# mratsim/trace-of-radiance

Measured on AMD Instinct MI355X. Metric: Msamples/s (pixels×spp/s) on book-1 random_scene, higher is better.
Workload: dtype f64

## Files before the change

include/tor_render.h:

```cpp
#ifndef TOR_RENDER_H
#define TOR_RENDER_H

#include <stddef.h>
#include <stdint.h>

#ifdef __cplusplus
extern "C" {
#endif

#define TOR_API __attribute__((visibility("default")))


typedef struct TorVec3 { double x, y, z; } TorVec3;

enum { TOR_LAMBERTIAN = 0, TOR_METAL = 1, TOR_DIELECTRIC = 2 };

typedef struct TorMaterial {
  uint8_t kind;
  uint8_t _pad[7];
  union {
    struct { TorVec3 albedo; } lambertian;
    struct { TorVec3 albedo; double fuzz; } metal;
    struct { double refraction_index; } dielectric;
  } u;
// ... 199 lines not shown
                                double time_hi, int32_t mode, TorHit* hits, const uint32_t* masks, uint32_t mask);
TOR_API int tor_occluded_masked_device(TorContext* ctx, int64_t n_rays, const TorRay* d_rays, const double* d_t_range,
                                       const int32_t* d_list, int64_t n_list, double time_lo, double time_hi, int32_t mode,
                                       int32_t* d_occluded, void* hip_stream, const uint32_t* d_mask, uint32_t mask);
TOR_API int tor_occluded_masked_host(TorContext* ctx, int64_t n_rays, const TorRay* rays, const double* t_range, const int32_t* list,
                                     int64_t n_list, double time_lo, double time_hi, int32_t mode, int32_t* occluded,
                                     const uint32_t* masks, uint32_t mask);
TOR_API int tor_bounce_masked_device(TorContext* ctx, int64_t n_rays, TorRay* d_rays, TorRng* d_rng, const int32_t* d_list,
                                     int64_t n_list, double time_lo, double time_hi, int32_t mode, TorHit* d_hits,
                                     double* d_attenuation, int32_t* d_status, void* hip_stream, const uint32_t* d_mask, uint32_t mask);

enum { TOR_CROSSINGS_MAX = 16 };
typedef struct TorCrossing { double t; int32_t object; int32_t which; } TorCrossing;
TOR_API int tor_crossings_device(TorContext* ctx, int64_t n_rays, const TorRay* d_rays, const double* d_t_range, const int32_t* d_list,
                                 int64_t n_list, int32_t k, const uint32_t* d_mask, uint32_t mask, double time_lo, double time_hi,
                                 int32_t mode, TorCrossing* d_cross, int32_t* d_count, TorHit* d_records, void* hip_stream);
TOR_API int tor_crossings_host(TorContext* ctx, int64_t n_rays, const TorRay* rays, const double* t_range, const int32_t* list,
                               int64_t n_list, int32_t k, const uint32_t* masks, uint32_t mask, double time_lo, double time_hi,
                               int32_t mode, TorCrossing* cross, int32_t* count, TorHit* records);

typedef struct TorPoint { TorVec3 p; double time; } TorPoint;
enum { TOR_NEAREST_MAX = 16 };
typedef struct TorNear { double distance; int32_t object; int32_t inside; } TorNear;
TOR_API int tor_nearest_device(TorContext* ctx, int64_t n_points, const TorPoint* d_points, const double* d_max_dist, const int32_t* d_list,
                               int64_t n_list, int32_t k, const uint32_t* d_mask, uint32_t mask, double time_lo, double time_hi,
                               int32_t mode, TorNear* d_near, int32_t* d_count, void* hip_stream);
TOR_API int tor_nearest_host(TorContext* ctx, int64_t n_points, const TorPoint* points, const double* max_dist, const int32_t* list,
                             int64_t n_list, int32_t k, const uint32_t* masks, uint32_t mask, double time_lo, double time_hi,
                             int32_t mode, TorNear* near, int32_t* count);

TOR_API int tor_deposit_device(TorContext* ctx, int64_t n, const double* d_color, const int32_t* d_pixel, const int32_t* d_index,
                               int64_t n_index, double max_value, int64_t npix, double* d_sums, double* d_moments, int32_t* d_counts,
                               int64_t* d_rejected, void* hip_stream);

TOR_API int tor_comm_unique_id(uint8_t id_out[128]);
TOR_API int tor_comm_init_rank(TorContext* ctx, const uint8_t id[128], int32_t rank, int32_t world);
TOR_API int tor_comm_destroy(TorContext* ctx);
TOR_API int tor_comm_abort(TorContext* ctx);
TOR_API int tor_comm_count(TorContext* ctx, int32_t* ranks_out);
TOR_API int tor_render_gather_device(TorContext* ctx, const TorCamera* cam, int32_t nrows, int32_t ncols,
                                     int32_t samples_per_pixel, float gamma_correction, int64_t max_depth,
                                     const TorOptions* opt, int32_t root, double* d_frame, void* hip_stream);

TOR_API int tor_context_handoff_stalled(TorContext* ctx, int32_t* stalled_out, int64_t* total_out);

TOR_API int tor_context_scene_counters(TorContext* ctx, int64_t out[3]);

TOR_API int tor_quantize_rgb8_device(TorContext* ctx, const double* d_pixels, int64_t n_values,
                                     uint8_t* d_rgb8, void* hip_stream);

TOR_API int tor_h264_stream_header(int32_t width, int32_t height, uint8_t* out, int32_t cap);
TOR_API int64_t tor_h264_frame_bytes(int32_t width, int32_t height);
TOR_API int tor_mp4_mux_file(const char* src_annexb_path, const char* dst_mp4_path, int32_t width,
                             int32_t height, int32_t fps);
TOR_API int tor_encode_frame_device(TorContext* ctx, const double* d_pixels, int32_t nrows, int32_t ncols,
                                    uint8_t* d_slice, uint8_t* d_y, uint8_t* d_cb, uint8_t* d_cr,
                                    void* hip_stream);

TOR_API int tor_render_frame_h264(TorContext* ctx, const TorCamera* cam, int32_t nrows, int32_t ncols,
                                  int32_t samples_per_pixel, float gamma_correction, int64_t max_depth,
                                  const TorOptions* opt, uint8_t* slice_out, int64_t cap);

TOR_API int tor_last_kernel_ms(TorContext* ctx, float* ms_out, int64_t* samples_out);
TOR_API int tor_kernel_ms_mean(TorContext* ctx, int32_t last_n, float* mean_ms_out, int32_t* n_used_out);

typedef struct TorStats {
  uint64_t hit_queries;
  uint64_t object_tests;
  uint64_t candidates;
  uint64_t wave_iterations;
  uint64_t lane_slots;
  uint64_t samples;
  uint64_t block_tests;
  uint64_t exact_tests;
} TorStats;
TOR_API int tor_context_set_stats(TorContext* ctx, int32_t enable);
TOR_API int tor_last_stats(TorContext* ctx, TorStats* out);
TOR_API int tor_last_wave_log(TorContext* ctx, uint64_t* out, int64_t cap_waves);
TOR_API int tor_last_handoff_counters(TorContext* ctx, uint64_t out[16]);
TOR_API int64_t tor_last_pixel_cost(TorContext* ctx, uint32_t* out, int64_t cap_pixels);


TOR_API int tor_camera_init(TorCamera* out, const TorVec3* look_from, const TorVec3* look_at,
                            const TorVec3* view_up, double vertical_fov_degrees,
                            double aspect_ratio, double aperture, double focus_distance,
                            double shutter_open, double shutter_close);

TOR_API int64_t tor_random_scene(uint64_t seed, TorHittableVariant* out, int64_t cap);

typedef struct TorAnimation TorAnimation;
TOR_API int tor_animation_create(uint64_t seed, int32_t height, int32_t width, float dt, float t_min,
                                 float t_max, TorAnimation** out);
TOR_API void tor_animation_destroy(TorAnimation* anim);
TOR_API int64_t tor_animation_object_count(const TorAnimation* anim);
TOR_API int tor_animation_next(TorAnimation* anim, int32_t skip, TorCamera* cam, TorHittableVariant* objects,
                               int64_t cap, int64_t* n_out, float* t_out);

TOR_API int tor_canvas_to_rgb8(const TorCanvas* canvas, uint8_t* out);


TOR_API int tor_debug_accel_layout(TorHittableList world, double t_lo, double t_hi, int64_t* slot_object,
                                   int64_t slot_cap, double* block_boxes, double* super_boxes, int64_t box_cap,
                                   int32_t* two_level_out);

TOR_API int tor_debug_last_variant(TorContext* ctx, int32_t out[5]);
TOR_API int tor_debug_last_split_tiles(TorContext* ctx, int64_t* tiles_out);

TOR_API int tor_debug_filter32_scene(TorHittableList world, int64_t n_rays, const double* o, const double* d,
                                     const double* time, int8_t* keep);

TOR_API int tor_debug_screen2_scene(TorHittableList world, int64_t n_rays, const double* o, const double* d,
                                    const double* time, int8_t* keep, int32_t* kind_out, int8_t* pays_out, int64_t n_segs_out);

TOR_API int tor_debug_plane32_scene(TorHittableList world, int64_t n_rays, const double* o, const double* d, const double* time,
                                    int8_t* keep, int32_t* pad_kept, int64_t* n_pad_out);

TOR_API int tor_debug_layout_segments(TorHittableList world, int32_t* out, int64_t max_segs, int64_t* n_segs_out);

TOR_API int tor_selftest_slab32_host(int64_t n, const double* o, const double* d, const double* lo, const double* hi,
                                     const double* origin, int32_t* keep, int32_t* need);

TOR_API int tor_selftest_filter32_host(int64_t n, const double* o, const double* d, const double* c0,
                                       const double* dc, const int32_t* moving, const double* f, const double* r2,
                                       const double* origin, int32_t* keep, int32_t* need);

TOR_API int tor_selftest_screen_host(int64_t n, const double* o, const double* d, const double* c0,
                                     const double* dc, const int32_t* moving, const double* f, const double* r2,
                                     int32_t* keep, int32_t* need);
TOR_API int tor_selftest_screen2_host(int64_t n, const double* o, const double* d, const double* c0,
                                      const double* dc, const int32_t* moving, const double* f, const double* r2,
                                      int32_t variant, int32_t* keep, int32_t* need);

TOR_API int tor_selftest_math_device(int32_t op, const double* x, const double* y, double* out0,
                                     double* out1, int64_t n, int32_t device);
TOR_API int tor_selftest_math_host(int32_t op, const double* x, const double* y, double* out0,
                                   double* out1, int64_t n);
TOR_API int tor_selftest_rng_host(int32_t mode, uint64_t a, uint64_t b, uint64_t c,
                                  uint64_t state_out[4], uint64_t* draws_out, int64_t n);

TOR_API const char* tor_version(void);

#ifdef __cplusplus
}
#endif

#include "tor_lights.h"

#include "tor_env.h"

#include "tor_camera.h"

#include "tor_bsdf.h"

#endif
```

trace-of-radiance_amd/__init__.py:

```python
from __future__ import annotations

import ctypes as C
import os
import subprocess
import sys

import numpy as np

_HERE = os.path.dirname(os.path.abspath(__file__))
LIB_PATH = os.path.join(_HERE, "lib", "libtor_mi355x.so")
INCLUDE_DIR = os.path.join(os.path.dirname(_HERE), "include")

SEED_PIXEL, SEED_SAMPLE = 0, 1
ARITH_STRICT, ARITH_FUSED = 0, 1
ACCEL_NONE, ACCEL_BLOCKS, ACCEL_F32 = 0, 1, 2
GATHER_AUTO, GATHER_RCCL, GATHER_PEER, GATHER_HOST = 0, 1, 2, 3
PIXEL_KERNEL_AUTO, PIXEL_KERNEL_LANE, PIXEL_KERNEL_WAVE = 0, 1, 2
OK, ERR_INVALID_ARGUMENT, ERR_NO_DEVICE, ERR_HIP, ERR_OUT_OF_MEMORY, ERR_INCOMPLETE = 0, -1, -2, -3, -4, -5
MAX_DEVICES = 16
LAMBERTIAN, METAL, DIELECTRIC = 0, 1, 2
SPHERE, MOVING_SPHERE = 0, 1


class TorError(RuntimeError):
    def __init__(self, code: int, msg: str):
        super().__init__(f"tor_mi355x error {code}: {msg}")
        self.code = code


class Vec3(C.Structure):
    _fields_ = [("x", C.c_double), ("y", C.c_double), ("z", C.c_double)]


class _Lambertian(C.Structure):
    _fields_ = [("albedo", Vec3)]


class _Metal(C.Structure):
    _fields_ = [("albedo", Vec3), ("fuzz", C.c_double)]


class _Dielectric(C.Structure):
    _fields_ = [("refraction_index", C.c_double)]


class _MaterialU(C.Union):
    _fields_ = [("lambertian", _Lambertian), ("metal", _Metal), ("dielectric", _Dielectric)]


class Material(C.Structure):
    _fields_ = [("kind", C.c_uint8), ("_pad", C.c_uint8 * 7), ("u", _MaterialU)]


class Sphere(C.Structure):
    _fields_ = [("center", Vec3), ("radius", C.c_double), ("material", Material)]


class MovingSphere(C.Structure):
    _fields_ = [("center0", Vec3), ("center1", Vec3), ("time0", C.c_double), ("time1", C.c_double),
                ("radius", C.c_double), ("material", Material)]


class _HittableU(C.Union):
    _fields_ = [("sphere", Sphere), ("moving_sphere", MovingSphere)]


class HittableVariant(C.Structure):
    _fields_ = [("kind", C.c_uint8), ("_pad", C.c_uint8 * 7), ("u", _HittableU)]


class HittableList(C.Structure):
    _fields_ = [("len", C.c_int64), ("objects", C.POINTER(HittableVariant))]


class Camera(C.Structure):
    _fields_ = [("origin", Vec3), ("lower_left_corner", Vec3), ("horizontal", Vec3), ("vertical", Vec3),
                ("u", Vec3), ("v", Vec3), ("w", Vec3), ("lens_radius", C.c_double),
                ("shutter_open", C.c_double), ("shutter_close", C.c_double)]

    def as_array(self) -> np.ndarray:
        return np.frombuffer(bytes(self), dtype=np.float64).copy()


class CanvasStruct(C.Structure):
    _fields_ = [("pixels", C.POINTER(Vec3)), ("nrows", C.c_int32), ("ncols", C.c_int32),
                ("samples_per_pixel", C.c_int32), ("gamma_correction", C.c_float)]


class Options(C.Structure):
    _fields_ = [("struct_size", C.c_uint32), ("seeding", C.c_int32), ("arith", C.c_int32),
                ("device", C.c_int32), ("shard_index", C.c_int32), ("shard_count", C.c_int32),
                ("row_tile", C.c_int32), ("accel", C.c_int32),
                ("device_count", C.c_int32), ("gather", C.c_int32), ("devices", C.c_int32 * MAX_DEVICES),
                ("pixel_kernel", C.c_int32)]


class Stats(C.Structure):
    _fields_ = [("hit_queries", C.c_uint64), ("object_tests", C.c_uint64), ("candidates", C.c_uint64),
                ("wave_iterations", C.c_uint64), ("lane_slots", C.c_uint64), ("samples", C.c_uint64),
                ("block_tests", C.c_uint64), ("exact_tests", C.c_uint64)]


class Ray(C.Structure):
    _fields_ = [("origin", Vec3), ("direction", Vec3), ("time", C.c_double)]


class Hit(C.Structure):
    _fields_ = [("p", Vec3), ("normal", Vec3), ("t", C.c_double), ("object", C.c_int32), ("front_face", C.c_int32)]


class Rng(C.Structure):
    _fields_ = [("s0", C.c_uint64), ("s1", C.c_uint64), ("s2", C.c_uint64), ("s3", C.c_uint64)]


assert C.sizeof(Rng) == 32
assert C.sizeof(Ray) == 56 and C.sizeof(Hit) == 64 and Hit.object.offset == 56 and Hit.front_face.offset == 60
assert C.sizeof(Vec3) == 24 and C.sizeof(Material) == 40 and C.sizeof(Sphere) == 72
assert C.sizeof(MovingSphere) == 112 and C.sizeof(HittableVariant) == 120
assert C.sizeof(HittableList) == 16 and C.sizeof(Camera) == 192 and C.sizeof(CanvasStruct) == 24

EXPORTED_SYMBOLS = [
    "tor_render", "tor_render_opt", "tor_last_error", "tor_context_create", "tor_context_destroy",
    "tor_scene_upload", "tor_shard_rows", "tor_render_device", "tor_quantize_rgb8_device",
    "tor_last_kernel_ms", "tor_kernel_ms_mean", "tor_context_set_stats", "tor_last_stats", "tor_last_wave_log", "tor_camera_init",
    "tor_random_scene", "tor_canvas_to_rgb8", "tor_animation_create", "tor_animation_destroy",
    "tor_animation_object_count", "tor_animation_next", "tor_h264_stream_header", "tor_h264_frame_bytes",
    "tor_encode_frame_device", "tor_render_frame_h264", "tor_mp4_mux_file", "tor_debug_accel_layout", "tor_selftest_filter32_host", "tor_selftest_screen_host", "tor_selftest_slab32_host", "tor_debug_filter32_scene", "tor_selftest_math_device", "tor_selftest_math_host",
    "tor_selftest_rng_host", "tor_version",
    "tor_last_render_timing", "tor_comm_unique_id", "tor_comm_init_rank", "tor_comm_destroy", "tor_render_gather_device",
    "tor_context_scene_counters", "tor_render_ptr", "tor_last_pixel_cost", "tor_last_note", "tor_last_handoff_counters",
    "tor_selftest_screen2_host", "tor_debug_screen2_scene", "tor_debug_layout_segments", "tor_debug_plane32_scene", "tor_knob_count", "tor_knob_info", "tor_last_gather_info", "tor_last_device_kernel_ms", "tor_comm_abort", "tor_comm_count", "tor_context_handoff_stalled",
    "tor_render_accumulate_device", "tor_resolve_device", "tor_accum_noise_device",
    "tor_render_accumulate_list_device", "tor_adaptive_select_device", "tor_resolve_counts_device", "tor_debug_last_variant",
    "tor_hit_device", "tor_hit_host", "tor_radiance_device", "tor_radiance_host", "tor_camera_rays_device",
    "tor_bounce_device", "tor_bounce_host", "tor_scatter_device", "tor_scatter_host", "tor_sky_device", "tor_bounce_select_device",
    "tor_render_resume_device", "tor_debug_last_split_tiles", "tor_render_resume_list_device",
    "tor_occluded_device", "tor_occluded_host",
    "tor_scene_groups", "tor_hit_masked_device", "tor_hit_masked_host", "tor_occluded_masked_device", "tor_occluded_masked_host",
    "tor_bounce_masked_device",
    "tor_crossings_device", "tor_crossings_host",
    "tor_nearest_device", "tor_nearest_host",
    "tor_deposit_device",
]
LIGHT_SYMBOLS = ["tor_scene_lights", "tor_light_sample_device", "tor_light_sample_host", "tor_light_pdf_device", "tor_light_pdf_host"]
LIGHT_BY_WEIGHT, LIGHT_BY_SOLID_ANGLE = 0, 1
LIGHT_STRATEGIES = {"weight": LIGHT_BY_WEIGHT, "solid_angle": LIGHT_BY_SOLID_ANGLE}
ENV_SYMBOLS = ["tor_scene_environment", "tor_env_sample_device", "tor_env_sample_host", "tor_env_eval_device", "tor_env_eval_host"]
ENV_MAX_SIDE = 2048
CAMERA_SYMBOLS = ["tor_camera_connect_device", "tor_camera_connect_host", "tor_light_emit_device", "tor_light_emit_host"]
BSDF_SYMBOLS = ["tor_bsdf_eval_device", "tor_bsdf_eval_host"]
BSDF_NONE, BSDF_DENSITY, BSDF_DELTA = 0, 1, 2
HIT_AUTO, HIT_BRUTE, HIT_BLOCKS = 0, 1, 2
HIT_MODES = {"auto": HIT_AUTO, "brute": HIT_BRUTE, "blocks": HIT_BLOCKS}
BOUNCE_MISS, BOUNCE_SCATTERED, BOUNCE_ABSORBED = 0, 1, 2
CROSSINGS_MAX = 16
NEAREST_MAX = 16
DEPOSIT_MAX_VALUE = 128.0
MAT_LAMBERTIAN, MAT_METAL, MAT_DIELECTRIC = 0, 1, 2

_lib = None


def build(force: bool = False) -> str:
    import fcntl
    src_dir = os.path.join(_HERE, "csrc")
    lock_path = os.path.join(src_dir, ".build.lock")
    if not os.access(src_dir, os.W_OK):
        import hashlib
        import tempfile
        lock_path = os.path.join(tempfile.gettempdir(), "tor_mi355x_" + hashlib.sha1(src_dir.encode()).hexdigest()[:12] + ".lock")
    with open(lock_path, "w") as lock:
        fcntl.flock(lock, fcntl.LOCK_EX)
        try:
            cmd = ["make", "-C", src_dir] + (["-B"] if force or not os.path.exists(LIB_PATH) else []) + ["all"]
            r = subprocess.run(cmd, capture_output=True, text=True)
            if r.returncode != 0:
                raise TorError(-3, f"building libtor_mi355x.so failed ({' '.join(cmd)}):\n{r.stdout[-4000:]}\n{r.stderr[-8000:]}")
        finally:
            fcntl.flock(lock, fcntl.LOCK_UN)
    return LIB_PATH


def ensure_built() -> str:
    if not os.path.exists(LIB_PATH):
        build()
    return LIB_PATH


def lib():
    global _lib
    if _lib is not None:
        return _lib
    if not os.path.exists(LIB_PATH):
        raise TorError(-2, f"HIP extension missing: {LIB_PATH} (run __graft_entry__.build()); "
                           "there is no CPU fallback")
    if os.environ.get("TOR_NO_TORCH", "0") != "1":
        try:
            import torch
        except Exception:
            pass
    ab = os.environ.get("TOR_AB_LIB")
    if ab:
        print(f"trace-of-radiance_amd: TOR_AB_LIB set -- loading {ab} instead of the in-tree library", file=sys.stderr, flush=True)
    L = C.CDLL(ab or LIB_PATH)
    _bind(L, skip_missing=bool(ab))
    _bind_lights(L, skip_missing=bool(ab))
    _bind_env(L, skip_missing=bool(ab))
    _bind_camera(L, skip_missing=bool(ab))
    _bind_bsdf(L, skip_missing=bool(ab))
    _lib = L
    return L


def _signatures() -> dict:
    v, i32, i64, u32, u64, d, f, P = C.c_void_p, C.c_int32, C.c_int64, C.c_uint32, C.c_uint64, C.c_double, C.c_float, C.POINTER
    dp, cam, opt, obj = P(d), P(Camera), P(Options), P(HittableVariant)
    frame = [v, cam, i32, i32, i32, f, i64, opt]
    passes = [v, cam, i32, i32, i32, i32, i64, opt]
    listed = [v, cam, i32, i32, v, i32, i32, i32, i64, opt]
    return {
        "tor_last_error": (None, C.c_char_p),
        "tor_version": (None, C.c_char_p),
        "tor_last_note": (None, C.c_char_p),
        "tor_render": [P(CanvasStruct), cam, HittableList, i64],
        "tor_render_ptr": [P(CanvasStruct), cam, P(HittableList), i64],
        "tor_render_opt": [P(CanvasStruct), cam, HittableList, i64, opt],
        "tor_context_create": [i32, P(v)],
        "tor_context_destroy": [v],
        "tor_scene_upload": [v, HittableList],
        "tor_shard_rows": [i32, i32, i32, i32, P(i32)],
        "tor_render_device": frame + [v, v],
        "tor_quantize_rgb8_device": [v, v, i64, v, v],
        "tor_last_kernel_ms": [v, P(f), P(i64)],
        "tor_kernel_ms_mean": [v, i32, P(f), P(i32)],
        "tor_context_set_stats": [v, i32],
        "tor_last_stats": [v, P(Stats)],
        "tor_last_wave_log": [v, P(u64), i64],
        "tor_last_pixel_cost": ([v, P(u32), i64], i64),
        "tor_last_handoff_counters": [v, P(u64)],
        "tor_camera_init": [cam, P(Vec3), P(Vec3), P(Vec3)] + [d] * 6,
        "tor_random_scene": ([u64, obj, i64], i64),
        "tor_canvas_to_rgb8": [P(CanvasStruct), P(C.c_uint8)],
        "tor_animation_create": [u64, i32, i32, f, f, f, P(v)],
        "tor_animation_destroy": ([v], None),
        "tor_animation_object_count": ([v], i64),
        "tor_animation_next": [v, i32, cam, obj, i64, P(i64), P(f)],
        "tor_h264_stream_header": [i32, i32, P(C.c_uint8), i32],
        "tor_h264_frame_bytes": ([i32, i32], i64),
        "tor_encode_frame_device": [v, v, i32, i32, v, v, v, v, v],
        "tor_render_frame_h264": frame + [P(C.c_uint8), i64],
        "tor_mp4_mux_file": [C.c_char_p, C.c_char_p, i32, i32, i32],
        "tor_debug_accel_layout": [HittableList, d, d, P(i64), i64, dp, dp, i64, P(i32)],
        "tor_selftest_filter32_host": [i64] + [dp] * 4 + [P(i32)] + [dp] * 3 + [P(i32)] * 2,
        "tor_selftest_screen_host": [i64] + [dp] * 4 + [P(i32)] + [dp] * 2 + [P(i32)] * 2,
        "tor_selftest_screen2_host": [i64] + [dp] * 4 + [P(i32)] + [dp] * 2 + [i32] + [P(i32)] * 2,
        "tor_selftest_slab32_host": [i64] + [dp] * 5 + [P(i32)] * 2,
        "tor_debug_filter32_scene": [HittableList, i64] + [dp] * 3 + [P(C.c_int8)],
        "tor_debug_screen2_scene": [HittableList, i64] + [dp] * 3 + [P(C.c_int8), P(i32), P(C.c_int8), i64],
        "tor_debug_plane32_scene": [HittableList, i64] + [dp] * 3 + [P(C.c_int8), P(i32), P(i64)],
        "tor_debug_layout_segments": [HittableList, P(i32), i64, P(i64)],
        "tor_selftest_math_device": [i32, dp, dp, dp, dp, i64, i32],
        "tor_selftest_math_host": [i32, dp, dp, dp, dp, i64],
        "tor_selftest_rng_host": [i32, u64, u64, u64, P(u64), P(u64), i64],
        "tor_last_render_timing": [dp],
        "tor_comm_unique_id": [P(C.c_uint8)],
        "tor_comm_init_rank": [v, P(C.c_uint8), i32, i32],
        "tor_comm_destroy": [v],
        "tor_render_gather_device": frame + [i32, v, v],
        "tor_context_scene_counters": [v, P(i64)],
        "tor_knob_count": (None, i32),
        "tor_knob_info": [i32] + [P(C.c_char_p)] * 5,
        "tor_last_gather_info": [P(i32)],
        "tor_last_device_kernel_ms": [P(f), i32],
        "tor_comm_abort": [v],
        "tor_comm_count": [v, P(i32)],
        "tor_context_handoff_stalled": [v, P(i32), P(i64)],
        "tor_render_accumulate_device": passes + [v, v, v],
        "tor_resolve_device": [v, v, i64, i64, f, v, v],
        "tor_accum_noise_device": [v, v, v, i64, i64, v, dp, v],
        "tor_render_accumulate_list_device": listed + [v, v, v],
        "tor_adaptive_select_device": [v, v, v, v, i32, i64, d, d, v, v, P(i32), v],
        "tor_resolve_counts_device": [v, v, v, i64, f, v, v],
        "tor_debug_last_variant": [v, P(i32)],
        "tor_render_resume_device": passes + [v, v, v, v],
        "tor_debug_last_split_tiles": [v, P(i64)],
        "tor_render_resume_list_device": listed + [v, v, v, v],
        "tor_hit_device": [v, i64, v, v, d, d, i32, v, v],
        "tor_hit_host": [v, i64, v, v, d, d, i32, v],
        "tor_hit_masked_device": [v, i64, v, v, d, d, i32, v, v, v, u32],
        "tor_hit_masked_host": [v, i64, v, v, d, d, i32, v, v, u32],
        "tor_radiance_device": [v, i64, v, v, i32, d, d, i32, v, v],
        "tor_radiance_host": [v, i64, v, v, i32, d, d, i32, v],
        "tor_camera_rays_device": [v, cam, i32, i32, v, i64, i32, i32, i32, v, v, v],
        "tor_bounce_device": [v, i64, v, v, v, i64, d, d, i32, v, v, v, v],
        "tor_bounce_host": [v, i64, v, v, v, i64, d, d, i32, v, v, v],
        "tor_bounce_masked_device": [v, i64, v, v, v, i64, d, d, i32, v, v, v, v, v, u32],
        "tor_scatter_device": [v, i64, v, v, v, v, i64, v, v, v],
        "tor_scatter_host": [v, i64, v, v, v, v, i64, v, v],
        "tor_sky_device": [v, i64, v, v, i64, v, v],
        "tor_bounce_select_device": [v, i64, v, v, i64, v, P(i64), v],
        "tor_occluded_device": [v, i64, v, v, v, i64, d, d, i32, v, v],
        "tor_occluded_host": [v, i64, v, v, v, i64, d, d, i32, v],
        "tor_occluded_masked_device": [v, i64, v, v, v, i64, d, d, i32, v, v, v, u32],
        "tor_occluded_masked_host": [v, i64, v, v, v, i64, d, d, i32, v, v, u32],
        "tor_scene_groups": [v, i64, v],
        "tor_crossings_device": [v, i64, v, v, v, i64, i32, v, u32, d, d, i32, v, v, v, v],
        "tor_crossings_host": [v, i64, v, v, v, i64, i32, v, u32, d, d, i32, v, v, v],
        "tor_nearest_device": [v, i64, v, v, v, i64, i32, v, u32, d, d, i32, v, v, v],
        "tor_nearest_host": [v, i64, v, v, v, i64, i32, v, u32, d, d, i32, v, v],
        "tor_deposit_device": [v, i64, v, v, v, i64, d, i64, v, v, v, v, v],
    }


_SIGNATURES = _signatures()


def _bind(L, names=None, skip_missing=False) -> None:
    for name in _SIGNATURES if names is None else names:
        if skip_missing and not hasattr(L, name):
            continue
        sig = _SIGNATURES[name]
        argtypes, *restype = sig if isinstance(sig, tuple) else (sig,)
        fn = getattr(L, name)
        if argtypes is not None:
            fn.argtypes = argtypes
        if restype:
            fn.restype = restype[0]


def _light_signatures() -> dict:
    v, i32, i64 = C.c_void_p, C.c_int32, C.c_int64
    return {
        "tor_scene_lights": [v, i64, v, v],
        "tor_light_sample_device": [v, i64, v, v, v, i64, i32, v, v, v, v, v],
        "tor_light_sample_host": [v, i64, v, v, v, i64, i32, v, v, v, v],
        "tor_light_pdf_device": [v, i64, v, v, v, i64, i32, v, v],
        "tor_light_pdf_host": [v, i64, v, v, v, i64, i32, v],
    }


_LIGHT_SIGNATURES = _light_signatures()


def _bind_lights(L, skip_missing=False) -> None:
    for name in LIGHT_SYMBOLS:
        if skip_missing and not hasattr(L, name):
            continue
        getattr(L, name).argtypes = _LIGHT_SIGNATURES[name]


def _env_signatures() -> dict:
    v, i64 = C.c_void_p, C.c_int64
    return {
        "tor_scene_environment": [v, i64, v, v],
        "tor_env_sample_device": [v, i64, v, v, v, i64, v, v, v, v, v],
        "tor_env_sample_host": [v, i64, v, v, v, i64, v, v, v, v],
        "tor_env_eval_device": [v, i64, v, v, i64, v, v, v, v],
        "tor_env_eval_host": [v, i64, v, v, i64, v, v, v],
    }


_ENV_SIGNATURES = _env_signatures()


def _bind_env(L, skip_missing=False) -> None:
    for name in ENV_SYMBOLS:
        if skip_missing and not hasattr(L, name):
            continue
        getattr(L, name).argtypes = _ENV_SIGNATURES[name]


def _camera_signatures() -> dict:
    v, i32, i64, d, cam = C.c_void_p, C.c_int32, C.c_int64, C.c_double, C.POINTER(Camera)
    return {
        "tor_camera_connect_device": [v, cam, i32, i32, i64, v, v, v, i64, v, v, v, v, v],
        "tor_camera_connect_host": [v, cam, i32, i32, i64, v, v, v, i64, v, v, v, v],
        "tor_light_emit_device": [v, i64, v, v, i64, d, d, v, v, v, v, v],
        "tor_light_emit_host": [v, i64, v, v, i64, d, d, v, v, v, v],
    }


_CAMERA_SIGNATURES = _camera_signatures()


def _bind_camera(L, skip_missing=False) -> None:
    for name in CAMERA_SYMBOLS:
        if skip_missing and not hasattr(L, name):
            continue
        getattr(L, name).argtypes = _CAMERA_SIGNATURES[name]


def _bsdf_signatures() -> dict:
    v, i64 = C.c_void_p, C.c_int64
    return {
        "tor_bsdf_eval_device": [v, i64, v, v, v, v, i64, v, v, v, v],
        "tor_bsdf_eval_host": [v, i64, v, v, v, v, i64, v, v, v],
    }


_BSDF_SIGNATURES = _bsdf_signatures()


def _bind_bsdf(L, skip_missing=False) -> None:
    for name in BSDF_SYMBOLS:
        if skip_missing and not hasattr(L, name):
            continue
        getattr(L, name).argtypes = _BSDF_SIGNATURES[name]


def _check(rc: int) -> None:
    if rc != 0:
        raise TorError(rc, lib().tor_last_error().decode("utf-8", "replace"))


_GOLDEN, _MIX = np.uint64(0x9e3779b97f4a7c15), np.uint64(0xbf58476d1ce4e5b9)


def _u64(x) -> np.ndarray:
    a = np.asarray(x)
    if a.dtype.kind == "u":
        return a.astype(np.uint64).reshape(-1)
    if a.dtype.kind == "i":
        return a.astype(np.int64).view(np.uint64).reshape(-1)
    return np.array([int(v) & 0xFFFFFFFFFFFFFFFF for v in a.reshape(-1)], dtype=np.uint64)


def _splitmix64(state: np.ndarray):
    with np.errstate(over="ignore"):
        state = state + _GOLDEN
        r = (state ^ (state >> np.uint64(30))) * _MIX
        r = (r ^ (r >> np.uint64(27))) * _MIX
    return state, r ^ (r >> np.uint64(31))


def rng_seed1(x) -> np.ndarray:
    sm = _u64(x)
    out = np.empty((sm.shape[0], 4), dtype=np.uint64)
    for k in range(4):
        sm, out[:, k] = _splitmix64(sm)
    return out


def rng_seed2(x, y) -> np.ndarray:
    x, y = np.broadcast_arrays(_u64(x), _u64(y))
    return rng_seed1((x << np.uint64(32)) ^ y)


def rng_seed3(row, col, sample) -> np.ndarray:
    row, col, sample = np.broadcast_arrays(_u64(row), _u64(col), _u64(sample))
    _, h = _splitmix64((row << np.uint64(32)) ^ col)
    return rng_seed1(h ^ sample)


def vec3(x, y, z) -> Vec3:
    return Vec3(float(x), float(y), float(z))


def camera(look_from=(13, 2, 3), look_at=(0, 0, 0), view_up=(0, 1, 0), vertical_field_of_view=20.0,
           aspect_ratio=16.0 / 9.0, aperture=0.1, focus_distance=10.0, shutter_open=0.0,
           shutter_close=1.0) -> Camera:
    cam = Camera()
    a, b, c = vec3(*look_from), vec3(*look_at), vec3(*view_up)
    _check(lib().tor_camera_init(C.byref(cam), C.byref(a), C.byref(b), C.byref(c),
                                 vertical_field_of_view, aspect_ratio, aperture, focus_distance,
                                 shutter_open, shutter_close))
    return cam


class Scene:

    def __init__(self, objects=None, n: int = 0):
        self.objects = objects if objects is not None else (HittableVariant * 1)()
        self.n = n

    def list(self) -> HittableList:
        return HittableList(self.n, C.cast(self.objects, C.POINTER(HittableVariant)))

    def __len__(self):
        return self.n

    @staticmethod
    def from_records(recs: np.ndarray) -> "Scene":
        n = int(recs.shape[0])
        arr = (HittableVariant * max(n, 1))()
        for i in range(n):
            r = recs[i]
            h = arr[i]
            mat = Material()
            mat.kind = int(r[10])
            if mat.kind == LAMBERTIAN:
                mat.u.lambertian.albedo = vec3(r[11], r[12], r[13])
            elif mat.kind == METAL:
                mat.u.metal.albedo = vec3(r[11], r[12], r[13])
                mat.u.metal.fuzz = float(r[14])
            else:
                mat.u.dielectric.refraction_index = float(r[15])
            if int(r[0]) == SPHERE:
                h.kind = SPHERE
                h.u.sphere.center = vec3(r[1], r[2], r[3])
                h.u.sphere.radius = float(r[9])
                h.u.sphere.material = mat
            else:
                h.kind = MOVING_SPHERE
                h.u.moving_sphere.center0 = vec3(r[1], r[2], r[3])
                h.u.moving_sphere.center1 = vec3(r[4], r[5], r[6])
                h.u.moving_sphere.time0 = float(r[7])
                h.u.moving_sphere.time1 = float(r[8])
                h.u.moving_sphere.radius = float(r[9])
                h.u.moving_sphere.material = mat
        return Scene(arr, n)

    def to_records(self) -> np.ndarray:
        out = np.zeros((self.n, 16), dtype=np.float64)
        for i in range(self.n):
            h = self.objects[i]
            if h.kind == SPHERE:
                s = h.u.sphere
                c0 = c1 = s.center
                t0, t1, rad, m = 0.0, 1.0, s.radius, s.material
            else:
                s = h.u.moving_sphere
                c0, c1, t0, t1, rad, m = s.center0, s.center1, s.time0, s.time1, s.radius, s.material
            out[i, 0] = h.kind
            out[i, 1:4] = (c0.x, c0.y, c0.z)
            out[i, 4:7] = (c1.x, c1.y, c1.z)
            out[i, 7:10] = (t0, t1, rad)
            out[i, 10] = m.kind
            if m.kind == LAMBERTIAN:
                a = m.u.lambertian.albedo
                out[i, 11:14] = (a.x, a.y, a.z)
            elif m.kind == METAL:
                a = m.u.metal.albedo
                out[i, 11:14] = (a.x, a.y, a.z)
                out[i, 14] = m.u.metal.fuzz
            else:
                out[i, 15] = m.u.dielectric.refraction_index
        return out


def random_scene(seed: int = 0xFACADE) -> Scene:
    cap = 2048
    arr = (HittableVariant * cap)()
    n = lib().tor_random_scene(seed, arr, cap)
    if n < 0:
        raise TorError(int(n), "tor_random_scene failed")
    return Scene(arr, int(n))


class Animation:

    def __init__(self, height: int, width: int, dt: float = 0.005, t_min: float = 0.0, t_max: float = 2.0,
                 seed: int = 0xFACADE):
        self._h = C.c_void_p()
        _check(lib().tor_animation_create(seed, height, width, dt, t_min, t_max, C.byref(self._h)))
        self.n_objects = int(lib().tor_animation_object_count(self._h))

    def scenes(self, skip: int = 6):
        while True:
            cam = Camera()
            arr = (HittableVariant * self.n_objects)()
# ... 1800 lines not shown
        self.rng = torch.zeros((self.rows, self.ncols, 4), dtype=torch.int64, device=self.sums.device)

    def _pass(self, k: int, stream: int) -> None:
        self.ctx.resume_list_device(self.cam, self.nrows, self.ncols, self._list.data_ptr(), self.active, self.samples, k,
                                    self.max_depth, self.options, self.rng.data_ptr(), self.sums.data_ptr(), self.moments.data_ptr(),
                                    stream)

    def state(self) -> dict:
        st = super().state()
        st["rng"] = self.rng.cpu().numpy().view(np.uint64)
        return st

    @classmethod
    def from_state(cls, ctx: Context, cam: Camera, nrows: int, ncols: int, max_depth: int, options: Options | None, state: dict,
                   device=None, **policy) -> "PixelAdaptive":
        import torch
        opts = options if options is not None else cls._default_options()
        want = (cls._shard_rows(nrows, opts), int(ncols), 4)
        rng = np.asarray(state.get("rng"))
        if rng.dtype != np.uint64 or rng.shape != want:
            raise TorError(ERR_INVALID_ARGUMENT, f"PixelAdaptive.from_state: generator states of dtype {rng.dtype}, shape {rng.shape}; "
                                                 f"expected uint64 {want}")
        ad = super().from_state(ctx, cam, nrows, ncols, max_depth, options, state, device=device, **policy)
        ad.rng.copy_(torch.from_numpy(np.ascontiguousarray(rng).view(np.int64)))
        return ad


def mp4_mux_file(src_annexb_path: str, dst_mp4_path: str, width: int, height: int, fps: int = 30) -> int:
    n = lib().tor_mp4_mux_file(os.fsencode(src_annexb_path), os.fsencode(dst_mp4_path), width, height, fps)
    if n < 0:
        raise TorError(n, lib().tor_last_error().decode())
    return n


def debug_accel_layout(world: HittableList, t_lo: float, t_hi: float):
    cap = int(world.len) + 64
    slots = np.full(cap, -1, dtype=np.int64)
    boxes = np.zeros((cap // 8 + 16, 6), dtype=np.float64)
    supers = np.zeros((cap // 64 + 16, 6), dtype=np.float64)
    two = C.c_int32(0)
    n = lib().tor_debug_accel_layout(world, t_lo, t_hi, slots.ctypes.data_as(C.POINTER(C.c_int64)), cap,
                                     boxes.ctypes.data_as(C.POINTER(C.c_double)),
                                     supers.ctypes.data_as(C.POINTER(C.c_double)), boxes.shape[0], C.byref(two))
    if n < 0:
        raise TorError(n, "tor_debug_accel_layout failed")
    if n == 0:
        return None
    n_p = (n + 7) // 8 * 8
    return slots[: n * 8].reshape(n, 8), boxes[:n_p], supers[: n_p // 8], bool(two.value)


def selftest_filter32(o, d, c0, dc, moving, f, r2, origin):
    dp = lambda x: np.ascontiguousarray(x, dtype=np.float64)
    o, d, c0, dc, f, r2, origin = dp(o), dp(d), dp(c0), dp(dc), dp(f), dp(r2), dp(origin)
    moving = np.ascontiguousarray(moving, dtype=np.int32)
    n = len(f)
    keep = np.zeros(n, dtype=np.int32)
    need = np.zeros(n, dtype=np.int32)
    P = C.POINTER(C.c_double)
    I = C.POINTER(C.c_int32)
    _check(lib().tor_selftest_filter32_host(n, o.ctypes.data_as(P), d.ctypes.data_as(P), c0.ctypes.data_as(P),
                                            dc.ctypes.data_as(P), moving.ctypes.data_as(I), f.ctypes.data_as(P),
                                            r2.ctypes.data_as(P), origin.ctypes.data_as(P), keep.ctypes.data_as(I),
                                            need.ctypes.data_as(I)))
    return keep, need


def selftest_screen(o, d, c0, dc, moving, f, r2):
    dp = lambda x: np.ascontiguousarray(x, dtype=np.float64)
    o, d, c0, dc, f, r2 = dp(o), dp(d), dp(c0), dp(dc), dp(f), dp(r2)
    moving = np.ascontiguousarray(moving, dtype=np.int32)
    n = len(f)
    keep = np.zeros(n, dtype=np.int32)
    need = np.zeros(n, dtype=np.int32)
    P = C.POINTER(C.c_double)
    I = C.POINTER(C.c_int32)
    _check(lib().tor_selftest_screen_host(n, o.ctypes.data_as(P), d.ctypes.data_as(P), c0.ctypes.data_as(P), dc.ctypes.data_as(P),
                                          moving.ctypes.data_as(I), f.ctypes.data_as(P), r2.ctypes.data_as(P), keep.ctypes.data_as(I),
                                          need.ctypes.data_as(I)))
    return keep, need


def selftest_screen2(o, d, c0, dc, moving, f, r2, variant=0):
    dp = lambda x: np.ascontiguousarray(x, dtype=np.float64)
    o, d, c0, dc, f, r2 = dp(o), dp(d), dp(c0), dp(dc), dp(f), dp(r2)
    moving = np.ascontiguousarray(moving, dtype=np.int32)
    n = len(f)
    keep = np.zeros(n, dtype=np.int32)
    need = np.zeros(n, dtype=np.int32)
    P = C.POINTER(C.c_double)
    I = C.POINTER(C.c_int32)
    _check(lib().tor_selftest_screen2_host(n, o.ctypes.data_as(P), d.ctypes.data_as(P), c0.ctypes.data_as(P), dc.ctypes.data_as(P),
                                           moving.ctypes.data_as(I), f.ctypes.data_as(P), r2.ctypes.data_as(P), int(variant),
                                           keep.ctypes.data_as(I), need.ctypes.data_as(I)))
    return keep, need


def selftest_slab32(o, d, lo, hi, origin):
    dp = lambda x: np.ascontiguousarray(x, dtype=np.float64)
    o, d, lo, hi, origin = dp(o), dp(d), dp(lo), dp(hi), dp(origin)
    n = len(o)
    keep = np.zeros(n, dtype=np.int32)
    need = np.zeros(n, dtype=np.int32)
    P = C.POINTER(C.c_double)
    I = C.POINTER(C.c_int32)
    _check(lib().tor_selftest_slab32_host(n, o.ctypes.data_as(P), d.ctypes.data_as(P), lo.ctypes.data_as(P), hi.ctypes.data_as(P),
                                          origin.ctypes.data_as(P), keep.ctypes.data_as(I), need.ctypes.data_as(I)))
    return keep, need


def debug_filter32_scene(world: HittableList, o, d, time):
    dp = lambda x: np.ascontiguousarray(x, dtype=np.float64)
    o, d, time = dp(o), dp(d), dp(time)
    keep = np.zeros((len(time), int(world.len)), dtype=np.int8)
    P = C.POINTER(C.c_double)
    _check(lib().tor_debug_filter32_scene(world, len(time), o.ctypes.data_as(P), d.ctypes.data_as(P), time.ctypes.data_as(P),
                                          keep.ctypes.data_as(C.POINTER(C.c_int8))))
    return keep


def debug_layout_segments(world: HittableList, max_segs: int = 64):
    out = np.zeros((max_segs, 4), dtype=np.int32)
    n = C.c_int64(0)
    _check(lib().tor_debug_layout_segments(world, out.ctypes.data_as(C.POINTER(C.c_int32)), max_segs, C.byref(n)))
    return [tuple(int(v) for v in row) for row in out[:min(int(n.value), max_segs)]]


def debug_screen2_scene(world: HittableList, o, d, time, max_segs: int = 0):
    dp = lambda x: np.ascontiguousarray(x, dtype=np.float64)
    o, d, time = dp(o), dp(d), dp(time)
    keep = np.zeros((len(time), int(world.len)), dtype=np.int8)
    kind = np.zeros(int(world.len), dtype=np.int32)
    pays = np.full((len(time), max(max_segs, 1)), -1, dtype=np.int8)
    P = C.POINTER(C.c_double)
    _check(lib().tor_debug_screen2_scene(world, len(time), o.ctypes.data_as(P), d.ctypes.data_as(P), time.ctypes.data_as(P),
                                         keep.ctypes.data_as(C.POINTER(C.c_int8)), kind.ctypes.data_as(C.POINTER(C.c_int32)),
                                         pays.ctypes.data_as(C.POINTER(C.c_int8)) if max_segs > 0 else None, max_segs))
    return (keep, kind, pays) if max_segs > 0 else (keep, kind)


def debug_plane32_scene(world: HittableList, o, d, time):
    dp = lambda x: np.ascontiguousarray(x, dtype=np.float64)
    o, d, time = dp(o), dp(d), dp(time)
    keep = np.zeros((len(time), int(world.len)), dtype=np.int8)
    pad_kept = np.zeros(len(time), dtype=np.int32)
    n_pad = C.c_int64(0)
    P = C.POINTER(C.c_double)
    _check(lib().tor_debug_plane32_scene(world, len(time), o.ctypes.data_as(P), d.ctypes.data_as(P), time.ctypes.data_as(P),
                                         keep.ctypes.data_as(C.POINTER(C.c_int8)), pad_kept.ctypes.data_as(C.POINTER(C.c_int32)),
                                         C.byref(n_pad)))
    return keep, pad_kept, int(n_pad.value)


def selftest_math(op: int, x: np.ndarray, y: np.ndarray | None = None, where: str = "device", device: int = -1):
    x = np.ascontiguousarray(x, dtype=np.float64)
    yy = np.ascontiguousarray(y, dtype=np.float64) if y is not None else None
    o0 = np.zeros_like(x)
    o1 = np.zeros_like(x)
    dp = C.POINTER(C.c_double)
    yp = yy.ctypes.data_as(dp) if yy is not None else None
    if where == "device":
        _check(lib().tor_selftest_math_device(op, x.ctypes.data_as(dp), yp, o0.ctypes.data_as(dp),
                                              o1.ctypes.data_as(dp), x.size, device))
    else:
        _check(lib().tor_selftest_math_host(op, x.ctypes.data_as(dp), yp, o0.ctypes.data_as(dp),
                                            o1.ctypes.data_as(dp), x.size))
    return o0, o1


def selftest_rng(mode: int, a: int, b: int = 0, c: int = 0, n: int = 4):
    state = (C.c_uint64 * 4)()
    draws = (C.c_uint64 * max(n, 1))()
    _check(lib().tor_selftest_rng_host(mode, a, b, c, state, draws, n))
    return [int(v) for v in state], [int(v) for v in draws[:n]]
```

trace-of-radiance_amd/csrc/kernel/integrate_loop_plane.inc:

```
            if constexpr (kWords) {
            const int x_first = h_xfirst;
            const int pl_first = h_plfirst;
            const bool mover = xkind >= 12;
            double f = 0.0;
            if (mover) {
              f = (time - SEG_T0) / SEG_DT;
              fc_f = f; fc_t0 = double_to_bits(SEG_T0); fc_dt = double_to_bits(SEG_DT);
            }
            const int i_begin = i;
            {
              const PlaneSeg ps = plane_seg(sray, pray, SEG_REACH, SEG_TRAVEL, f, h_rmax2);
              auto stage_one = [&](auto PWc) {
                constexpr int PW = decltype(PWc)::value;
                using Rec = std::conditional_t<PW == 2, float, double>;
                using RecPtr = std::conditional_t<PW == 2, cfptr, cdptr>;
                RecPtr rec = (RecPtr)(uintptr_t)(PW == 2 ? (const void*)p.xpl32 : (const void*)p.xpl) + ((long)pl_first + PW * (long)i);
                PlaneSeg32 ps32{};
                Rec n0, n1, n2 = 0, n3 = 0;
                if constexpr (PW == 2) {
                  ps32 = plane_seg32(sray, ps, h_r1, h_r2, (double)__int_as_float(__double2loint(h_r3)), (double)__int_as_float(__double2hiint(h_r3)));
                  n0 = __int_as_float(__double2loint(h_r0)); n1 = __int_as_float(__double2hiint(h_r0));
                } else {
                  n0 = h_r0; n1 = h_r1; n2 = h_r2; n3 = h_r3;
                }
                if (i != 0) {
                  n0 = rec[0]; n1 = rec[1];
                  if constexpr (PW == 4) { n2 = rec[2]; n3 = rec[3]; }
                }
                auto one = [&](unsigned m, int j) {
                  const Rec c0 = n0, c1 = n1, c2 = n2, c3 = n3;
                  n0 = rec[PW * (j + 1) + 0]; n1 = rec[PW * (j + 1) + 1];
                  if constexpr (PW == 4) {
                    n2 = rec[PW * (j + 1) + 2]; n3 = rec[PW * (j + 1) + 3];
                    return push_bit(m, plane_word_mov(ps, c0, c1, c2, c3));
                  } else {
                    (void)c2; (void)c3;
                    return push_bit(m, plane_word32(ps32, c0, c1));
                  }
                };
                int gb = seg_block0 + (int)((unsigned)i / (unsigned)kBlock);
                for (;;) {
                  while (i < seg_count && ((gb & 3) != 0 || seg_count - i < 4 * kBlock)) {
                    unsigned m = mw;
                    if (seg_real - i <= kBlock / 2) {
#pragma unroll
                      for (int j = 0; j < kBlock / 2; ++j) m = one(m, j);
                      m <<= (unsigned)(kBlock / 2);
                    } else {
#pragma unroll
                      for (int j = 0; j < kBlock; ++j) m = one(m, j);
                    }
                    rec += PW * kBlock;
                    mw = m;
                    gb_next = gb + 1;
                    i += kBlock;
                    if ((gb & 3) == 3) {
                      q[(unsigned)w_count * 64] = m;
                      nz = push_cond(nz, m != 0u);
                      w_count += 1;
                      if (w_count == kQCap) { full = true; break; }
                    }
                    gb += 1;
                  }
                  if (full || i >= seg_count) break;
                  int nw = (seg_count - i) / (4 * kBlock);
                  nw = nw < kQCap - w_count ? nw : kQCap - w_count;
                  unsigned m = 0;
                  int w = 0;
                  auto word = [&]() {
                    m = 0;
#pragma unroll
                    for (int j = 0; j < 4 * kBlock; ++j) m = one(m, j);
                    rec += PW * 4 * kBlock;
                    q[(unsigned)(w_count + w) * 64] = m;
                    nz = push_cond(nz, m != 0u);
                    w += 1;
                  };
#pragma unroll 1
                  while (w + 2 <= nw) { word(); word(); }
                  if (w < nw) word();
                  mw = m;
                  i += nw * 4 * kBlock;
                  gb += 4 * nw;
                  gb_next = gb;
                  w_count += nw;
                  if (w_count == kQCap) { full = true; break; }
                }
              };
              if (xkind == 13) stage_one(std::integral_constant<int, 4>{});
              else stage_one(std::integral_constant<int, 2>{});
            }
            {
              const int slot0 = seg_block0 * kBlock;
              const int slot_a = slot0 + i_begin, slot_b = slot0 + i;
              const int nb = gb_next & 3;
              const bool partial = !full && nb != 0;
              unsigned nzl = nz;
              if (partial) {
                const unsigned placed = mw << (unsigned)(8 * (4 - nb));
                q[(unsigned)w_count * 64] = placed;
                nzl = push_cond(nzl, placed != 0u);
              }
              const int k_a = (slot_a >> 5) - w_base, k_b = ((slot_b - 1) >> 5) - w_base;
              nzl &= (2u << (unsigned)(k_b - k_a)) - 1u;
              const bool shared_word = slot_b > slot_a && (slot_a & 31) != 0;
              unsigned sat_out = 0;
              if (shared_word) {
                const unsigned first_mask = 0xffffffffu >> (unsigned)(slot_a & 31);
                const unsigned w = q[(unsigned)k_a * 64];
                sat_out = w & ~first_mask;
                q[(unsigned)k_a * 64] = w & first_mask;
              }
              int k = k_a;
              unsigned cur = 0;
              unsigned* wp = q;
              const unsigned last_slot = (unsigned)(slot_b - 1);
              struct Pick { bool v; unsigned* w; int b; unsigned slot; };
              auto pick = [&]() {
                if (cur == 0 && nzl != 0) {
                  const int wb = 31 - __builtin_clz(nzl);
                  nzl &= ~(1u << wb);
                  k = k_b - wb;
                  wp = q + (unsigned)k * 64;
                  cur = *wp;
                }
                Pick c;
                c.v = cur != 0;
                c.b = 31 - __builtin_clz(cur | 1u);
                cur &= ~(1u << c.b);
                c.w = wp;
                const unsigned slot = ((unsigned)(w_base + k) << 5) + (unsigned)(31 - c.b);
                c.slot = slot < last_slot ? slot : last_slot;
                return c;
              };
              unsigned long long s2_t0 = 0;
              if (prof && lane == 0) s2_t0 = __builtin_readcyclecounter();
              if (slot_b > slot_a && xkind <= 12) {
                const ScreenSeg ss = screen2_seg(sray, SEG_REACH, SEG_TRAVEL, h_y, f);
                auto stage_two = [&](auto xr, auto KINDc) {
                  constexpr int KIND = decltype(KINDc)::value;
                  struct Cand { bool v; unsigned* w; int b; double r0, r1, r2, r3; };
                  constexpr bool kRecLds = std::is_same<decltype(xr), ldptr>::value;
                  unsigned lds_base = 0;
                  if constexpr (kRecLds) {
                    lds_base = (unsigned)(uintptr_t)xr;
                    asm volatile("" : "+v"(lds_base));
                  }
                  auto fetch = [&](Cand& c) {
                    const Pick pk = pick();
                    c.v = pk.v; c.w = pk.w; c.b = pk.b;
                    if constexpr (kRecLds) {
                      const ldptr r = (ldptr)(uintptr_t)(lds_base + pk.slot * 32u);
                      c.r0 = r[0]; c.r1 = r[1]; c.r2 = r[2]; c.r3 = r[3];
                    } else {
                      const auto r = xr + 4 * (long)pk.slot;
                      c.r0 = r[0]; c.r1 = r[1]; c.r2 = r[2]; c.r3 = r[3];
                    }
                  };
                  auto test = [&](const Cand& c) {
                    const int word = KIND == 12   ? screen2_movy_y<true>(ss, c.r0, c.r1, c.r2, c.r3)
                                     : KIND == 11 ? screen2_static_y<true>(ss, c.r0, c.r1, c.r2)
                                                  : screen2_static<true>(ss, c.r0, c.r1, c.r2, c.r3);
                    if (c.v && word >= 0) atomicAnd(c.w, ~(1u << c.b));
                  };
                  Cand ca{false, q, 0, 0.0, 0.0, 0.0, 0.0}, cb{false, q, 0, 0.0, 0.0, 0.0, 0.0};
                  fetch(ca);
                  for (;;) {
                    if (ballot64(ca.v || nzl != 0) == 0) break;
                    fetch(cb);
                    test(ca);
                    if (ballot64(cb.v || nzl != 0) == 0) break;
                    fetch(ca);
                    test(cb);
                  }
                };
                auto run = [&](auto KINDc) {
                  if (xstaged) stage_two((ldptr)stage + ((long)x_first - 4 * (long)slot0), KINDc);
                  else stage_two((gdptr)(uintptr_t)p.xrec + ((long)x_first - 4 * (long)slot0), KINDc);
                };
                if (xkind == 12) run(std::integral_constant<int, 12>{});
                else if (xkind == 11) run(std::integral_constant<int, 11>{});
                else run(std::integral_constant<int, 10>{});
                plane_ran = true;
              } else if (slot_b > slot_a) {
                double negmu, am;
                screen_margins(scr_s1 + SEG_REACH + SEG_TRAVEL * __builtin_fabs(f), scr_d1, a, negmu, am);
                const double neg_f = -f;
                auto stage_two = [&](auto xr) {
                  constexpr bool kRecLds = std::is_same<decltype(xr), ldptr>::value;
                  unsigned lds_base = 0;
                  if constexpr (kRecLds) {
                    lds_base = (unsigned)(uintptr_t)xr;
                    asm volatile("" : "+v"(lds_base));
                  }
                  for (;;) {
                    const Pick pk = pick();
                    if (ballot64(pk.v || nzl != 0) == 0) break;
                    double r0, r1, r2, r3, r4, r5, r6;
                    if constexpr (kRecLds) {
                      const ldptr r = (ldptr)(uintptr_t)(lds_base + pk.slot * 64u);
                      r0 = r[0]; r1 = r[1]; r2 = r[2]; r3 = r[3]; r4 = r[4]; r5 = r[5]; r6 = r[6];
                    } else {
                      const auto r = xr + 8 * (long)pk.slot;
                      r0 = r[0]; r1 = r[1]; r2 = r[2]; r3 = r[3]; r4 = r[4]; r5 = r[5]; r6 = r[6];
                    }
                    const int word = screen_filter(fma_(neg_f, r4, ox - r0), fma_(neg_f, r5, oy - r1), fma_(neg_f, r6, oz - r2), dx, dy, dz, a, negmu, am, r3);
                    if (pk.v && word >= 0) atomicAnd(pk.w, ~(1u << pk.b));
                  }
                };
                if (xstaged) stage_two((ldptr)stage + ((long)x_first - 8 * (long)slot0));
                else stage_two((gdptr)(uintptr_t)p.xrec + ((long)x_first - 8 * (long)slot0));
                plane_ran = true;
              }
              if (prof && lane == 0) prof_lds[kSecStage2] += __builtin_readcyclecounter() - s2_t0;
              if (shared_word) q[(unsigned)k_a * 64] |= sat_out;
              if (partial) mw = q[(unsigned)w_count * 64] >> (unsigned)(8 * (4 - nb));
            }
            }
```

trace-of-radiance_amd/csrc/tor_api.cpp:

```cpp
#include "../../include/tor_render.h"

#include <hip/hip_runtime_api.h>

#include <chrono>
#include <cmath>
#include <cstdio>
#include <cstdlib>
#include <cstring>
#include <map>
#include <mutex>
#include <new>
#include <string>
#include <utility>
#include <vector>

#include "tor_context.hpp"
#include "tor_knobs.hpp"
#include "tor_screen.hpp"

static_assert(sizeof(TorVec3) == 24, "Vec3 is 3 x float64 (vec3s.nim:12-14)");
static_assert(sizeof(TorMaterial) == 40 && offsetof(TorMaterial, u) == 8, "Material (core.nim:16-28)");
static_assert(sizeof(TorSphere) == 72, "Sphere (spheres.nim:15-18)");
static_assert(sizeof(TorMovingSphere) == 112, "MovingSphere (moving_spheres.nim:15-20)");
static_assert(sizeof(TorHittableVariant) == 120 && offsetof(TorHittableVariant, u) == 8,
              "HittableVariant (hittables_variants.nim:50-57)");
static_assert(sizeof(TorHittableList) == 16, "HittableList (hittables_lists.nim:20-24)");
static_assert(sizeof(TorCamera) == 192, "Camera (cameras.nim:15-22)");
static_assert(sizeof(TorCanvas) == 24, "Canvas (canvas.nim:20-28)");
static_assert(sizeof(tor::Camera) == sizeof(TorCamera), "device camera mirrors TorCamera");
static_assert(offsetof(TorOptions, device_count) == 32, "the round-1 TorOptions is a prefix of the current one");

namespace {
std::mutex g_handoff_mutex;
std::map<int, hipEvent_t> g_handoff_event;
thread_local std::string g_last_error = "";
thread_local double g_last_timing[5] = {0, 0, 0, 0, 0};
}

namespace tor {

void set_last_error(const std::string& msg) { g_last_error = msg; }

int fail(int code, const std::string& msg) {
  g_last_error = msg;
  return code;
}

int fail_hip(hipError_t e, const char* what) {
  std::string m = std::string(what) + ": " + hipGetErrorString(e);
  if (e == hipErrorNoDevice || e == hipErrorInvalidDevice || e == hipErrorInsufficientDriver)
    return fail(TOR_ERR_NO_DEVICE, m + " (libtor_mi355x has no CPU fallback)");
  if (e == hipErrorOutOfMemory) return fail(TOR_ERR_OUT_OF_MEMORY, m);
  return fail(TOR_ERR_HIP, m);
}

hipError_t DeviceLayout::put(const HostLayout& lay, const std::vector<double>* cold_override) {
  const std::vector<double>& c = cold_override ? *cold_override : lay.cold;
  struct Part { const void* src; size_t bytes; size_t off; };
  Part parts[11] = {{lay.stat.data(), lay.stat.size() * 8, 0}, {lay.mov.data(), lay.mov.size() * 8, 0},
                   {lay.movy.data(), lay.movy.size() * 8, 0}, {lay.segs.data(), lay.segs.size() * 8, 0},
                   {c.data(), c.size() * 8, 0},               {lay.hot32.data(), lay.hot32.size() * 4, 0},
                   {lay.coop_trips.data(), lay.coop_trips.size() * 8, 0},
                   {lay.xhdr.data(), lay.xhdr.size() * 8, 0}, {lay.xrec.data(), lay.xrec.size() * 8, 0},
                    {lay.xpl.data(), lay.xpl.size() * 8, 0}, {lay.xpl32.data(), lay.xpl32.size() * 4, 0}};
  size_t total = 0;
  for (Part& p : parts) {
    p.off = total;
    total += (p.bytes + 255) / 256 * 256 + 256;
  }
  std::vector<unsigned char> host(total, 0);
  for (const Part& p : parts)
    if (p.bytes > 0) std::memcpy(host.data() + p.off, p.src, p.bytes);
  hipError_t e = blob.ensure(total);
  if (e == hipSuccess) e = hipMemcpy(blob.ptr, host.data(), total, hipMemcpyHostToDevice);
  const char* b = (const char*)blob.ptr;
  stat = (const double*)(b + parts[0].off);
  mov = (const double*)(b + parts[1].off);
  movy = (const double*)(b + parts[2].off);
  segs = (const double*)(b + parts[3].off);
  cold = (const double*)(b + parts[4].off);
  hot32 = (const float*)(b + parts[5].off);
  coop_trips = (const double*)(b + parts[6].off);
  xhdr = (const double*)(b + parts[7].off);
  xrec = (const double*)(b + parts[8].off);
  xpl = (const double*)(b + parts[9].off);
  xpl32 = (const float*)(b + parts[10].off);
  n_segs = lay.n_segs;
  n_sorted = (int)lay.n_sorted;
  n_xrec = (int)lay.xrec.size();
  has_f32 = false;
  for (int s = 0; s < lay.n_segs; ++s) has_f32 = has_f32 || lay.segs[8 * (size_t)s] >= 5.0;
  return e;
}

static bool parse_device_list(const char* e, TorOptions& o) {
  int count = 0;
  if (hipGetDeviceCount(&count) != hipSuccess || count <= 0) return false;
  o.device_count = 0;
  if (std::strcmp(e, "all") == 0) {
    for (int d = 0; d < count && d < TOR_MAX_DEVICES; ++d) o.devices[o.device_count++] = d;
    return true;
  }
  const char* p = e;
  while (*p) {
    char* endp = nullptr;
    const long v = std::strtol(p, &endp, 10);
    if (endp == p || v < 0 || v >= count || o.device_count >= TOR_MAX_DEVICES) return false;
    o.devices[o.device_count++] = (int32_t)v;
    p = endp;
    if (*p == ',') ++p;
    else if (*p) return false;
  }
  return o.device_count > 0;
}

thread_local std::string g_options_why;
const std::string& options_why() { return g_options_why; }

bool valid_options(const TorOptions* opt, TorOptions& o, bool for_drop_in) {
  g_options_why.clear();
  auto no = [](const char* why) { g_options_why = why; return false; };
  o = TorOptions{};
  o.struct_size = sizeof(TorOptions);
  o.seeding = TOR_SEED_PIXEL;
  o.arith = TOR_ARITH_STRICT;
  o.device = -1;
  o.shard_index = 0;
  o.shard_count = 1;
  o.row_tile = 1;
  o.gather = TOR_GATHER_AUTO;
  constexpr uint32_t kV1Size = 32;
  if (opt) {
    if (opt->struct_size == sizeof(TorOptions)) o = *opt;
    else if (opt->struct_size == kV1Size) std::memcpy(&o, opt, kV1Size);
    else return no("struct_size is neither sizeof(TorOptions) nor the 32-byte round-1 layout");
    o.struct_size = sizeof(TorOptions);
  } else if (for_drop_in) {
    o.accel = TOR_ACCEL_BLOCKS | TOR_ACCEL_F32;
    if (const char* e = tor::knob("TOR_DEFAULT_ACCEL")) {
      char* endp = nullptr;
      const long v = std::strtol(e, &endp, 10);
      if (endp != e && *endp == 0 && v >= 0 && v <= (TOR_ACCEL_BLOCKS | TOR_ACCEL_F32)) o.accel = (int32_t)v;
      else return no("TOR_DEFAULT_ACCEL must be 0, 1, 2 or 3");
    }
    if (const char* e = tor::knob("TOR_DEFAULT_SEEDING")) {
      if (!std::strcmp(e, "sample")) o.seeding = TOR_SEED_SAMPLE;
      else if (!std::strcmp(e, "pixel")) o.seeding = TOR_SEED_PIXEL;
      else return no("TOR_DEFAULT_SEEDING must be pixel or sample");
    }
    if (const char* e = tor::knob("TOR_DEVICES")) {
      TorOptions t = o;
      if (parse_device_list(e, t)) o = t;
      else return no("TOR_DEVICES must be \"all\" or a comma list of HIP device ordinals that exist (at most TOR_MAX_DEVICES)");
    }
    if (const char* e = tor::knob("TOR_GATHER")) {
      if (!std::strcmp(e, "rccl")) o.gather = TOR_GATHER_RCCL;
      else if (!std::strcmp(e, "peer")) o.gather = TOR_GATHER_PEER;
      else if (!std::strcmp(e, "host")) o.gather = TOR_GATHER_HOST;
      else if (!std::strcmp(e, "auto")) o.gather = TOR_GATHER_AUTO;
      else return no("TOR_GATHER must be auto, rccl, peer or host");
    }
  }
  if (o.seeding != TOR_SEED_PIXEL && o.seeding != TOR_SEED_SAMPLE) return no("seeding must be TOR_SEED_PIXEL or TOR_SEED_SAMPLE");
  if (o.arith == TOR_ARITH_FUSED)
    return no("TOR_ARITH_FUSED was removed in round 5: it was not the reference's rounding (README.md:82) and TOR_ARITH_STRICT behind the conservative "
              "FMA screen is faster -- pass TOR_ARITH_STRICT (0)");
  if (o.arith != TOR_ARITH_STRICT) return no("arith must be TOR_ARITH_STRICT");
  if (o.accel < 0 || o.accel > (TOR_ACCEL_BLOCKS | TOR_ACCEL_F32)) return no("accel holds unknown TOR_ACCEL_* bits");
  if (o.shard_count < 1) o.shard_count = 1;
  if (o.row_tile == 0) o.row_tile = 1;
  if (o.row_tile < 0) return no("row_tile must be >= 1");
  if (o.shard_index < 0 || o.shard_index >= o.shard_count) return no("shard_index must lie in [0, shard_count)");
  if (o.device_count < 0 || o.device_count > TOR_MAX_DEVICES) return no("device_count must lie in [0, TOR_MAX_DEVICES]");
  if (o.gather < TOR_GATHER_AUTO || o.gather > TOR_GATHER_HOST) return no("gather must be a TOR_GATHER_* value");
  if (o.pixel_kernel < TOR_PIXEL_KERNEL_AUTO || o.pixel_kernel > TOR_PIXEL_KERNEL_WAVE) return no("pixel_kernel must be a TOR_PIXEL_KERNEL_* value");
  if (o.device_count > 1) {
    if (o.shard_count != 1 || o.shard_index != 0) return no("with a device list, shard_index / shard_count must be left at 0 / 1: entry k renders shard k");
    if (o.device > 0) {
      bool listed = false;
      for (int k = 0; k < o.device_count; ++k) listed = listed || o.devices[k] == o.device;
      if (!listed) return no("with a device list, `device` must be -1, 0 or one of the listed ordinals (it is ignored)");
    }
    o.device = -1;
    for (int k = 0; k < o.device_count; ++k)
      if (o.devices[k] < 0) return no("negative ordinal in the device list");
  } else if (o.device_count == 1) {
    if (o.devices[0] < 0) return no("negative ordinal in the device list");
    o.device = o.devices[0];
  }
  return true;
}

int ensure_layouts(TorContext* ctx, int accel) {
  const TorHittableVariant* objs = (const TorHittableVariant*)ctx->scene_bytes.data();
  const int64_t n = ctx->n_objects;
  const bool want_f32 = (accel & TOR_ACCEL_F32) != 0;
  const bool want_blocks = (accel & TOR_ACCEL_BLOCKS) != 0;
  if (want_f32 && !ctx->f32_built) {
    ctx->f32 = f32_options_for(objs, n);
    ctx->f32_built = true;
  }
  auto build_flat = [&](int v) -> int {
    if (ctx->flat_built[v]) return TOR_OK;
    std::vector<int64_t> ids((size_t)n);
    for (int64_t i = 0; i < n; ++i) ids[(size_t)i] = i;
    HostLayout lay;
    std::string err;
    if (!build_layout(objs, ids, lay, err, v == 1 ? &ctx->f32 : nullptr)) return fail(TOR_ERR_INVALID_ARGUMENT, "tor_scene_upload: " + err);
    if (n == 0) lay.n_segs = 0;
    HIP_TRY(ctx->flat[v].put(lay));
    ctx->flat_built[v] = true;
    ctx->n_layouts_built += 1;
    return TOR_OK;
  };
  auto build_blocks = [&](int v) -> int {
    if (ctx->accel_built[v]) return TOR_OK;
    build_accel(objs, n, ctx->accel[v], v == 1 ? &ctx->f32 : nullptr);
    if (!ctx->accel[v].available) {
      ctx->accel_built[v] = true;
      return TOR_OK;
    }
    struct Rollback {
      TorContext* c; int v; bool ok = false;
      ~Rollback() { if (!ok) { c->d_accel[v].release(); c->accel[v] = tor::HostAccel{}; } }
    } rollback{ctx, v};
    auto put = [](DeviceBuffer& b, const void* src, size_t bytes) -> hipError_t {
      hipError_t e = b.ensure(bytes > 0 ? bytes : 8);
      if (e == hipSuccess && bytes > 0) e = hipMemcpy(b.ptr, src, bytes, hipMemcpyHostToDevice);
      return e;
    };
    HIP_TRY(ctx->d_accel[v].always.put(ctx->accel[v].always, &ctx->accel[v].cold));
    HIP_TRY(put(ctx->d_accel[v].hot, ctx->accel[v].hot.data(), ctx->accel[v].hot.size() * 8));
    HIP_TRY(put(ctx->d_accel[v].grp, ctx->accel[v].groups.data(), ctx->accel[v].groups.size() * 8));
    if (ctx->accel[v].sp32) HIP_TRY(put(ctx->d_accel[v].hot32, ctx->accel[v].hot32.data(), ctx->accel[v].hot32.size() * 4));
    const size_t n_bnd_p = (ctx->accel[v].n_blocks + kPad - 1) / kPad * kPad;
    const size_t n_super_p = (n_bnd_p / kPad + kPad - 1) / kPad * kPad;
    const size_t slot_bytes = (8 * (n_bnd_p + 1 + n_super_p + 1)) * (8 + 4);
    if (slot_bytes * TorContext::kRing > ctx->bnd_ring.bytes) {
      if (ctx->bnd_ring.ptr) HIP_TRY(hipDeviceSynchronize());
// ... 168 lines not shown
  HIP_TRY(hipEventSynchronize(ctx->ev_stop[ctx->last_slot]));
  unsigned long long w = 0;
  HIP_TRY(hipMemcpy(&w, (unsigned long long*)ctx->counters.ptr + (size_t)ctx->last_slot * TorContext::kSlotWords + 6, sizeof w, hipMemcpyDeviceToHost));
  *tiles_out = (int64_t)w;
  return TOR_OK;
}

int tor_context_scene_counters(TorContext* ctx, int64_t out[3]) {
  if (!ctx || !out) return fail(TOR_ERR_INVALID_ARGUMENT, "tor_context_scene_counters: NULL argument");
  out[0] = ctx->n_uploads;
  out[1] = ctx->n_cache_hits;
  out[2] = ctx->n_layouts_built;
  return TOR_OK;
}

int tor_scene_upload(TorContext* ctx, TorHittableList world) {
  if (!ctx) return fail(TOR_ERR_INVALID_ARGUMENT, "tor_scene_upload: ctx is NULL");
  if (world.len < 0 || (world.len > 0 && !world.objects))
    return fail(TOR_ERR_INVALID_ARGUMENT, "tor_scene_upload: bad HittableList");
  if (world.len > (int64_t)1 << 24) return fail(TOR_ERR_INVALID_ARGUMENT, "tor_scene_upload: too many objects");
  ctx->n_uploads += 1;
  const size_t bytes = (size_t)world.len * sizeof(TorHittableVariant);
  if (ctx->scene_ready && ctx->n_objects == world.len && ctx->scene_bytes.size() == bytes &&
      (bytes == 0 || std::memcmp(ctx->scene_bytes.data(), world.objects, bytes) == 0)) {
    ctx->n_cache_hits += 1;
    return TOR_OK;
  }
  for (int64_t i = 0; i < world.len; ++i) {
    const TorHittableVariant& h = world.objects[i];
    if (h.kind != TOR_SPHERE && h.kind != TOR_MOVING_SPHERE) return fail(TOR_ERR_INVALID_ARGUMENT, "tor_scene_upload: unknown HittableVariant kind");
    const uint8_t mk = h.kind == TOR_SPHERE ? h.u.sphere.material.kind : h.u.moving_sphere.material.kind;
    if (mk > TOR_DIELECTRIC) return fail(TOR_ERR_INVALID_ARGUMENT, "tor_scene_upload: unknown Material kind");
  }
  HIP_TRY(hipSetDevice(ctx->device));
  if (ctx->scene_ready) HIP_TRY(hipDeviceSynchronize());
  ctx->scene_ready = false;
  ctx->scene_bytes.assign((const unsigned char*)world.objects, (const unsigned char*)world.objects + bytes);
  ctx->n_objects = world.len;
  for (int v = 0; v < 2; ++v) ctx->flat_built[v] = ctx->accel_built[v] = false;
  ctx->f32_built = false;
  ctx->hitq.groups.clear();
  ctx->hitq.groups_gen += 1;
  ctx->hitq.n_lights = 0;
  ctx->scene_ready = true;
  return TOR_OK;
}

int32_t tor_shard_rows(int32_t nrows, int32_t row_tile, int32_t shard_index, int32_t shard_count,
                       int32_t* rows_out) {
  if (nrows <= 0) return 0;
  if (shard_count < 1) shard_count = 1;
  if (row_tile < 1) row_tile = 1;
  if (shard_index < 0 || shard_index >= shard_count) return 0;
  int32_t n = 0;
  for (int32_t r = 0; r < nrows; ++r)
    if ((r / row_tile) % shard_count == shard_index) {
      if (rows_out) rows_out[n] = r;
      ++n;
    }
  return n;
}

static hipError_t launch_integrate_recorded(TorContext* ctx, const tor::KParams& p, int seeding, int arith, int waves_per_simd, int blocks,
                                            hipStream_t stream) {
  const hipError_t e = tor::launch_integrate(p, seeding, arith, waves_per_simd, blocks, stream);
  if (e == hipSuccess) tor::integrate_variant_key(p, seeding, arith, waves_per_simd, ctx->last_variant);
  return e;
}

static int render_device_impl(TorContext* ctx, const TorCamera* cam, int32_t nrows, int32_t ncols,
                              int32_t spp, float gamma_correction, int64_t max_depth, const TorOptions* opt,
                              double* d_pixels, void* hip_stream, const tor::AccumLaunch* acc) {
  const bool listed = acc && acc->list;
  const bool resume = acc && acc->rng;
  const bool rlist = resume && listed;
  const std::string who = rlist ? "tor_render_resume_list_device" : resume ? "tor_render_resume_device" : (listed ? "tor_render_accumulate_list_device" : (acc ? "tor_render_accumulate_device" : "tor_render_device"));
  if (!ctx || !cam || !d_pixels) return fail(TOR_ERR_INVALID_ARGUMENT, who + ": NULL argument");
  if (!ctx->scene_ready) return fail(TOR_ERR_INVALID_ARGUMENT, who + ": no scene uploaded");
  if (nrows < 2 || ncols < 2 || spp < 1)
    return fail(TOR_ERR_INVALID_ARGUMENT, who + ": need nrows >= 2, ncols >= 2, samples_per_pixel >= 1");
  if (max_depth > 0x7fffffff) max_depth = 0x7fffffff;
  TorOptions o;
  if (!valid_options(opt, o, false)) return fail(TOR_ERR_INVALID_ARGUMENT, who + ": bad TorOptions: " + tor::options_why());
  if (o.device_count > 1) return fail(TOR_ERR_INVALID_ARGUMENT, who + ": one context renders on one device (device lists: tor_render_opt)");
  if (resume && o.seeding != TOR_SEED_PIXEL)
    return fail(TOR_ERR_INVALID_ARGUMENT, who + ": needs TOR_SEED_PIXEL -- it continues the reference's per-pixel streams (render.nim:59-67) from per-pixel "
                                                "generator states; passes of TOR_SEED_SAMPLE streams are tor_render_accumulate_device's");
  if (acc && !resume && o.seeding != TOR_SEED_SAMPLE)
    return fail(TOR_ERR_INVALID_ARGUMENT, who + ": needs TOR_SEED_SAMPLE -- a TOR_SEED_PIXEL pixel is one sequential chain of "
                                                "samples on one generator (render.nim:59-67); resuming it would need per-pixel RNG state");
  const int kseed = rlist ? 7 : resume ? (acc->moments ? 6 : 5) : (listed ? 4 : ((acc && acc->moments) ? 3 : o.seeding));
  hipStream_t stream = (hipStream_t)hip_stream;
  HIP_TRY(hipSetDevice(ctx->device));

  const int32_t local_rows = tor_shard_rows(nrows, o.row_tile, o.shard_index, o.shard_count, nullptr);
  const long long npix = (long long)local_rows * ncols;
  const long long n_values = npix * 3;
  const long long work_pix = listed ? (long long)acc->n_list : npix;
  ctx->timing_valid = false;
  ctx->last_samples = 0;
  ctx->last_migrate = false;
  ctx->last_split = false;
  if (work_pix == 0) return TOR_OK;

  const int slot = (int)(ctx->launches % TorContext::kRing);
  if (ctx->launches >= TorContext::kRing) HIP_TRY(hipEventSynchronize(ctx->ev_stop[slot]));
  if (ctx->launches > 0 && ctx->last_stream_valid && ctx->last_stream != hip_stream) {
    const hipError_t q = hipEventQuery(ctx->ev_stop[ctx->last_slot]);
    if (q == hipErrorNotReady)
      return fail(TOR_ERR_INVALID_ARGUMENT, who + ": the previous launch of this context is still running on a different stream -- "
                                                  "launches of one context that may overlap must use ONE stream (or use one context per stream)");
    if (q != hipSuccess) return fail_hip(q, "hipEventQuery");
  }
  ctx->last_stream = hip_stream;
  ctx->last_stream_valid = true;
  unsigned long long* const slot_counters = (unsigned long long*)ctx->counters.ptr + (size_t)slot * TorContext::kSlotWords;
  HIP_TRY(hipMemsetAsync(slot_counters, 0, TorContext::kSlotWords * sizeof(unsigned long long), stream));
  if (!resume && (max_depth <= 0 || ctx->n_objects < 0)) {
    if (acc) return TOR_OK;
    HIP_TRY(hipMemsetAsync(d_pixels, 0, (size_t)n_values * 8, stream));
    return TOR_OK;
  }
  if (o.seeding == TOR_SEED_SAMPLE && !acc) HIP_TRY(hipMemsetAsync(d_pixels, 0, (size_t)n_values * 8, stream));

  tor::KParams p{};
  float split_frac = ctx->split_frac;
  if (split_frac < 0.0f) {
    split_frac = 0.0f;
    if (o.accel == (TOR_ACCEL_BLOCKS | TOR_ACCEL_F32) && npix <= 1200000) {
      split_frac = 20000.0f / (float)npix;
      if (split_frac > 0.2f) split_frac = 0.2f;
      if (split_frac < 0.02f) split_frac = 0.02f;
    }
  }
  auto configure = [&](tor::KParams& q, int accel, std::vector<double>& bnd_host, std::vector<float>& bnd32_host, bool& use_accel, int& stage_wg,
                       const tor::HostAccel*& hacc_out) -> int {
    {
      const int rc = tor::ensure_layouts(ctx, accel);
      if (rc != TOR_OK) return rc;
    }
    int v32 = (accel & TOR_ACCEL_F32) ? 1 : 0;
    if (v32 && (accel & TOR_ACCEL_BLOCKS) && ctx->accel[1].available && !ctx->accel[1].sp32) v32 = 0;
    auto use_layout = [&](const tor::DeviceLayout& L) {
      q.stat = L.stat;
      q.mov = L.mov;
      q.movy = L.movy;
      q.segs = L.segs;
      q.cold = L.cold;
      q.hot32 = L.has_f32 ? L.hot32 : nullptr;
      q.xhdr = L.xhdr;
      q.xrec = L.xrec;
      q.xpl = ctx->plane_screen != 0 ? L.xpl : nullptr;
      q.xpl32 = ctx->plane_screen != 0 ? L.xpl32 : nullptr;
      q.plane_gate2 = ctx->plane_screen == 2 ? 0.0 : 4.0 * tor::kPlaneGate * tor::kPlaneGate;
      q.xrec_lds_doubles = 0;
      if (q.xpl != nullptr && ctx->screen && accel == 0) {
        const size_t wgs = (size_t)std::max(1, ctx->max_blocks_per_cu[o.seeding][0]);
        const size_t need = (size_t)L.n_xrec * 8 + (size_t)tor::integrate_fixed_lds_bytes(0, 0, kseed);
        if (need <= (size_t)(160 * 1024) / wgs - 1024 && need <= (size_t)64 * 1024) q.xrec_lds_doubles = L.n_xrec;
      }
      q.n_segs = L.n_segs;
    };
    const bool blocks_avail = (accel & TOR_ACCEL_BLOCKS) && ctx->accel_built[v32] && ctx->accel[v32].available;
    if (!blocks_avail) use_layout(ctx->flat[v32]);
    for (int k = 0; k < 3; ++k) q.org[k] = ctx->f32.origin[k];
    q.bnd = nullptr;
    q.spatial_base = 0;
    q.shot = nullptr;
    q.sgrp = nullptr;
    q.shot_lds_doubles = 0;
    q.shot_stride = 8;
    use_accel = false;
    stage_wg = 0;
    const tor::HostAccel& hacc = ctx->accel[v32];
    hacc_out = &hacc;
    if (blocks_avail) {
      const double t_lo = std::fmin(0.0, std::fmin(cam->shutter_open, cam->shutter_close));
      const double t_hi = std::fmax(0.0, std::fmax(cam->shutter_open, cam->shutter_close));
      use_accel = tor::compute_block_bounds(hacc, t_lo, t_hi, bnd_host);
      if (!use_accel) {
        const int rc = tor::ensure_layouts(ctx, accel & ~TOR_ACCEL_BLOCKS);
        if (rc != TOR_OK) return rc;
        use_layout(ctx->flat[v32]);
      }
    }
    if (use_accel) {
      use_layout(ctx->d_accel[v32].always);
      q.bnd = (const double*)((char*)ctx->bnd_ring.ptr + (size_t)slot * ctx->bnd_slot_bytes);
      q.spatial_base = (int)hacc.spatial_base;
      q.n_super = (int)(tor::accel_boxes_padded(hacc) / tor::kPad);
      q.two_level = hacc.two_level ? 1 : 0;
      q.box_reach2 = -1.0;
      q.box_amin = INFINITY;
      for (int k = 0; k < 3; ++k) q.box_org[k] = 0.0;
      if (!(v32 && hacc.sp32)) tor::block_reach(hacc, bnd_host, q.box_org, &q.box_reach2, &q.box_amin);
      q.shot = (const double*)ctx->d_accel[v32].hot.ptr;
      q.sgrp = (const double*)ctx->d_accel[v32].grp.ptr;
      q.shot_stride = hacc.hot_stride;
      q.shot32 = nullptr;
      if (v32 && hacc.sp32) {
        q.shot32 = (const float*)ctx->d_accel[v32].hot32.ptr;
        q.shot32_stride = hacc.hot32_stride;
        q.shot32_block_stride = hacc.hot32_block_stride;
        q.sp_mc0max = hacc.sp_mc0max; q.sp_dcmax = hacc.sp_dcmax;
        q.sp_t0 = hacc.sp_t0; q.sp_dt = hacc.sp_dt;
      }
      size_t hot_bytes = q.shot32 ? hacc.hot32.size() * 4 : hacc.hot.size() * 8;
      size_t bnd32_stage_floats = 0;
      if (q.shot32) {
        q.sp_bmax = tor::block_bounds_f32(bnd_host, ctx->f32.origin, bnd32_host, &q.sp_hmin);
        q.bnd32 = (const float*)((const char*)q.bnd + bnd_host.size() * 8);
        if (hacc.two_level) bnd32_stage_floats = 8 * tor::accel_boxes_padded(hacc);
      }
      const char* st = tor::knob("TOR_STAGE_LDS");
      const size_t hard_cap = st ? (size_t)std::atoll(st) : (size_t)1 << 30;
      int& wg = stage_wg;
      wg = 0;
      auto fits = [&](size_t bytes, int wgs) {
        return bytes <= hard_cap && bytes + (size_t)tor::integrate_fixed_lds_bytes(1, q.shot32 != nullptr ? 1 : 0, kseed) <= (size_t)(160 * 1024) / (size_t)wgs - 1024;
      };
      const int full = ctx->max_blocks_per_cu[o.seeding][accel != 0];
      const bool stage_boxes = q.shot32 && bnd32_stage_floats > 0 && fits(bnd32_stage_floats * 4, full);
      const size_t box_bytes = stage_boxes ? bnd32_stage_floats * 4 : 0;
      bool stage_hot = fits(hot_bytes + box_bytes, full);
      wg = (stage_hot || stage_boxes) ? full : 0;
      if (!q.shot32 && !stage_hot && full > 2 && fits(hot_bytes, full - 1)) {
        stage_hot = true;
        wg = full - 1;
      }
      q.shot_lds_doubles = (stage_hot && !q.shot32) ? (int)hacc.hot.size() : 0;
      q.shot32_lds_floats = (stage_hot && q.shot32) ? (int)hacc.hot32.size() : 0;
      q.bnd32_lds_floats = stage_boxes ? (int)bnd32_stage_floats : 0;
    }
    return TOR_OK;
  };
  bool use_accel = false;
  int stage_wg = 0;
  const tor::HostAccel* hacc_p = nullptr;
  bool configured = false;
  int cap = 0, waves_per_simd = 0;
  long long resident_waves = 0;
  auto configure_frame = [&]() -> int {
    if (configured) return TOR_OK;
    const int rc = configure(p, o.accel, ctx->bnd_host[slot], ctx->bnd32_host[slot], use_accel, stage_wg, hacc_p);
    if (rc != TOR_OK) return rc;
    cap = ctx->max_blocks_per_cu[o.seeding][o.accel != 0];
    if (cap < 1) cap = 4;
    if (stage_wg > 0 && stage_wg < cap) cap = stage_wg;
    waves_per_simd = ctx->waves_override > 0 ? ctx->waves_override : ((cap >= 2 && cap <= 4) ? cap : 4);
    int bpc_eff = tor::integrate_blocks_per_cu(p, kseed, o.arith, waves_per_simd);
    if (bpc_eff > cap) bpc_eff = cap;
    resident_waves = (long long)ctx->num_cus * bpc_eff * (tor::kThreads / 64);
    configured = true;
    return TOR_OK;
  };
  const long long n_tiles = (npix + tor::kTilePixelsHost - 1) / tor::kTilePixelsHost;
  bool migrate = false;
  if (o.seeding == TOR_SEED_PIXEL && o.pixel_kernel == TOR_PIXEL_KERNEL_AUTO && ctx->mig_mode != 0 && o.accel == (TOR_ACCEL_BLOCKS | TOR_ACCEL_F32) &&
      ctx->lpt_min_spp > 0 && spp >= ctx->lpt_min_spp && npix > tor::kTilePixelsHost && !ctx->collect_stats && ctx->n_objects > 0 &&
      !resume) {
    const int rc = configure_frame();
    if (rc != TOR_OK) return rc;
    const tor::HostAccel& ha = ctx->accel[1];
    migrate = ctx->accel_built[1] && ha.available && ha.sp32 && !ha.two_level && tor::accel_boxes_padded(ha) <= 128 &&
              use_accel && n_tiles > 1 && tor::integrate_variant_serves_chains(p, o.seeding) && resident_waves >= 8;
  }
  const bool split_applies = !migrate && o.pixel_kernel == TOR_PIXEL_KERNEL_AUTO && split_frac > 0.0f && ctx->lpt_min_spp > 0 && spp >= ctx->lpt_min_spp &&
                             npix >= ctx->split_min_pixels && npix <= ctx->split_max_pixels && !ctx->collect_stats && ctx->n_objects > 0 &&
                             !rlist;
  const long long coop_max_listed = ctx->coop_max_pixels / 4 * 3;
  const bool want_wave_kernel = o.pixel_kernel == TOR_PIXEL_KERNEL_WAVE ||
                                (o.pixel_kernel == TOR_PIXEL_KERNEL_AUTO && ctx->coop_max_pixels > 0 && (rlist ? work_pix <= coop_max_listed : npix <= ctx->coop_max_pixels) && !split_applies && !migrate);
  if (o.seeding == TOR_SEED_PIXEL && !ctx->collect_stats && want_wave_kernel && ctx->n_objects > 0) {
    const int rc = tor::ensure_layouts(ctx, 0);
    if (rc != TOR_OK) return rc;
    const tor::DeviceLayout& L = ctx->flat[0];
    tor::KParams wp{};
    wp.cold = L.cold;
    wp.n_cold_slots = L.n_sorted;
    wp.coop_slots = (L.n_sorted + 63) / 64 * 64;
    wp.coop_trips = L.coop_trips;
    const int bpc = tor::coop_blocks_per_cu(wp, o.arith);
    if (bpc > 0) {
      wp.nrows = nrows; wp.ncols = ncols; wp.spp = spp; wp.max_depth = (int)max_depth;
      wp.shard_index = o.shard_index; wp.shard_count = o.shard_count; wp.row_tile = o.row_tile;
      wp.n_pixels = (unsigned)npix;
      wp.work_counter = slot_counters;
      wp.out = d_pixels;
      if (resume) { wp.first_sample = acc->first_sample; wp.mom = acc->moments; wp.rstate = acc->rng; }
      if (rlist) { wp.pixel_list = acc->list; wp.total_work = (unsigned long long)work_pix; }
      ctx->cam_host[slot] = *cam;
      wp.cam_dev = (const double*)((char*)ctx->cam_ring.ptr + (size_t)slot * sizeof(TorCamera));
      HIP_TRY(hipMemcpyAsync((void*)wp.cam_dev, &ctx->cam_host[slot], sizeof(TorCamera), hipMemcpyHostToDevice, stream));
      long long blocks = ((rlist ? work_pix : npix) + (tor::kThreads / 64) - 1) / (tor::kThreads / 64);
      const long long resident = (long long)ctx->num_cus * bpc;
      if (blocks > resident) blocks = resident;
      HIP_TRY(hipEventRecord(ctx->ev_start[slot], stream));
      HIP_TRY(tor::launch_coop(wp, o.arith, (int)blocks, stream));
      HIP_TRY(hipEventRecord(ctx->ev_stop[slot], stream));
      ctx->launches += 1;
      ctx->last_slot = slot;
      ctx->timing_valid = true;
      ctx->last_samples = (int64_t)(rlist ? work_pix : npix) * spp;
      if (resume) return TOR_OK;
      HIP_TRY(tor::launch_finalize(d_pixels, n_values, 1.0 / (double)spp, 1.0 / (double)gamma_correction, stream));
      return TOR_OK;
// ... 847 lines not shown
          std::memcpy(&orig, &lay.cold[16 * slot + 14], 8);
          const bool padding = lay.cold[16 * slot + 15] < 0.0;
          const int bit = (m >> (7 - j)) & 1;
          if (!padding) kr[orig] = (int8_t)bit;
        }
      }
    }
  }
  return TOR_OK;
}

int tor_debug_layout_segments(TorHittableList world, int32_t* out, int64_t max_segs, int64_t* n_segs_out) {
  if (world.len < 0 || (world.len > 0 && !world.objects) || max_segs < 0 || (max_segs > 0 && !out) || !n_segs_out)
    return fail(TOR_ERR_INVALID_ARGUMENT, "tor_debug_layout_segments: bad argument");
  std::vector<int64_t> ids((size_t)world.len);
  for (int64_t i = 0; i < world.len; ++i) ids[(size_t)i] = i;
  tor::HostLayout lay;
  std::string err;
  if (!tor::build_layout(world.objects, ids, lay, err, nullptr)) return fail(TOR_ERR_INVALID_ARGUMENT, err);
  *n_segs_out = lay.n_segs;
  for (int s = 0; s < lay.n_segs && s < max_segs; ++s) {
    const double* sg = &lay.segs[8 * (size_t)s];
    const int count = (int)sg[2] & 0xffffff, real = count - ((int)sg[2] >> 24);
    out[4 * s + 0] = (int32_t)lay.xsegs[8 * (size_t)s];
    out[4 * s + 1] = real;
    out[4 * s + 2] = count;
    out[4 * s + 3] = (int32_t)sg[3] * (int32_t)tor::kPad;
  }
  return TOR_OK;
}

int tor_debug_screen2_scene(TorHittableList world, int64_t n_rays, const double* o, const double* d, const double* time, int8_t* keep,
                            int32_t* kind_out, int8_t* pays_out, int64_t n_segs_out) {
  if (world.len < 0 || (world.len > 0 && !world.objects) || n_rays < 0 || !o || !d || !time || !keep)
    return fail(TOR_ERR_INVALID_ARGUMENT, "tor_debug_screen2_scene: bad argument");
  std::vector<int64_t> ids((size_t)world.len);
  for (int64_t i = 0; i < world.len; ++i) ids[(size_t)i] = i;
  tor::HostLayout lay;
  std::string err;
  if (!tor::build_layout(world.objects, ids, lay, err, nullptr)) return fail(TOR_ERR_INVALID_ARGUMENT, err);
  auto orig_of = [&](size_t slot) {
    int64_t v;
    std::memcpy(&v, &lay.cold[16 * slot + 14], 8);
    return v;
  };
  for (int64_t r = 0; r < n_rays; ++r) {
    int8_t* kr = keep + r * world.len;
    for (int64_t i = 0; i < world.len; ++i) kr[i] = 3;
    const double* oo = o + 3 * r; const double* dd = d + 3 * r;
    const double a = dd[0] * dd[0] + dd[1] * dd[1] + dd[2] * dd[2];
    const tor::ScreenRay ray = tor::screen2_ray(oo[0], oo[1], oo[2], dd[0], dd[1], dd[2], a);
    const tor::PlaneRay pray = tor::plane_ray(ray);
    for (int s = 0; s < lay.n_segs; ++s) {
      const double* sg = &lay.segs[8 * (size_t)s];
      const double* xs = &lay.xsegs[8 * (size_t)s];
      const int xkind = (int)xs[0];
      const int count = (int)sg[2] & 0xffffff, real = count - ((int)sg[2] >> 24), block0 = (int)sg[3];
      if (r == 0 && kind_out)
        for (int i = 0; i < real; ++i) kind_out[orig_of((size_t)block0 * tor::kPad + (size_t)i)] = xkind;
      if (xkind < 10) continue;
      const double f = xkind >= 12 ? (time[r] - sg[4]) / sg[5] : 0.0;
      const tor::ScreenSeg ss = tor::screen2_seg(ray, sg[6], sg[7], xs[2], f);
      const tor::PlaneSeg ps = tor::plane_seg(ray, pray, sg[6], sg[7], f, xs[4]);
      double negmu = 0.0, am = 0.0;
      tor::screen_margins(ray.s1 + sg[6] + sg[7] * std::fabs(f), std::fabs(dd[0]) + std::fabs(dd[1]) + std::fabs(dd[2]), a, negmu, am);
      const size_t xsz = xkind >= 13 ? 8 : 4, pw = xkind == 13 ? 4 : 2;
      for (int i = 0; i < real; ++i) {
        const double* x = &lay.xrec[(size_t)xs[1] + xsz * (size_t)i];
        const double* pl = &lay.xpl[(size_t)xs[3] + pw * (size_t)i];
        const bool table_ok = xkind == 10   ? (pl[0] == x[0] && pl[1] == x[2])
                              : xkind <= 12 ? (pl[0] == x[0] && pl[1] == x[1])
                              : xkind == 13 ? (pl[0] == x[0] && pl[1] == x[2] && pl[2] == x[4] && pl[3] == x[6])
                                            : (pl[0] == x[0] && pl[1] == x[2] && x[4] == 0.0 && x[6] == 0.0);
        if (!table_ok) return fail(TOR_ERR_INVALID_ARGUMENT, "tor_debug_screen2_scene: the plane table and the records disagree (layout bug)");
        int8_t verdict;
        const int w1 = xkind == 13 ? tor::plane_word_mov(ps, pl[0], pl[1], pl[2], pl[3]) : tor::plane_word(ps, pl[0], pl[1]);
        if (w1 >= 0) {
          verdict = 0;
        } else {
          int w2;
          if (xkind == 10) w2 = tor::screen2_static(ss, x[0], x[1], x[2], x[3]);
          else if (xkind == 11) w2 = tor::screen2_static_y(ss, x[0], x[1], x[2]);
          else if (xkind == 12) w2 = tor::screen2_movy_y(ss, x[0], x[1], x[2], x[3]);
          else w2 = tor::screen_filter(tor::fma_(-f, x[4], oo[0] - x[0]), tor::fma_(-f, x[5], oo[1] - x[1]), tor::fma_(-f, x[6], oo[2] - x[2]), dd[0], dd[1], dd[2], a, negmu, am, x[3]);
          verdict = w2 < 0 ? 2 : 1;
        }
        kr[orig_of((size_t)block0 * tor::kPad + (size_t)i)] = verdict;
      }
      if (pays_out && s < n_segs_out) pays_out[r * n_segs_out + s] = tor::plane_pays(pray, 4.0 * tor::kPlaneGate * tor::kPlaneGate, xs[4], xs[5], xs[6]) ? 1 : 0;
    }
  }
  return TOR_OK;
}

int tor_debug_plane32_scene(TorHittableList world, int64_t n_rays, const double* o, const double* d, const double* time, int8_t* keep,
                            int32_t* pad_kept, int64_t* n_pad_out) {
  if (world.len < 0 || (world.len > 0 && !world.objects) || n_rays < 0 || !o || !d || !time || !keep || !pad_kept || !n_pad_out)
    return fail(TOR_ERR_INVALID_ARGUMENT, "tor_debug_plane32_scene: bad argument");
  std::vector<int64_t> ids((size_t)world.len);
  for (int64_t i = 0; i < world.len; ++i) ids[(size_t)i] = i;
  tor::HostLayout lay;
  std::string err;
  if (!tor::build_layout(world.objects, ids, lay, err, nullptr)) return fail(TOR_ERR_INVALID_ARGUMENT, err);
  auto orig_of = [&](size_t slot) {
    int64_t v;
    std::memcpy(&v, &lay.cold[16 * slot + 14], 8);
    return v;
  };
  *n_pad_out = 0;
  for (int s = 0; s < lay.n_segs; ++s) {
    const double* sg = &lay.segs[8 * (size_t)s];
    const int xkind = (int)lay.xsegs[8 * (size_t)s];
    if (xkind >= 10 && xkind != 13) *n_pad_out += ((int)sg[2] >> 24);
  }
  for (int64_t r = 0; r < n_rays; ++r) {
    int8_t* kr = keep + r * world.len;
    for (int64_t i = 0; i < world.len; ++i) kr[i] = -1;
    pad_kept[r] = 0;
    const double* oo = o + 3 * r; const double* dd = d + 3 * r;
    const double a = dd[0] * dd[0] + dd[1] * dd[1] + dd[2] * dd[2];
    const tor::ScreenRay ray = tor::screen2_ray(oo[0], oo[1], oo[2], dd[0], dd[1], dd[2], a);
    const tor::PlaneRay pray = tor::plane_ray(ray);
    for (int s = 0; s < lay.n_segs; ++s) {
      const double* sg = &lay.segs[8 * (size_t)s];
      const double* xs = &lay.xsegs[8 * (size_t)s];
      const double* h = &lay.xhdr[16 * (size_t)s];
      const int xkind = (int)xs[0];
      if (xkind < 10 || xkind == 13) continue;
      const int count = (int)sg[2] & 0xffffff, real = count - ((int)sg[2] >> 24), block0 = (int)sg[3];
      const double f = xkind >= 12 ? (time[r] - sg[4]) / sg[5] : 0.0;
      const tor::PlaneSeg ps = tor::plane_seg(ray, pray, sg[6], sg[7], f, xs[4]);
      float first[2], ec[2];
      std::memcpy(first, &h[12], 8);
      std::memcpy(ec, &h[15], 8);
      const tor::PlaneSeg32 ps32 = tor::plane_seg32(ray, ps, h[13], h[14], (double)ec[0], (double)ec[1]);
      for (int i = 0; i < count; ++i) {
        const float* pl32 = &lay.xpl32[(size_t)xs[3] + 2 * (size_t)i];
        if (i == 0 && !(pl32[0] == first[0] && pl32[1] == first[1]))
          return fail(TOR_ERR_INVALID_ARGUMENT, "tor_debug_plane32_scene: the header's first record and the table disagree (layout bug)");
        const bool k32 = tor::plane_word32(ps32, pl32[0], pl32[1]) < 0;
        if (i >= real) {
          pad_kept[r] += k32 ? 1 : 0;
          continue;
        }
        const double* pl = &lay.xpl[(size_t)xs[3] + 2 * (size_t)i];
        const bool k64 = tor::plane_word(ps, pl[0], pl[1]) < 0;
        kr[orig_of((size_t)block0 * tor::kPad + (size_t)i)] = (int8_t)((k64 ? 1 : 0) | (k32 ? 2 : 0));
      }
    }
  }
  return TOR_OK;
}

int tor_selftest_slab32_host(int64_t n, const double* o, const double* d, const double* lo, const double* hi,
                             const double* origin, int32_t* keep, int32_t* need) {
  if (n < 0 || !o || !d || !lo || !hi || !origin || !keep || !need)
    return fail(TOR_ERR_INVALID_ARGUMENT, "tor_selftest_slab32_host: bad argument");
  std::vector<double> bnd((size_t)n * 8, 0.0);
  for (int64_t i = 0; i < n; ++i)
    for (int k = 0; k < 3; ++k) { bnd[8 * i + k] = lo[3 * i + k]; bnd[8 * i + 3 + k] = hi[3 * i + k]; }
  std::vector<float> bnd32;
  float hmin = 0.0f;
  const float bmax = tor::block_bounds_f32(bnd, origin, bnd32, &hmin);
  using tor::f2v;
  for (int64_t i = 0; i < n; ++i) {
    const double* oo = o + 3 * i; const double* dd = d + 3 * i;
    const double a = dd[0] * dd[0] + dd[1] * dd[1] + dd[2] * dd[2];
    const tor::RayF32 r = tor::make_ray_f32(oo[0], oo[1], oo[2], dd[0], dd[1], dd[2], a, origin[0], origin[1], origin[2]);
    const tor::BoxRay32 b = tor::make_box_ray32(r, bmax, hmin);
    const float* rec = &bnd32[8 * (size_t)i];
    keep[i] = (int32_t)(tor::slab_bit32(b, (f2v){rec[0], rec[1]}, (f2v){rec[2], rec[3]}, (f2v){rec[4], rec[5]}) | (r.wild & 1u));
    const double ix = 1.0 / dd[0], iy = 1.0 / dd[1], iz = 1.0 / dd[2];
    const double* c = &bnd[8 * (size_t)i];
    const double tx0 = (c[0] - oo[0]) * ix, tx1 = (c[3] - oo[0]) * ix;
    const double ty0 = (c[1] - oo[1]) * iy, ty1 = (c[4] - oo[1]) * iy;
    const double tz0 = (c[2] - oo[2]) * iz, tz1 = (c[5] - oo[2]) * iz;
    const double t_in = std::fmax(std::fmax(std::fmin(tx0, tx1), std::fmin(ty0, ty1)), std::fmax(std::fmin(tz0, tz1), 0.0));
    const double t_out = std::fmin(std::fmin(std::fmax(tx0, tx1), std::fmax(ty0, ty1)), std::fmax(tz0, tz1));
    need[i] = (t_in <= t_out) ? 1 : 0;
  }
  return TOR_OK;
}


int tor_selftest_math_host(int32_t op, const double* x, const double* y, double* out0, double* out1,
                           int64_t n) {
  if (!x || !out0 || n < 0) return fail(TOR_ERR_INVALID_ARGUMENT, "tor_selftest_math_host: bad argument");
  for (int64_t i = 0; i < n; ++i) {
    double a = 0, b = 0;
    tor::selftest_math_one(op, x[i], y ? y[i] : 0.0, a, b);
    out0[i] = a;
    if (out1) out1[i] = b;
  }
  return TOR_OK;
}

int tor_selftest_math_device(int32_t op, const double* x, const double* y, double* out0, double* out1,
                             int64_t n, int32_t device) {
  if (!x || !out0 || n < 0) return fail(TOR_ERR_INVALID_ARGUMENT, "tor_selftest_math_device: bad argument");
  int count = 0;
  hipError_t e = hipGetDeviceCount(&count);
  if (e != hipSuccess || count <= 0) return fail(TOR_ERR_NO_DEVICE, "no HIP device available");
  if (device >= 0) HIP_TRY(hipSetDevice(device));
  const size_t bytes = (size_t)n * 8;
  DeviceBuffer bx, by, b0, b1;
  struct Release {
    DeviceBuffer *a, *b, *c, *d;
    ~Release() { a->release(); b->release(); c->release(); d->release(); }
  } release{&bx, &by, &b0, &b1};
  HIP_TRY(bx.ensure(bytes + 8));
  HIP_TRY(by.ensure(bytes + 8));
  HIP_TRY(b0.ensure(bytes + 8));
  HIP_TRY(b1.ensure(bytes + 8));
  HIP_TRY(hipMemcpy(bx.ptr, x, bytes, hipMemcpyHostToDevice));
  if (y) HIP_TRY(hipMemcpy(by.ptr, y, bytes, hipMemcpyHostToDevice));
  else HIP_TRY(hipMemset(by.ptr, 0, bytes));
  HIP_TRY(hipMemset(b0.ptr, 0, bytes));
  HIP_TRY(hipMemset(b1.ptr, 0, bytes));
  HIP_TRY(tor::launch_selftest(op, (const double*)bx.ptr, (const double*)by.ptr, (double*)b0.ptr, (double*)b1.ptr, n, nullptr));
  HIP_TRY(hipDeviceSynchronize());
  HIP_TRY(hipMemcpy(out0, b0.ptr, bytes, hipMemcpyDeviceToHost));
  if (out1) HIP_TRY(hipMemcpy(out1, b1.ptr, bytes, hipMemcpyDeviceToHost));
  return TOR_OK;
}

int tor_selftest_rng_host(int32_t mode, uint64_t a, uint64_t b, uint64_t c, uint64_t state_out[4],
                          uint64_t* draws_out, int64_t n) {
  tor::Rng g{0, 0, 0, 0};
  if (mode == 1) tor::seed1(g, a);
  else if (mode == 2) tor::seed2(g, a, b);
  else if (mode == 3) tor::seed3(g, a, b, c);
  else return fail(TOR_ERR_INVALID_ARGUMENT, "tor_selftest_rng_host: mode must be 1, 2 or 3");
  if (state_out) { state_out[0] = g.s0; state_out[1] = g.s1; state_out[2] = g.s2; state_out[3] = g.s3; }
  for (int64_t i = 0; i < n && draws_out; ++i) draws_out[i] = tor::next(g);
  return TOR_OK;
}

}
```

trace-of-radiance_amd/csrc/tor_context.hpp:

```cpp
#pragma once

#include <hip/hip_runtime_api.h>

#include <cstdint>
#include <string>
#include <vector>

#include "../../include/tor_render.h"
#include "tor_filter32.hpp"
#include "tor_kernels.hpp"
#include "tor_scene.hpp"

namespace tor {

int fail(int code, const std::string& msg);
int fail_hip(hipError_t e, const char* what);
void set_last_note(const std::string& s);
const std::string& last_note();

#define HIP_TRY(expr)                                        \
  do {                                                       \
    hipError_t e__ = (expr);                                 \
    if (e__ != hipSuccess) return ::tor::fail_hip(e__, #expr); \
  } while (0)

struct DeviceBuffer {
  void* ptr = nullptr;
  size_t bytes = 0;
  hipError_t ensure(size_t n) {
    if (n <= bytes) return hipSuccess;
    if (ptr) (void)hipFree(ptr);
    ptr = nullptr;
    bytes = 0;
    hipError_t e = hipMalloc(&ptr, n);
    if (e == hipSuccess) bytes = n;
    return e;
  }
  void release() {
    if (ptr) (void)hipFree(ptr);
    ptr = nullptr;
    bytes = 0;
  }
};

struct PinnedBuffer {
  void* ptr = nullptr;
  size_t bytes = 0;
  hipError_t ensure(size_t n) {
    if (n <= bytes) return hipSuccess;
    if (ptr) (void)hipHostFree(ptr);
    ptr = nullptr;
    bytes = 0;
    hipError_t e = hipHostMalloc(&ptr, n, hipHostMallocDefault);
    if (e == hipSuccess) bytes = n;
    return e;
  }
  void release() {
    if (ptr) (void)hipHostFree(ptr);
    ptr = nullptr;
    bytes = 0;
  }
};

struct DeviceLayout {
  DeviceBuffer blob;
  const double *stat = nullptr, *mov = nullptr, *movy = nullptr, *segs = nullptr, *cold = nullptr;
  const float* hot32 = nullptr;
  const double* coop_trips = nullptr;
  const double *xhdr = nullptr, *xrec = nullptr, *xpl = nullptr;
  const float* xpl32 = nullptr;
  int n_segs = 0;
  int n_sorted = 0;
  int n_xrec = 0;
  bool has_f32 = false;
  hipError_t put(const HostLayout& lay, const std::vector<double>* cold_override = nullptr);
  void release() { blob.release(); }
};

struct DeviceAccel {
  DeviceLayout always;
  DeviceBuffer hot, grp, hot32;
  void release() { always.release(); hot.release(); grp.release(); hot32.release(); }
};

struct RcclComm;

struct HitQueryState {
  DeviceBuffer bnd;
  std::vector<double> bnd_host;
  int64_t bnd_scene = -1;
  uint64_t bnd_lo = 0, bnd_hi = 0;
  bool bnd_ok = false;
  double org[3] = {0.0, 0.0, 0.0};
  double reach2 = -1.0;
  double a_min = 0.0;
  DeviceBuffer io;
  DeviceBuffer head;
  DeviceBuffer obj_cold;
  std::vector<double> obj_cold_host;
  int64_t obj_scene = -1;
  DeviceBuffer sel;
  std::vector<uint32_t> groups;
  int64_t groups_gen = 0;
  DeviceBuffer grp[2];
  std::vector<uint32_t> grp_host[2];
  int64_t grp_scene[2] = {-1, -1}, grp_gen[2] = {-1, -1};
  DeviceBuffer absr[2];
  std::vector<double> absr_host[2];
  int64_t absr_scene[2] = {-1, -1};
  double pt_reach2 = -1.0;
  int64_t pt_scene = -1;
  uint64_t pt_lo = 0, pt_hi = 0;
  DeviceBuffer lights;
  int64_t n_lights = 0;
  double lights_total = 0.0;
  int64_t lights_last_pos = 0;
  DeviceBuffer env;
  int64_t env_n = 0;
  double env_total = 0.0;
  int32_t env_last_row = 0;
  hipEvent_t ev_done = nullptr;
  bool launched = false;
  void* stream = nullptr;
  ~HitQueryState();
};

}

struct TorContext {
  static constexpr int kRing = 64;
  static constexpr int kMigWord0 = 16;
  static constexpr int kSlotWords = kMigWord0 + tor::kMigWords;
  int device = 0;
  int num_cus = 0;
  std::vector<unsigned char> scene_bytes;
  int64_t n_objects = 0;
  bool scene_ready = false;
  int64_t n_uploads = 0, n_cache_hits = 0, n_layouts_built = 0;
  tor::DeviceLayout flat[2];
  bool flat_built[2] = {false, false};
  tor::F32Options f32;
  bool f32_built = false;
  tor::HostAccel accel[2];
  tor::DeviceAccel d_accel[2];
  bool accel_built[2] = {false, false};
  tor::DeviceBuffer bnd_ring;
  size_t bnd_slot_bytes = 0;
  tor::DeviceBuffer counters;
  tor::DeviceBuffer tile_order[kRing];
  tor::DeviceBuffer probe_buf;
  float hot_frac = 0.4f;
  int probe_spp = 2;
  int64_t last_probe_pixels = 0;
  int prio_shift = 16;
  tor::DeviceBuffer wave_log;
  tor::DeviceBuffer cam_ring;
  TorCamera cam_host[kRing];
  std::vector<double> bnd_host[kRing];
  std::vector<float> bnd32_host[kRing];
  std::vector<double> probe_bnd_host[kRing];
  std::vector<float> probe_bnd32_host[kRing];
  bool probe_accel = true;
  int plane_screen = 1;
  bool screen = true;
  hipEvent_t ev_start[kRing] = {}, ev_stop[kRing] = {};
  int64_t launches = 0;
  bool timing_valid = false;
  int64_t last_samples = 0;
  int64_t last_n_waves = 0;
  int last_slot = 0;
  bool collect_stats = false;
  tor::DeviceBuffer scratch;
  tor::DeviceBuffer slice;
  tor::DeviceBuffer gather;
  tor::DeviceBuffer frame;
  tor::DeviceBuffer noise;
  tor::DeviceBuffer adapt;
  tor::PinnedBuffer staging;
  std::vector<hipEvent_t> chunk_events;
  hipEvent_t ev_call[2] = {};
  void* last_stream = nullptr;
  bool last_stream_valid = false;
  hipStream_t stream = nullptr;
  tor::RcclComm* comm = nullptr;
  int max_blocks_per_cu[2][2] = {{3, 3}, {3, 3}};
  int lpt_min_spp = 32;
  int waves_override = 0;
  long long coop_max_pixels = 114688;
  float split_frac = -1.0f;
  long long split_min_pixels = 16384, split_max_pixels = 100000000;
  hipStream_t stream2 = nullptr;
  hipEvent_t ev_fork[kRing] = {}, ev_join[kRing] = {};
  int mig_mode = 1;
  float srv_frac = 0.07f, srv_min_frac = 0.005f, push_theta = 3.0f, chain_theta = 3.5f, floor_theta = 1.33f;
  int srv_patience_us = 8000;
  int key_mode = 1;
  int mig_tail_lanes = 8;
  int mig_tail_rest = 256;
  unsigned mig_flags = (8u << 8) | 2u | 4u;
  tor::DeviceBuffer mig_rec, mig_flag;
  double mig_stall_s = 60.0;
  int64_t n_stalled_frames = 0;
  bool last_split = false;
  bool last_migrate = false;
  int32_t last_variant[5] = {-1, -1, -1, -1, -1};
  tor::HitQueryState hitq;
};

namespace tor {

struct AccumLaunch {
  int first_sample;
  double* moments;
  const int32_t* list = nullptr;
  int32_t n_list = 0;
  unsigned long long* rng = nullptr;
};

bool valid_options(const TorOptions* opt, TorOptions& o, bool for_drop_in);
const std::string& options_why();

int ensure_layouts(TorContext* ctx, int accel);

// ... 14 lines not shown
```

trace-of-radiance_amd/csrc/tor_kernels.hpp:

```cpp
#pragma once

#include <hip/hip_runtime_api.h>

#include <cstdint>

#include "tor_device.hpp"
#include "tor_filter32.hpp"

namespace tor {

constexpr int kThreads = 256;
constexpr int kPad = 8;
#ifdef TOR_BOX_FANOUT
constexpr int kBoxFanout = TOR_BOX_FANOUT;
#else
constexpr int kBoxFanout = 1;
#endif

struct KParams {
  const double* stat;
  const double* mov;
  const double* movy;
  const double* segs;
  const double* cold;
  const double* xrec;
  int xrec_lds_doubles;
  const double* xhdr;
  const double* xpl;
  const float* xpl32;
  double plane_gate2;
  const float* hot32;
  double org[3];
  const double* bnd;
  const double* shot;
  int shot_stride;
  int shot_lds_doubles;
  const double* sgrp;
  const float* shot32;
  int shot32_stride;
  int shot32_block_stride;
  int shot32_lds_floats;
  float sp_mc0max, sp_dcmax;
  int two_level;
  double box_org[3];
  double box_reach2;
  double box_amin;
  const float* bnd32;
  float sp_bmax;
  float sp_hmin;
  int bnd32_lds_floats;
  double sp_t0, sp_dt;
  int spatial_base;
  int n_super;
  int n_segs;
  int nrows, ncols, spp, max_depth;
  double inv_spp, inv_ncols, inv_row_tile;
  int shard_index, shard_count, row_tile;
  unsigned chunk;
  unsigned n_waves;
  unsigned n_pixels;
  const unsigned* order;
  unsigned* pixel_cost;
  unsigned long long* sched;
  int prio_shift;
  unsigned long long total_work;
  unsigned long long* work_counter;
  double* out;
  unsigned long long* stats;
  unsigned long long* wave_log;
  const double* cam_dev;
  int n_cold_slots, coop_slots;
  const unsigned long long* split;
  const double* coop_trips;
  unsigned long long* mig;
  unsigned long long* mig_rec;
  unsigned* mig_flag;
  unsigned mig_cap;
  int mig_tail_lanes;
  int mig_tail_rest;
  unsigned mig_patience;
  unsigned long long mig_stall_ticks;
  unsigned mig_flags;
  int screen;
  int n_boxes;
  int first_sample;
  double* mom;
  const int32_t* pixel_list;
  unsigned long long* rstate;
};

enum : int {
  kMigHead = 0,
  kMigTail = 16,
  kMigLaneWaves = 32,
  kMigSrvWgs = 48,
  kMigPush = 49,
  kMigPushFloor = 50,
  kMigServed = 64,
  kMigHotPushes = 65,
  kMigTailPushes = 66,
  kMigT0 = 67,
  kMigTLaneEnd = 68,
  kMigTHotDone = 69,
  kMigTTailDone = 70,
  kMigItsHot = 71,
  kMigItsTail = 72,
  kMigTCounterDry = 73,
  kMigConverted = 74,
  kMigProgress = 75,
  kMigStalled = 95,
  kMigPushNow = 80,
  kMigWords = 96
};

hipError_t launch_integrate(const KParams& p, int seeding, int arith, int waves_per_simd, int blocks,
                            hipStream_t stream);
int integrate_blocks_per_cu(const KParams& p, int seeding, int arith, int waves_per_simd);
size_t coop_lds_bytes(int coop_slots);
int coop_blocks_per_cu(const KParams& p, int arith);
hipError_t launch_coop(const KParams& p, int arith, int blocks, hipStream_t stream);
int integrate_fixed_lds_bytes(int blocks, int f32, int seeding = 0);
hipError_t launch_probe(const KParams& p, int blocks, hipStream_t stream);
struct MigSchedule {
  unsigned long long* mig = nullptr;
  float lavg_scale = 0.f, srv_frac = 0.f, srv_min_frac = 0.f, push_theta = 0.f;
  float chain_scale = 0.f, chain_theta = 0.f, floor_theta = 0.f;
  int blocks = 0, spp = 0, max_depth = 0;
  int key_mode = 0, probe_spp = 2;
};
hipError_t launch_tile_order(const unsigned* pixel_cost, unsigned n_pixels, unsigned* key, unsigned* work, unsigned* order, int n_tiles,
                             float split_frac, unsigned long long* split_out, unsigned long long* lane_counter,
                             float hot_chain, unsigned long long* sched, const MigSchedule& mig, hipStream_t stream);
void integrate_variant_key(const KParams& p, int seeding, int arith, int waves_per_simd, int32_t out[5]);
bool integrate_variant_serves_chains(const KParams& p, int seeding);
constexpr int kTilePixelsHost = 64;
constexpr size_t kTileSortScratchBytes = 4096 * (8 + 4 + 4) + 16;
hipError_t launch_finalize(double* pixels, long long n_values, double scale, double gamma, hipStream_t stream);
hipError_t launch_resolve(const double* sums, double* pixels, long long n_values, double scale, double gamma, hipStream_t stream);
constexpr int kNoiseMaxBlocks = 1024;
hipError_t launch_accum_noise(const double* sums, const double* moments, long long npix, double n, double* err, double* partials,
                              double* out2, hipStream_t stream);
size_t adaptive_select_scratch_bytes(long long n_in);
hipError_t launch_adaptive_select(const double* sums, const double* moments, const int32_t* list_in, long long n_in, double n, double abs_tol,
                                  double rel_tol, int32_t* list_out, int32_t* counts, void* scratch, int32_t* n_out_dev, hipStream_t stream);
hipError_t launch_resolve_counts(const double* sums, const int32_t* counts, double* pixels, long long n_values, double gamma, hipStream_t stream);
hipError_t launch_quantize(const double* pixels, long long n_values, uint8_t* out, hipStream_t stream);
hipError_t launch_encode_ipcm(const double* pixels, int nrows, int ncols, uint8_t* out, uint8_t* plane_y,
                              uint8_t* plane_cb, uint8_t* plane_cr, hipStream_t stream);
hipError_t launch_gather_rows(const double* gathered, double* frame, int nrows, int ncols, int row_tile, int shard_count,
                              long long shard_stride, hipStream_t stream);
hipError_t launch_spin_until(volatile unsigned* flag, unsigned long long max_ticks, hipStream_t stream);
hipError_t launch_selftest(int op, const double* x, const double* y, double* out0, double* out1, long long n,
                           hipStream_t stream);

TOR_HD void selftest_math_one(int op, double x, double y, double& out0, double& out1) {
  switch (op) {
    case 0: sincos_2pi(x, out0, out1); break;
    case 1: out0 = pow5(x); break;
    case 2: out0 = pow_pos(x, y); break;
    case 3: out0 = __builtin_sqrt(x); break;
    case 4: out0 = x / y; break;
    case 5: out0 = quantize36(x); break;
    case 6: {
      V3 u = unit_vector(v3(x, y, 0.5));
      out0 = dot(u, v3(1.0, 2.0, 3.0));
      out1 = u.x;
      break;
    }
    default: out0 = x; break;
  }
}

}
```

trace-of-radiance_amd/csrc/tor_knobs.hpp:

```cpp
#pragma once

#include <cstdlib>
#include <cstring>

namespace tor {

struct Knob {
  const char* name;
  const char* dflt;
  const char* range;
  const char* when;
  const char* what;
};

constexpr Knob kKnobs[] = {
    {"TOR_DEFAULT_ACCEL", "3", "0..3", "call", "TOR_ACCEL_* bits tor_render() runs with (3 = block culling + float32 pre-filter, both exact); 0 = the reference's float64 brute force"},
    {"TOR_DEFAULT_SEEDING", "pixel", "pixel | sample", "call", "random streams of tor_render(): the reference's one stream per pixel (render.nim:59-67) or the counter-based per-sample streams (TOR_SEED_SAMPLE: the mode that shards a frame over 8 GPUs)"},
    {"TOR_DEVICES", "(current device)", "all | comma list of HIP ordinals", "call", "device list of tor_render(): row shards on several GPUs, framebuffer gather inside the library"},
    {"TOR_GATHER", "auto", "auto | rccl | peer | host", "call", "how the row shards of a device list reach the canvas (TorOptions.gather)"},
    {"TOR_RCCL_TIMEOUT_MS", "10000 + 1 per MB", "> 0", "call", "deadline of one RCCL framebuffer transfer; past it the communicators are aborted and TOR_GATHER=auto carries on with peer copies"},
    {"TOR_RCCL_INIT_TIMEOUT_MS", "120000", "> 0", "call", "deadline of communicator creation + self-check (runs in a helper thread that is abandoned when it does not return)"},
    {"TOR_FAULT_INJECT", "(none)", "comma list of rccl_init | rccl_xfer | rccl_hang | peer", "call", "TEST: the named gather leg fails (or, rccl_hang, never completes) at that point"},
    {"TOR_BLOCKS_PER_CU", "3", "1..8", "context", "workgroups per CU of integrate_kernel (all modes)"},
    {"TOR_WAVES_PER_SIMD", "(from the launch shape)", "2 | 3", "context", "force the register-budget variant of integrate_kernel (256 / 168 VGPRs)"},
    {"TOR_ACCEL_ORDER", "sah", "sah | morton", "upload", "order of the objects behind TOR_ACCEL_BLOCKS' boxes: top-down surface-area build (round 6) or the Morton curve of rounds 1-5 (A/B; same canvas)"},
    {"TOR_STAGE_LDS", "(no cap)", "bytes, 0 = off", "call", "cap of the LDS staging of block records / boxes (TOR_ACCEL_BLOCKS)"},
    {"TOR_SCREEN", "1", "0 | 1", "context", "0: strict brute-force launches evaluate the reference's unfused discriminant for every object instead of the conservative FMA screen (same canvas)"},
    {"TOR_PLANE", "1", "0 | 1 | 2", "context", "stage one of the FMA screen (the 4-instruction plane screen in front of the segment's wave-uniform test, per-lane stage two on what it keeps): 0 off, 1 on the segments where it pays (default), 2 on every segment (same candidates, same canvas)"},
    {"TOR_COOP_MAX_PIXELS", "114688", ">= 0", "context", "frames up to this many pixels (per device) run one WAVE per pixel when neither hand-off nor split mode applies; 0 = never"},
    {"TOR_LPT_MIN_SPP", "32", ">= 0", "context", "cost probe + chain-length-ordered tile schedule from this many spp on; 0 = never"},
    {"TOR_HOT_FRAC", "0.4", ">= 0", "context", "a pixel chain is HOT (arbiter priority 3) from this share of an average wave's iterations; 0 = off"},
    {"TOR_PRIO_SHIFT", "16", "0..31", "context", "arbiter-priority rotation period, log2 shader-clock ticks; 0 = off"},
    {"TOR_MIGRATE", "1", "0 | 1", "context", "0: no chain hand-off (split mode / wave-per-pixel kernel instead)"},
    {"TOR_SRV_FRAC", "0.07", "0..1", "context", "share of the workgroups that start as servers when the frame can hold a chain above the threshold's floor"},
    {"TOR_SRV_MIN_FRAC", "0.005", "0..1", "context", "... otherwise"},
    {"TOR_SRV_PATIENCE_US", "8000", ">= 0", "context", "a dedicated server without a chain for this long becomes a lane wave; 0 = never"},
    {"TOR_SRV_STALL_S", "60", "seconds; 0 = never; < 0 = at once (TEST)", "call", "a WAITING server that sees no progress of the frame for this long flags the frame incomplete and leaves (launch not fully resident); the blocking entry points render it again without the hand-off"},
    {"TOR_PUSH_THETA", "3.0", "> 0", "context", "first push threshold, x the bounce iterations of an average lane"},
    {"TOR_FLOOR_THETA", "1.33", "> 0", "context", "floor of the adaptive push threshold, same unit"},
    {"TOR_CHAIN_THETA", "3.5", "> 0", "context", "... and never below this x the frame's mean chain"},
    {"TOR_TAIL_LANES", "8", "-2..64", "context", "an exhausted wave hands its chains over from this many live lanes down; -1 nobody pushes in the tail; -2 nobody serves (debug)"},
    {"TOR_TAIL_REST", "256", ">= 0", "context", "... with more live lanes: only chains with at least this many bounce iterations to go"},
    {"TOR_MIG_FLAGS", "0x806", "bit mask", "context", "bit 0 acquire polling, bit 1 adaptive threshold, bit 2 tail chains served at priority 1, bits 8-15 longest back-off (naps), bits 16-31 cap of waiting servers"},
};

constexpr int kKnobCount = (int)(sizeof(kKnobs) / sizeof(kKnobs[0]));

inline const char* knob(const char* name) {
  for (int i = 0; i < kKnobCount; ++i)
    if (std::strcmp(kKnobs[i].name, name) == 0) return std::getenv(name);
  return nullptr;
}

}
```

trace-of-radiance_amd/csrc/tor_scene.cpp:

```cpp
#include "tor_scene.hpp"
#include "tor_knobs.hpp"

#include <algorithm>
#include <cmath>
#include <cstdlib>
#include <cstring>
#include <utility>

#include "tor_filter32.hpp"
#include "tor_kernels.hpp"
#include "tor_screen.hpp"

namespace tor {

namespace {

inline double i64_as_double(int64_t v) {
  double d;
  std::memcpy(&d, &v, 8);
  return d;
}

size_t padded(size_t c) { return (c + kPad - 1) / kPad * kPad; }

bool fill_material(double* c, const TorMaterial& m, int moving) {
  int64_t flags = (moving ? 1 : 0) | ((int64_t)m.kind << 8);
  c[13] = i64_as_double(flags);
  switch (m.kind) {
    case TOR_LAMBERTIAN:
      c[9] = m.u.lambertian.albedo.x; c[10] = m.u.lambertian.albedo.y; c[11] = m.u.lambertian.albedo.z;
      return true;
    case TOR_METAL:
      c[9] = m.u.metal.albedo.x; c[10] = m.u.metal.albedo.y; c[11] = m.u.metal.albedo.z;
      c[12] = m.u.metal.fuzz;
      return true;
    case TOR_DIELECTRIC: {
      const double ri = m.u.dielectric.refraction_index;
      c[12] = ri;
      const double inv = 1.0 / ri;
      double r0f = (1.0 - inv) / (1.0 + inv);
      double r0b = (1.0 - ri) / (1.0 + ri);
      c[9] = inv;
      c[10] = r0f * r0f;
      c[11] = r0b * r0b;
      return true;
    }
    default:
      return false;
  }
}

bool fill_cold(double* c, const TorHittableVariant& h, int64_t orig) {
  if (h.kind == TOR_SPHERE) {
    const TorSphere& s = h.u.sphere;
    c[0] = s.center.x; c[1] = s.center.y; c[2] = s.center.z;
    c[6] = 1.0 / s.radius;
    c[14] = i64_as_double(orig);
    c[15] = s.radius * s.radius;
    return fill_material(c, s.material, 0);
  }
  const TorMovingSphere& s = h.u.moving_sphere;
  c[0] = s.center0.x; c[1] = s.center0.y; c[2] = s.center0.z;
  c[3] = s.center1.x - s.center0.x; c[4] = s.center1.y - s.center0.y; c[5] = s.center1.z - s.center0.z;
  c[6] = 1.0 / s.radius;
  c[7] = s.time0; c[8] = s.time1 - s.time0;
  c[14] = i64_as_double(orig);
  c[15] = s.radius * s.radius;
  return fill_material(c, s.material, 1);
}

}

namespace {

struct TimeGroup {
  uint64_t k0, k1;
  std::vector<int64_t> ids;
};

void add_to_group(std::vector<TimeGroup>& groups, const TorMovingSphere& s, int64_t i) {
  uint64_t k0, k1;
  std::memcpy(&k0, &s.time0, 8);
  std::memcpy(&k1, &s.time1, 8);
  for (auto& g : groups)
    if (g.k0 == k0 && g.k1 == k1) {
      g.ids.push_back(i);
      return;
    }
  groups.push_back({k0, k1, {i}});
}

bool group_moves_along_y_only(const TorHittableVariant* objs, const TimeGroup& g) {
  for (int64_t idx : g.ids) {
    const TorMovingSphere& s = objs[idx].u.moving_sphere;
    if (!(s.center1.x - s.center0.x == 0.0 && s.center1.z - s.center0.z == 0.0)) return false;
  }
  return true;
}

double norm3(double x, double y, double z) { return std::sqrt(x * x + y * y + z * z); }

}

F32Options f32_options_for(const TorHittableVariant* objs, int64_t n) {
  F32Options o;
  std::vector<double> ax[3];
  for (int64_t i = 0; i < n; ++i) {
    const TorVec3* c = objs[i].kind == TOR_SPHERE ? &objs[i].u.sphere.center
                       : (objs[i].kind == TOR_MOVING_SPHERE ? &objs[i].u.moving_sphere.center0 : nullptr);
    if (!c || !std::isfinite(c->x) || !std::isfinite(c->y) || !std::isfinite(c->z)) continue;
    ax[0].push_back(c->x); ax[1].push_back(c->y); ax[2].push_back(c->z);
  }
  if (ax[0].empty()) return o;
  const size_t mid = ax[0].size() / 2;
  for (int a = 0; a < 3; ++a) {
    std::vector<double> t = ax[a];
    std::nth_element(t.begin(), t.begin() + mid, t.end());
    o.origin[a] = t[mid];
  }
  std::vector<double> dist(ax[0].size());
  for (size_t k = 0; k < dist.size(); ++k)
    dist[k] = norm3(ax[0][k] - o.origin[0], ax[1][k] - o.origin[1], ax[2][k] - o.origin[2]);
  std::nth_element(dist.begin(), dist.begin() + mid, dist.end());
  o.far_limit = 8.0 * dist[mid];
  if (!(o.far_limit > 0.0) || !std::isfinite(o.far_limit)) o.far_limit = 0.0;
  return o;
}

bool build_layout(const TorHittableVariant* objs, const std::vector<int64_t>& ids, HostLayout& out, std::string& err,
                  const F32Options* f32) {
  std::vector<int64_t> statics, statics32;
  std::vector<TimeGroup> groups, groups32;
  auto dist0 = [&](const TorVec3& c) {
    return norm3(c.x - f32->origin[0], c.y - f32->origin[1], c.z - f32->origin[2]);
  };
  for (int64_t i : ids) {
    const TorHittableVariant& h = objs[i];
    if (h.kind == TOR_SPHERE) {
      const TorSphere& s = h.u.sphere;
      const bool q = f32 && f32_eligible(dist0(s.center), 0.0, s.radius * s.radius) && dist0(s.center) <= f32->far_limit;
      (q ? statics32 : statics).push_back(i);
    } else if (h.kind == TOR_MOVING_SPHERE) {
      const TorMovingSphere& s = h.u.moving_sphere;
      const double dt = s.time1 - s.time0;
      const bool q = f32 && std::isfinite(s.time0) && std::isfinite(dt) && dt != 0.0 &&
                     f32_eligible(dist0(s.center0), norm3(s.center1.x - s.center0.x, s.center1.y - s.center0.y, s.center1.z - s.center0.z),
                                  s.radius * s.radius) &&
                     dist0(s.center0) <= f32->far_limit;
      add_to_group(q ? groups32 : groups, s, i);
    } else {
      err = "unknown HittableVariant kind";
      return false;
    }
  }
  struct Seg64 { int kind; std::vector<int64_t> ids; double t0, dt; int xkind; double y; };
  std::vector<Seg64> segs64;
  auto y_of = [&](int64_t i) { return objs[i].kind == TOR_SPHERE ? objs[i].u.sphere.center.y : objs[i].u.moving_sphere.center0.y; };
  auto r2_of = [&](int64_t i) {
    const double r = objs[i].kind == TOR_SPHERE ? objs[i].u.sphere.radius : objs[i].u.moving_sphere.radius;
    return r * r;
  };
  auto cut_by_y = [&](const std::vector<int64_t>& all_members, int kind, double t0, double dt, int xkind_rest, int xkind_uniform) {
    std::vector<int64_t> members, big;
    if (all_members.size() >= 2 * (size_t)kPad) {
      std::vector<double> r2s;
      for (int64_t i : all_members) r2s.push_back(r2_of(i));
      std::nth_element(r2s.begin(), r2s.begin() + r2s.size() / 2, r2s.end());
      const double limit = 16.0 * r2s[r2s.size() / 2];
      for (int64_t i : all_members) (r2_of(i) > limit ? big : members).push_back(i);
    } else {
      members = all_members;
    }
    const size_t big_at = segs64.size();
    if (!big.empty()) segs64.push_back({kind, big, t0, dt, xkind_rest, 0.0});
    if (members.empty()) return;
    std::vector<std::pair<uint64_t, std::vector<int64_t>>> by_y;
    for (int64_t i : members) {
      const double y = y_of(i);
      uint64_t b;
      std::memcpy(&b, &y, 8);
      bool found = false;
      for (auto& g : by_y)
        if (g.first == b) { g.second.push_back(i); found = true; break; }
      if (!found) by_y.push_back({b, {i}});
      if (by_y.size() > 64) break;
    }
    std::vector<int64_t> rest;
    std::vector<Seg64> uniform;
    if (by_y.size() <= 64 && xkind_uniform != 0) {
      for (auto& g : by_y)
        if (g.second.size() >= (size_t)kPad && std::isfinite(y_of(g.second[0]))) uniform.push_back({kind, g.second, t0, dt, xkind_uniform, y_of(g.second[0])});
      for (int64_t i : members) {
        const double y = y_of(i);
        bool in_uniform = false;
        for (const Seg64& u : uniform) {
          uint64_t a, b;
          std::memcpy(&a, &y, 8); std::memcpy(&b, &u.y, 8);
          if (a == b) { in_uniform = true; break; }
        }
        if (!in_uniform) rest.push_back(i);
      }
    } else {
      rest = members;
    }
    if (!rest.empty() && !big.empty() && rest.size() + big.size() < 48) {
      segs64[big_at].ids.insert(segs64[big_at].ids.end(), rest.begin(), rest.end());
      rest.clear();
    }
    if (!rest.empty()) segs64.push_back({kind, rest, t0, dt, xkind_rest, 0.0});
    for (Seg64& u : uniform) segs64.push_back(std::move(u));
  };
  if (!statics.empty()) cut_by_y(statics, 0, 0.0, 1.0, 10, 11);
  for (size_t gi = 0; gi < groups.size(); ++gi) {
    const TorMovingSphere& first = objs[groups[gi].ids[0]].u.moving_sphere;
    const double t0 = first.time0, dt = first.time1 - first.time0;
    const bool sane = std::isfinite(t0) && std::isfinite(dt) && dt != 0.0;
    TimeGroup gy{groups[gi].k0, groups[gi].k1, {}}, gg{groups[gi].k0, groups[gi].k1, {}};
    for (int64_t idx : groups[gi].ids) {
      const TorMovingSphere& s = objs[idx].u.moving_sphere;
      ((s.center1.x - s.center0.x == 0.0 && s.center1.z - s.center0.z == 0.0) ? gy : gg).ids.push_back(idx);
    }
    if (!gy.ids.empty()) cut_by_y(gy.ids, 1, t0, dt, sane ? 14 : 0, sane ? 12 : 0);
    if (!gg.ids.empty()) cut_by_y(gg.ids, 2, t0, dt, sane ? 13 : 0, 0);
  }
  for (size_t a = 0; a < segs64.size(); ++a) {
    if (!(segs64[a].kind == 0 && segs64[a].xkind == 11)) continue;
    for (size_t b = 0; b < segs64.size(); ++b) {
      Seg64& mv = segs64[b];
      if (!(mv.kind == 1 && mv.xkind == 12)) continue;
      uint64_t ya, yb;
      std::memcpy(&ya, &segs64[a].y, 8); std::memcpy(&yb, &mv.y, 8);
      if (ya != yb) continue;
      double ra = 0.0, rb = 0.0;
      for (int64_t i : segs64[a].ids) ra = std::fmax(ra, r2_of(i));
      for (int64_t i : mv.ids) rb = std::fmax(rb, r2_of(i));
      if (!(ra <= 4.0 * rb && rb <= 4.0 * ra)) continue;
      mv.ids.insert(mv.ids.end(), segs64[a].ids.begin(), segs64[a].ids.end());
      segs64.erase(segs64.begin() + (long)a);
      --a;
      break;
    }
  }
  std::stable_sort(segs64.begin(), segs64.end(), [](const Seg64& a, const Seg64& b) { return a.ids.size() > b.ids.size(); });
  auto as_mover = [&](int64_t idx) {
    if (objs[idx].kind == TOR_MOVING_SPHERE) return objs[idx].u.moving_sphere;
    TorMovingSphere m{};
    m.center0 = m.center1 = objs[idx].u.sphere.center;
    m.radius = objs[idx].u.sphere.radius;
    m.material = objs[idx].u.sphere.material;
    return m;
  };
  auto xs_of = [](int xkind) { return xkind == 0 ? 0 : (xkind >= 13 ? 8 : 4); };
  auto pw_of = [](int xkind) { return xkind == 0 ? 0 : (xkind == 13 ? 4 : 2); };
  auto slots_of = [&](const Seg64& sg, bool words) {
    size_t c = padded(sg.ids.size());
    if (words && sg.xkind >= 10 && sg.ids.size() >= 48 && c % 32 > 16) c = (c + 31) / 32 * 32;
    return c;
  };
  bool pad_words = true;
  {
    size_t t0 = 0, t1 = 0;
    for (const Seg64& sg : segs64) { t0 += slots_of(sg, false); t1 += slots_of(sg, true); }
    if ((t1 + 511) / 512 > (t0 + 511) / 512) pad_words = false;
  }
  size_t n_stat_p = 0, n_mov_p = 0, n_movy_p = 0, n_xrec = 0, n_xpl = 0;
  for (const Seg64& sg : segs64) {
    const size_t cp = slots_of(sg, pad_words);
    (sg.kind == 0 ? n_stat_p : (sg.kind == 1 ? n_movy_p : n_mov_p)) += cp;
    n_xrec += cp * (size_t)xs_of(sg.xkind);
    n_xpl += cp * (size_t)pw_of(sg.xkind);
  }
  std::vector<char> yonly32(groups32.size(), 0);
  size_t n32_slots = padded(statics32.size()), n32_floats = padded(statics32.size()) / 2 * 10;
  for (size_t gi = 0; gi < groups32.size(); ++gi) {
    const bool y = group_moves_along_y_only(objs, groups32[gi]);
    yonly32[gi] = y ? 1 : 0;
    n32_slots += padded(groups32[gi].ids.size());
    n32_floats += padded(groups32[gi].ids.size()) / 2 * (y ? 12 : 16);
  }
  out.n_sorted = n_stat_p + n_mov_p + n_movy_p + n32_slots;
  out.stat.assign(4 * n_stat_p + 8, 0.0);
  out.mov.assign(8 * n_mov_p + 8, 0.0);
  out.movy.assign(6 * n_movy_p + 8, 0.0);
  out.xrec.assign(n_xrec + 8, 0.0);
  out.xpl.assign(n_xpl + 8, 1e300);
  out.xpl32.assign(n_xpl + 16, kPlane32PadX);
  for (size_t k = 1; k < out.xpl32.size(); k += 2) out.xpl32[k] = kPlane32PadZ;
  out.xpl32seg.clear();
  out.hot32.assign(n32_floats + 32, 0.0f);
  out.cold.assign(16 * out.n_sorted + 16, 0.0);
  out.segs.clear();
  out.xsegs.clear();
  for (size_t k = 0; k < n_stat_p; ++k) out.stat[4 * k + 3] = -1.0;
  for (size_t k = 0; k < n_mov_p; ++k) out.mov[8 * k + 3] = -1.0;
  for (size_t k = 0; k < n_movy_p; ++k) out.movy[6 * k + 3] = -1.0;
  for (size_t k = 0; k < out.n_sorted; ++k) out.cold[16 * k + 15] = -1.0;

  auto up = [](double x) { return x * (1.0 + 0x1p-40); };
  size_t sorted = 0, stat_rec = 0, mov_rec = 0, movy_rec = 0, x_off = 0, pl_off = 0;
  for (const Seg64& sg : segs64) {
    const size_t cnt_p = slots_of(sg, pad_words);
    double reach = 0.0, travel = 0.0, rmax2 = 0.0;
    double xlo = INFINITY, xhi = -INFINITY, zlo = INFINITY, zhi = -INFINITY, dcx_max = 0.0, dcz_max = 0.0;
    auto grow = [&](double x, double z) {
      if (std::isfinite(x)) { xlo = std::fmin(xlo, x); xhi = std::fmax(xhi, x); }
      if (std::isfinite(z)) { zlo = std::fmin(zlo, z); zhi = std::fmax(zhi, z); }
    };
    for (int64_t idx : sg.ids) {
      if (sg.kind == 0) {
        const TorSphere& s = objs[idx].u.sphere;
        reach = std::fmax(reach, norm3(s.center.x, s.center.y, s.center.z) + std::fabs(s.radius));
        rmax2 = std::fmax(rmax2, s.radius * s.radius);
        grow(s.center.x, s.center.z);
      } else {
        const TorMovingSphere s = as_mover(idx);
        reach = std::fmax(reach, norm3(s.center0.x, s.center0.y, s.center0.z) + std::fabs(s.radius));
        rmax2 = std::fmax(rmax2, s.radius * s.radius);
        travel = std::fmax(travel, norm3(s.center1.x - s.center0.x, s.center1.y - s.center0.y, s.center1.z - s.center0.z));
        grow(s.center0.x, s.center0.z);
        dcx_max = std::fmax(dcx_max, std::fabs(s.center1.x - s.center0.x));
        dcz_max = std::fmax(dcz_max, std::fabs(s.center1.z - s.center0.z));
      }
    }
    const double ext_x = xhi >= xlo ? (xhi - xlo) + dcx_max : 0.0, ext_z = zhi >= zlo ? (zhi - zlo) + dcz_max : 0.0;
    const size_t first_rec = sg.kind == 0 ? stat_rec : (sg.kind == 1 ? movy_rec : mov_rec);
    out.segs.insert(out.segs.end(), {(double)sg.kind, (double)first_rec, (double)(cnt_p | ((cnt_p - sg.ids.size()) << 24)), (double)(sorted / kPad),
                                     sg.kind == 0 ? 0.0 : sg.t0, sg.kind == 0 ? 0.0 : sg.dt, up(reach), up(travel)});
    out.xsegs.insert(out.xsegs.end(), {(double)sg.xkind, (double)x_off, sg.y, (double)pl_off, rmax2, ext_x, ext_z, 0.0});
    double e32 = 0.0, cm32 = 0.0;
    const bool pl32 = sg.xkind >= 10 && sg.xkind != 13;
    const double orx = pl32 && xhi >= xlo ? 0.5 * xlo + 0.5 * xhi : 0.0, orz = pl32 && zhi >= zlo ? 0.5 * zlo + 0.5 * zhi : 0.0;
    for (size_t k = 0; k < sg.ids.size() && pl32; ++k) {
      const TorMovingSphere s = as_mover(sg.ids[k]);
      const float fx = plane32_offset(s.center0.x, orx, e32), fz = plane32_offset(s.center0.z, orz, e32);
      out.xpl32[pl_off + 2 * k] = fx; out.xpl32[pl_off + 2 * k + 1] = fz;
      cm32 = std::fmax(cm32, std::fmax(std::fabs((double)fx), std::fabs((double)fz)));
    }
    out.xpl32seg.insert(out.xpl32seg.end(), {orx, orz, e32, cm32});
    const size_t xs = (size_t)xs_of(sg.xkind), pw = (size_t)pw_of(sg.xkind);
    for (size_t k = 0; k < cnt_p && xs != 0; ++k) {
      double* x = &out.xrec[x_off + xs * k];
      if (xs == 4) x[sg.xkind == 10 ? 3 : 2] = 1e300;
      else x[3] = -1.0;
    }
    for (size_t k = 0; k < cnt_p && pw == 4; ++k) {
      double* pl = &out.xpl[pl_off + 4 * k];
      pl[2] = 0.0; pl[3] = 0.0;
    }
    for (size_t k = 0; k < sg.ids.size(); ++k) {
      const TorHittableVariant& hv = objs[sg.ids[k]];
      if (sg.kind == 0) {
        const TorSphere& s = hv.u.sphere;
        double* m = &out.stat[4 * (stat_rec + k)];
        m[0] = s.center.x; m[1] = s.center.y; m[2] = s.center.z;
        m[3] = s.radius * s.radius;
        double* x = &out.xrec[x_off + 4 * k];
        if (sg.xkind == 10) { x[0] = s.center.x; x[1] = s.center.y; x[2] = s.center.z; x[3] = screen2_K(s.center.x, s.center.y, s.center.z, s.radius * s.radius); }
        else { x[0] = s.center.x; x[1] = s.center.z; x[2] = screen2_Ky(s.center.x, s.center.z, s.radius * s.radius); x[3] = 0.0; }
        out.xpl[pl_off + 2 * k] = s.center.x; out.xpl[pl_off + 2 * k + 1] = s.center.z;
      } else {
        const TorMovingSphere s = as_mover(sg.ids[k]);
        const double dcx = s.center1.x - s.center0.x, dcy = s.center1.y - s.center0.y, dcz = s.center1.z - s.center0.z;
        if (sg.kind == 1) {
          double* m = &out.movy[6 * (movy_rec + k)];
          m[0] = s.center0.x; m[1] = s.center0.y; m[2] = s.center0.z;
          m[3] = s.radius * s.radius;
          m[4] = dcy;
          if (sg.xkind == 12) {
            double* x = &out.xrec[x_off + 4 * k];
            x[0] = s.center0.x; x[1] = s.center0.z; x[2] = screen2_Ky(s.center0.x, s.center0.z, s.radius * s.radius);
            x[3] = dcy;
          }
          if (sg.xkind != 0) { out.xpl[pl_off + 2 * k] = s.center0.x; out.xpl[pl_off + 2 * k + 1] = s.center0.z; }
        } else {
          double* m = &out.mov[8 * (mov_rec + k)];
          m[0] = s.center0.x; m[1] = s.center0.y; m[2] = s.center0.z;
          m[3] = s.radius * s.radius;
          m[4] = dcx; m[5] = dcy; m[6] = dcz;
          if (sg.xkind == 13) {
            double* pl = &out.xpl[pl_off + 4 * k];
            pl[0] = s.center0.x; pl[1] = s.center0.z; pl[2] = dcx; pl[3] = dcz;
          }
        }
        if (sg.xkind >= 13) {
          double* x = &out.xrec[x_off + 8 * k];
          x[0] = s.center0.x; x[1] = s.center0.y; x[2] = s.center0.z; x[3] = s.radius * s.radius;
          x[4] = dcx; x[5] = dcy; x[6] = dcz; x[7] = 0.0;
        }
      }
      if (!fill_cold(&out.cold[16 * (sorted + k)], hv, sg.ids[k])) { err = "unknown Material kind"; return false; }
    }
    (sg.kind == 0 ? stat_rec : (sg.kind == 1 ? movy_rec : mov_rec)) += cnt_p;
    x_off += cnt_p * xs;
    pl_off += cnt_p * pw;
    sorted += cnt_p;
  }

  size_t f_off = 0;
  auto emit32 = [&](const std::vector<int64_t>& members, int kind, double t0, double dt) -> bool {
    const int stride = kind == 5 ? 10 : (kind == 6 ? 12 : 16);
    const size_t cnt_p = padded(members.size());
    double mc0max = 0.0, dcmax = 0.0;
    for (size_t k = 0; k < cnt_p; ++k) {
      float* rec = &out.hot32[f_off + (k / 2) * (size_t)stride];
      const int h = (int)(k & 1);
      if (k >= members.size()) {
        rec[6 + h] = kF32PadR2;
        continue;
      }
      const TorHittableVariant& hv = objs[members[k]];
      const bool moving = hv.kind == TOR_MOVING_SPHERE;
      const TorVec3& c0 = moving ? hv.u.moving_sphere.center0 : hv.u.sphere.center;
      const double r = moving ? hv.u.moving_sphere.radius : hv.u.sphere.radius;
      const double q[3] = {c0.x - f32->origin[0], c0.y - f32->origin[1], c0.z - f32->origin[2]};
      const double mc0 = norm3(q[0], q[1], q[2]);
      rec[0 + h] = (float)q[0]; rec[2 + h] = (float)q[1]; rec[4 + h] = (float)q[2];
      rec[6 + h] = (float)(r * r);
      rec[8 + h] = f32_object_k(mc0, r * r, moving);
      mc0max = std::max(mc0max, mc0);
      if (moving) {
        const TorMovingSphere& s = hv.u.moving_sphere;
        const double dc[3] = {s.center1.x - s.center0.x, s.center1.y - s.center0.y, s.center1.z - s.center0.z};
        dcmax = std::max(dcmax, norm3(dc[0], dc[1], dc[2]));
        if (kind == 6) {
          rec[10 + h] = (float)dc[1];
        } else {
          rec[10 + h] = (float)dc[0]; rec[12 + h] = (float)dc[1]; rec[14 + h] = (float)dc[2];
        }
      }
      if (!fill_cold(&out.cold[16 * (sorted + k)], hv, members[k])) { err = "unknown Material kind"; return false; }
    }
    out.segs.insert(out.segs.end(), {(double)kind, (double)f_off, (double)cnt_p, (double)(sorted / kPad), t0, dt,
                                     (double)f32_round_up(mc0max * 1.000001), (double)f32_round_up(dcmax * 1.000001)});
    out.xsegs.insert(out.xsegs.end(), 8, 0.0);
    out.xpl32seg.insert(out.xpl32seg.end(), 4, 0.0);
    f_off += cnt_p / 2 * (size_t)stride;
    sorted += cnt_p;
    return true;
  };
  if (!statics32.empty() && !emit32(statics32, 5, 0.0, 1.0)) return false;
  for (size_t gi = 0; gi < groups32.size(); ++gi) {
    const TorMovingSphere& first = objs[groups32[gi].ids[0]].u.moving_sphere;
    if (!emit32(groups32[gi].ids, yonly32[gi] ? 6 : 7, first.time0, first.time1 - first.time0)) return false;
  }
  out.n_segs = (int)(out.segs.size() / 8);
  if (out.segs.empty()) out.segs.assign(8, 0.0);
  if (out.xsegs.empty()) out.xsegs.assign(8, 0.0);
  out.xhdr.assign(16 * (size_t)std::max(out.n_segs, 1) + 16, 0.0);
  for (int s = 0; s < out.n_segs; ++s) {
    const double* sg = &out.segs[8 * (size_t)s];
    const double* xs = &out.xsegs[8 * (size_t)s];
    double* h = &out.xhdr[16 * (size_t)s];
    int32_t gate = 0;
    const int n_real = ((int)sg[2] & 0xffffff) - ((int)sg[2] >> 24);
    if ((int)xs[0] >= 10 && n_real >= 48) {
      const double band = 2.0 * kPlaneGate * std::sqrt(xs[4]);
      const double e_min = std::fmin(xs[5], xs[6]), e_max = std::hypot(xs[5], xs[6]);
      gate = band < e_min ? 1 : (band < e_max ? 2 : 0);
    }
    const int32_t ints[8] = {(int32_t)xs[0], (int32_t)sg[0], (int32_t)sg[2], (int32_t)sg[3], (int32_t)sg[1], (int32_t)xs[1], (int32_t)xs[3], gate};
    std::memcpy(h, ints, sizeof(ints));
    h[4] = sg[4]; h[5] = sg[5]; h[6] = sg[6]; h[7] = sg[7];
    h[8] = xs[2]; h[9] = xs[4]; h[10] = xs[5]; h[11] = xs[6];
    const int xkind = (int)xs[0];
    if (xkind == 13) {
      for (size_t k = 0; k < 4; ++k) h[12 + k] = out.xpl[(size_t)xs[3] + k];
    } else if (xkind >= 10) {
      const double* o32 = &out.xpl32seg[4 * (size_t)s];
      std::memcpy(&h[12], &out.xpl32[(size_t)xs[3]], 8);
      h[13] = o32[0]; h[14] = o32[1];
      const float ec[2] = {o32[2] < 0x1p126 ? f32_up(o32[2]) : INFINITY, o32[3] < 0x1p126 ? f32_up(o32[3]) : INFINITY};
      std::memcpy(&h[15], ec, 8);
    }
  }
  const size_t n_trips = (out.n_sorted + 63) / 64;
  out.coop_trips.assign(4 * n_trips + 4, 0.0);
  for (size_t t = 0; t < n_trips; ++t) {
    bool any_mover = false, any_static = false, y_only = true, same_group = true, sane = true;
    uint64_t g0 = 0, g1 = 0;
    double t0 = 0.0, dt = 1.0;
    for (size_t k = 64 * t; k < 64 * (t + 1); ++k) {
      if (k >= out.n_sorted) { any_static = true; continue; }
      const double* cr = &out.cold[16 * k];
      int64_t flags;
      std::memcpy(&flags, &cr[13], 8);
      if (!(flags & 1)) { any_static = true; continue; }
      uint64_t b0, b1;
      std::memcpy(&b0, &cr[7], 8); std::memcpy(&b1, &cr[8], 8);
      if (!any_mover) { g0 = b0; g1 = b1; t0 = cr[7]; dt = cr[8]; }
      else if (b0 != g0 || b1 != g1) same_group = false;
      any_mover = true;
      if (!(cr[3] == 0.0 && cr[5] == 0.0)) y_only = false;
      if (!std::isfinite(cr[7]) || !std::isfinite(cr[8]) || cr[8] == 0.0) sane = false;
    }
    double kind = 3.0;
    if (!any_mover) kind = 0.0;
    else if (!any_static && same_group && sane) kind = y_only ? 1.0 : 2.0;
    out.coop_trips[4 * t + 0] = kind;
    out.coop_trips[4 * t + 1] = t0;
    out.coop_trips[4 * t + 2] = dt;
  }
  return true;
}

namespace {

constexpr size_t kTwoLevelMinBlocks = 96;

uint32_t spread10(uint32_t v) {
  v &= 0x3ff;
  v = (v | (v << 16)) & 0x030000FF;
  v = (v | (v << 8)) & 0x0300F00F;
  v = (v | (v << 4)) & 0x030C30C3;
  v = (v | (v << 2)) & 0x09249249;
  return v;
}

bool finite3(const TorVec3& v) { return std::isfinite(v.x) && std::isfinite(v.y) && std::isfinite(v.z); }

}

void build_accel(const TorHittableVariant* objs, int64_t n, HostAccel& out, const F32Options* f32) {
  out = HostAccel{};
  if (n < 64) return;
  std::vector<double> radii;
  radii.reserve((size_t)n);
  for (int64_t i = 0; i < n; ++i) {
    const double r = objs[i].kind == TOR_SPHERE ? objs[i].u.sphere.radius : objs[i].u.moving_sphere.radius;
    radii.push_back(std::fabs(r));
  }
  std::vector<double> tmp = radii;
  std::nth_element(tmp.begin(), tmp.begin() + tmp.size() / 2, tmp.end());
  const double median_r = tmp[tmp.size() / 2];
  std::vector<int64_t> always, spatial;
  for (int64_t i = 0; i < n; ++i) {
    bool ok = std::isfinite(radii[(size_t)i]) && radii[(size_t)i] <= 2.5 * median_r;
    if (objs[i].kind == TOR_SPHERE) {
      ok = ok && finite3(objs[i].u.sphere.center);
    } else if (objs[i].kind == TOR_MOVING_SPHERE) {
      const TorMovingSphere& s = objs[i].u.moving_sphere;
      const double dt = s.time1 - s.time0;
      ok = ok && finite3(s.center0) && finite3(s.center1) && std::isfinite(s.time0) && std::isfinite(dt) && dt != 0.0;
    } else {
      return;
    }
    (ok ? spatial : always).push_back(i);
  }
  if (spatial.size() < 32) return;
  std::string err;
  if (!build_layout(objs, always, out.always, err, f32)) return;
  std::vector<std::pair<uint32_t, int64_t>> keyed;
  keyed.reserve(spatial.size());
  const char* order_knob = knob("TOR_ACCEL_ORDER");
  const bool use_morton = order_knob && std::strcmp(order_knob, "morton") == 0;
  if (use_morton) {
    double lo[3] = {1e300, 1e300, 1e300}, hi[3] = {-1e300, -1e300, -1e300};
    auto c0 = [&](int64_t i, int a) {
      const TorVec3& c = objs[i].kind == TOR_SPHERE ? objs[i].u.sphere.center : objs[i].u.moving_sphere.center0;
      return a == 0 ? c.x : (a == 1 ? c.y : c.z);
    };
    for (int64_t i : spatial)
      for (int a = 0; a < 3; ++a) { lo[a] = std::min(lo[a], c0(i, a)); hi[a] = std::max(hi[a], c0(i, a)); }
    double ext = 1e-300;
    for (int a = 0; a < 3; ++a) ext = std::max(ext, hi[a] - lo[a]);
    for (int64_t i : spatial) {
      uint32_t q[3];
      for (int a = 0; a < 3; ++a) q[a] = (uint32_t)std::min(1023.0, std::max(0.0, (c0(i, a) - lo[a]) / ext * 1023.0));
      keyed.push_back({spread10(q[0]) | (spread10(q[2]) << 1) | (spread10(q[1]) << 2), i});
    }
    std::stable_sort(keyed.begin(), keyed.end());
  } else {
    const size_t ns = spatial.size();
    const bool second_level = ((ns + kPad - 1) / kPad + (size_t)kBoxFanout - 1) / (size_t)kBoxFanout > kTwoLevelMinBlocks;
    struct Hull { double lo[3], hi[3], mid[3]; };
    std::vector<Hull> hull(ns);
    for (size_t k = 0; k < ns; ++k) {
      const TorHittableVariant& ob = objs[spatial[k]];
      const bool mv = ob.kind == TOR_MOVING_SPHERE;
      const TorVec3& a0 = mv ? ob.u.moving_sphere.center0 : ob.u.sphere.center;
      const TorVec3& a1 = mv ? ob.u.moving_sphere.center1 : ob.u.sphere.center;
      const double r = radii[(size_t)spatial[k]];
      const double p0[3] = {a0.x, a0.y, a0.z}, p1[3] = {a1.x, a1.y, a1.z};
      for (int a = 0; a < 3; ++a) {
        hull[k].lo[a] = std::min(p0[a], p1[a]) - r;
        hull[k].hi[a] = std::max(p0[a], p1[a]) + r;
        hull[k].mid[a] = 0.5 * (p0[a] + p1[a]);
      }
    }
    std::vector<uint32_t> ord(ns), best_ord, cand;
    for (size_t k = 0; k < ns; ++k) ord[k] = (uint32_t)k;
    std::vector<double> suffix;
    auto half_area = [](const double lo[3], const double hi[3]) {
      const double dx = hi[0] - lo[0], dy = hi[1] - lo[1], dz = hi[2] - lo[2];
      return dx * dy + dy * dz + dx * dz;
    };
    std::vector<std::pair<size_t, size_t>> todo{{0, ns}};
    while (!todo.empty()) {
      const auto [b, e] = todo.back();
      todo.pop_back();
      const size_t n_here = e - b;
      if (n_here <= (size_t)kPad) continue;
      const size_t box_objs = (size_t)kPad * (size_t)kBoxFanout;
      const size_t unit = (second_level && n_here > box_objs * kPad) ? box_objs * kPad : (n_here > box_objs ? box_objs : (size_t)kPad);
      double best_cost = INFINITY;
      size_t best_pos = (n_here / 2 + unit - 1) / unit * unit;
      if (best_pos >= n_here) best_pos = (n_here - 1) / unit * unit;
      bool have = false;
      for (int ax = 0; ax < 3; ++ax) {
        cand.assign(ord.begin() + (long)b, ord.begin() + (long)e);
        std::stable_sort(cand.begin(), cand.end(), [&](uint32_t x, uint32_t y) { return hull[x].mid[ax] < hull[y].mid[ax]; });
        suffix.assign(n_here + 1, 0.0);
        double lo[3] = {INFINITY, INFINITY, INFINITY}, hi[3] = {-INFINITY, -INFINITY, -INFINITY};
// ... 245 lines not shown
```

trace-of-radiance_amd/csrc/tor_scene.hpp:

```cpp
#pragma once

#include <cstdint>
#include <string>
#include <vector>

#include "../../include/tor_render.h"

namespace tor {

struct HostLayout {
  std::vector<double> stat, mov, movy, segs, cold;
  std::vector<double> xsegs, xrec;
  std::vector<double> xhdr;
  std::vector<double> xpl;
  std::vector<float> xpl32;
  std::vector<double> xpl32seg;
  std::vector<float> hot32;
  int n_segs = 0;
  size_t n_sorted = 0;
  std::vector<double> coop_trips;
};

struct F32Options {
  double origin[3] = {0.0, 0.0, 0.0};
  double far_limit = 0.0;
};
F32Options f32_options_for(const TorHittableVariant* objs, int64_t n);

bool build_layout(const TorHittableVariant* objs, const std::vector<int64_t>& ids, HostLayout& out, std::string& err,
                  const F32Options* f32 = nullptr);

struct HostAccel {
  bool available = false;
  HostLayout always;
  std::vector<double> cold;
  std::vector<double> hot;
  int hot_stride = 8;
  std::vector<double> groups;
  size_t spatial_base = 0;
  size_t n_blocks = 0;
  int fanout = 1;
  size_t n_boxes = 0;
  bool two_level = false;
  struct Obj { double c0[3], dc[3], t0, dt, abs_r; bool moving, valid; };
  std::vector<Obj> spatial;
  bool sp32 = false;
  std::vector<float> hot32;
  int hot32_stride = 10;
  int hot32_block_stride = 40;
  double sp_t0 = 0.0, sp_dt = 1.0;
  float sp_mc0max = 0.0f, sp_dcmax = 0.0f;
};

void build_accel(const TorHittableVariant* objs, int64_t n, HostAccel& out, const F32Options* f32 = nullptr);

bool compute_block_bounds(const HostAccel& acc, double t_lo, double t_hi, std::vector<double>& bnd);
inline size_t accel_boxes_padded(const HostAccel& acc) { return (acc.n_boxes + 7) / 8 * 8; }

void block_reach(const HostAccel& acc, const std::vector<double>& bnd, double org[3], double* reach2, double* a_min);

float block_bounds_f32(const std::vector<double>& bnd, const double origin[3], std::vector<float>& bnd32, float* hmin_out);

}
```

trace-of-radiance_amd/csrc/tor_screen.hpp:

```cpp
#pragma once
#include "tor_math.hpp"

namespace tor {

#if defined(TOR_SCREEN_MUTATE) && TOR_SCREEN_MUTATE == 1
#define TOR_MARGIN(x) 0.0
#else
#define TOR_MARGIN(x) (x)
#endif
TOR_HD void screen_margins(double B, double d1, double a, double& negmu, double& am) {
  negmu = TOR_MARGIN(-(B * d1) * 0x1p-48);
  am = TOR_MARGIN(a * ((B * B) * 0x1p-45));
}
TOR_HD int screen_filter(double ocx, double ocy, double ocz, double dx, double dy, double dz, double a, double negmu,
                         double am, double r2) {
  const double hb = fma_(ocz, dz, fma_(ocy, dy, fma_(ocx, dx, negmu)));
  const double cc = fma_(ocz, ocz, fma_(ocy, ocy, fma_(ocx, ocx, -r2)));
  const double t = fma_(-a, cc, am);
  const double disc = fma_(hb, hb, t);
  const unsigned h = (unsigned)(double_to_bits(hb) >> 32), y = (unsigned)(double_to_bits(t) >> 32), z = (unsigned)(double_to_bits(disc) >> 32);
#if defined(__HIP_DEVICE_COMPILE__) && __has_builtin(__builtin_amdgcn_bitop3_b32)
  return (int)__builtin_amdgcn_bitop3_b32(h, y, z, 0x51);
#else
  return (int)((h | ~y) & ~z);
// ... 44 lines not shown
}
TOR_HD ScreenSeg screen2_seg(const ScreenRay& r, double reach, double travel, double y_rel, double f) {
  ScreenSeg s;
  const double B = r.s1 + reach + travel * __builtin_fabs(f);
  const double mu = TOR_MARGIN(B * 0x1p-47);
  const double M = TOR_MARGIN((B * B) * 0x1p-45);
  const bool wild = r.wild || !((B * B) * 0x1p-45 < __builtin_inf()) || !(f * f < __builtin_inf());
  uint64_t e = (double_to_bits(B) >> 52) & 0x7ffu;
  if (e < 3u) e = 3u;
  if (e > 0x7fbu) e = 0x7fbu;
  const double sg = bits_to_double((uint64_t)(0x7fcu - e) << 52), sg2 = sg * sg;
  const double oy = r.oy - y_rel;
  const double dnx = wild ? 0.0 : r.dnx, dny = wild ? 0.0 : r.dny, dnz = wild ? 0.0 : r.dnz;
  s.hx = sg * dnx; s.hy = sg * dny; s.hz = sg * dnz;
  const double P = fma_(oy, dny, fma_(r.oz, dnz, r.ox * dnx)) - mu;
  const double Q = fma_(oy, oy, fma_(r.oz, r.oz, r.ox * r.ox));
  s.Pn = wild ? 0.0 : -(sg * P);
  s.Tn = wild ? -__builtin_inf() : -(sg2 * (M - Q));
  const double n2 = wild ? 0.0 : -(sg2 + sg2);
  s.a2x = n2 * r.ox; s.a2y = n2 * oy; s.a2z = n2 * r.oz;
  s.ks = wild ? 0.0 : sg2;
  const double fw = wild ? 0.0 : f;
  s.fdy = fw * s.hy;
  s.gn = fw * s.a2y;
  s.f2n = sg2 * (fw * fw);
  return s;
}
TOR_HD int screen2_word(double nh, double tn) {
  const double q = fma_(-nh, nh, tn);
  return (int)(unsigned)(double_to_bits(q) >> 32);
}
template <bool kLane = false>
TOR_HD int screen2_static(const ScreenSeg& s, double cx, double cy, double cz, double K) {
  const double nh = kLane ? fma_clamp_v(cx, s.hx, fma_(cy, s.hy, fma_(cz, s.hz, s.Pn))) : fma_clamp_s(cx, s.hx, fma_(cy, s.hy, fma_(cz, s.hz, s.Pn)));
  const double tn = fma_(s.ks, K, fma_(s.a2x, cx, fma_(s.a2y, cy, fma_(s.a2z, cz, s.Tn))));
  return screen2_word(nh, tn);
}
template <bool kLane = false>
TOR_HD int screen2_static_y(const ScreenSeg& s, double cx, double cz, double K) {
  const double nh = kLane ? fma_clamp_v(cx, s.hx, fma_(cz, s.hz, s.Pn)) : fma_clamp_s(cx, s.hx, fma_(cz, s.hz, s.Pn));
  const double tn = fma_(s.ks, K, fma_(s.a2x, cx, fma_(s.a2z, cz, s.Tn)));
  return screen2_word(nh, tn);
}
template <bool kLane = false>
TOR_HD int screen2_movy_y(const ScreenSeg& s, double cx, double cz, double K, double dcy) {
  const double nh = kLane ? fma_clamp_v(dcy, s.fdy, fma_(cx, s.hx, fma_(cz, s.hz, s.Pn))) : fma_clamp_s(dcy, s.fdy, fma_(cx, s.hx, fma_(cz, s.hz, s.Pn)));
  const double w = fma_(s.f2n, dcy, s.gn);
  const double tn = fma_(s.ks, K, fma_(w, dcy, fma_(s.a2x, cx, fma_(s.a2z, cz, s.Tn))));
  return screen2_word(nh, tn);
}
TOR_HD double screen2_clampK(double k) { return __builtin_fmin(__builtin_fmax(k, -0x1.fffffffffffffp1023), 0x1.fffffffffffffp1023); }
TOR_HD double screen2_K(double cx, double cy, double cz, double r2) { return screen2_clampK(((cx * cx + cy * cy) + cz * cz) - r2); }
TOR_HD double screen2_Ky(double cx, double cz, double r2) { return screen2_clampK((cx * cx + cz * cz) - r2); }

struct PlaneRay {
  double nx, nz;
  double w2;
  bool all;
};
struct PlaneSeg {
  double nx, nz;
  double c0;
  double negthr;
  double fnx, fnz;
};
TOR_HD PlaneRay plane_ray(const ScreenRay& r) {
  PlaneRay pr;
  pr.nx = -r.dnz;
  pr.nz = r.dnx;
  pr.w2 = fma_(r.dnz, r.dnz, r.dnx * r.dnx);
  pr.all = r.wild || !(pr.w2 >= 0x1p-200);
  return pr;
}
TOR_HD PlaneSeg plane_seg(const ScreenRay& r, const PlaneRay& pr, double reach, double travel, double f, double rmax2) {
  PlaneSeg s;
  const double B = r.s1 + reach + travel * __builtin_fabs(f);
#if defined(TOR_SCREEN_MUTATE) && TOR_SCREEN_MUTATE <= 2
  const double M = 0.0;
  const double thr = rmax2 * pr.w2;
#else
  const double M = (B * B) * 0x1p-45;
  const double thr = (fma_(rmax2, 0x1p-40, rmax2) + M) * pr.w2;
#endif
  const bool all = pr.all || !(thr >= 0x1p-900 && thr < __builtin_inf());
  s.nx = all ? 0.0 : pr.nx;
  s.nz = all ? 0.0 : pr.nz;
  s.c0 = all ? 0.0 : -fma_(s.nx, r.ox, s.nz * r.oz);
  s.negthr = all ? -__builtin_inf() : -thr;
  s.fnx = all ? 0.0 : f * s.nx;
  s.fnz = all ? 0.0 : f * s.nz;
  return s;
}
TOR_HD int plane_word(const PlaneSeg& s, double cx, double cz) {
  const double v = fma_(s.nx, cx, fma_(s.nz, cz, s.c0));
  const double q = fma_(v, v, s.negthr);
  return (int)(unsigned)(double_to_bits(q) >> 32);
}
TOR_HD int plane_word_mov(const PlaneSeg& s, double c0x, double c0z, double dcx, double dcz) {
  const double v = fma_(s.nx, c0x, fma_(s.nz, c0z, fma_(s.fnx, dcx, fma_(s.fnz, dcz, s.c0))));
  const double q = fma_(v, v, s.negthr);
  return (int)(unsigned)(double_to_bits(q) >> 32);
}
constexpr float kPlane32PadX = 0x1p100f, kPlane32PadZ = 0x1.3c6ef3p99f;
constexpr double kPlane32Clamp = 0x1p100;
struct PlaneSeg32 {
  float nx, nz;
  float c0;
  float T;
};
TOR_HD float f32_up(double x) {
  float f = (float)x;
  if ((double)f < x) f = __builtin_bit_cast(float, __builtin_bit_cast(uint32_t, f) + 1u);
  return f;
}
TOR_HD PlaneSeg32 plane_seg32(const ScreenRay& r, const PlaneSeg& ps, double orx, double orz, double e32, double cm) {
  PlaneSeg32 s;
  const double ox = r.ox - orx, oz = r.oz - orz;
  const double co = __builtin_fabs(ox) + __builtin_fabs(oz);
  const double n1 = __builtin_fabs(ps.nx) + __builtin_fabs(ps.nz);
  const double thr = -ps.negthr;
  const float nx = (float)ps.nx, nz = (float)ps.nz;
  const double c0 = -fma_((double)nx, ox, (double)nz * oz);
#if defined(TOR_SCREEN_MUTATE) && TOR_SCREEN_MUTATE == 3
  (void)n1;
  const double T = __builtin_sqrt(thr);
  const float tf = (float)T;
#else
  const double T = (fma_(0x1p-20, __builtin_sqrt(thr) + n1 * e32, __builtin_sqrt(thr) + n1 * e32) +
                    fma_(n1, 0x1p-21, 0x1p-140) * ((cm + co) + e32) + 0x1p-140) * (1.0 + 0x1p-40);
  const float tf = T < 0x1p126 ? f32_up(T) : __builtin_inff();
#endif
  const bool all = !(ps.negthr > -__builtin_inf()) || !(cm <= 0x1p60 && co <= 0x1p60 && e32 <= 0x1p60) || !(tf < __builtin_inff());
  s.nx = all ? 0.0f : nx;
  s.nz = all ? 0.0f : nz;
  s.c0 = all ? 0.0f : (float)c0;
  s.T = all ? __builtin_inff() : tf;
  return s;
}
TOR_HD int plane_word32(const PlaneSeg32& s, float cx, float cz) {
  const float v = __builtin_fmaf(s.nx, cx, __builtin_fmaf(s.nz, cz, s.c0));
  const float q = __builtin_fabsf(v) - s.T;
  return (int)__builtin_bit_cast(uint32_t, q);
}
TOR_HD float plane32_offset(double c, double o, double& err_io) {
  const double d = c - o;
  const double bb = d - c, t = (c - (d - bb)) + (-o - bb);
  const double dc = __builtin_fmin(__builtin_fmax(d, -kPlane32Clamp), kPlane32Clamp);
  const float f = (float)dc;
  const double e = __builtin_fabs((d - (double)f) + t) * (1.0 + 0x1p-50);
  err_io = !(e < __builtin_inf()) ? __builtin_inf() : __builtin_fmax(err_io, e);
  return f;
}

constexpr double kPlaneGate = 16.0;
TOR_HD bool plane_pays(const PlaneRay& pr, double gate2, double rmax2, double sx, double sz) {
  const double e = fma_(__builtin_fabs(pr.nx), sx, __builtin_fabs(pr.nz) * sz);
  return !pr.all && (gate2 * rmax2) * pr.w2 < e * e;
}

}
```

Before: 3914.

## Add per-word conservative plane cull of 32-object words behind stage-one plane screen

Builds a per-32-slot bounding box table (xz center/half-extent) plus per-segment y-range data at layout time, uploads it, and in the f32 plane-screen loop computes a per-ray cull interval along the ray's perpendicular so whole words whose boxes fall outside are zeroed before the per-lane stage. The goal is to drop candidate masks that stage one would otherwise keep, cutting downstream intersection work. It adds four float loads and a few FMAs per word plus per-segment setup, and adds debug host entry points and a TOR_PLANE=3 mode that disables the cull.

```diff
diff --git a/include/tor_plane_cull.h b/include/tor_plane_cull.h
--- /dev/null
+++ b/include/tor_plane_cull.h
@@ -0,0 +1,21 @@
+#ifndef TOR_PLANE_CULL_H
+#define TOR_PLANE_CULL_H
+
+#ifndef TOR_RENDER_H
+#include "tor_render.h"
+#endif
+
+#ifdef __cplusplus
+extern "C" {
+#endif
+
+TOR_API int tor_debug_plane_cull_scene(TorHittableList world, int64_t n_rays, const double* o, const double* d, const double* time,
+                                       int8_t* culled, int32_t* words_kept);
+TOR_API int tor_debug_plane_cull_layout(TorHittableList world, int64_t max_slots, int32_t* slot_object, double* word_box,
+                                        int64_t* n_slots_out);
+
+#ifdef __cplusplus
+}
+#endif
+
+#endif
diff --git a/include/tor_render.h b/include/tor_render.h
--- a/include/tor_render.h
+++ b/include/tor_render.h
@@ -375,4 +375,6 @@
 
 #include "tor_bsdf.h"
 
+#include "tor_plane_cull.h"
+
 #endif
diff --git a/trace-of-radiance_amd/__init__.py b/trace-of-radiance_amd/__init__.py
--- a/trace-of-radiance_amd/__init__.py
+++ b/trace-of-radiance_amd/__init__.py
@@ -149,6 +149,7 @@
 ENV_MAX_SIDE = 2048
 CAMERA_SYMBOLS = ["tor_camera_connect_device", "tor_camera_connect_host", "tor_light_emit_device", "tor_light_emit_host"]
 BSDF_SYMBOLS = ["tor_bsdf_eval_device", "tor_bsdf_eval_host"]
+PLANE_CULL_SYMBOLS = ["tor_debug_plane_cull_scene", "tor_debug_plane_cull_layout"]
 BSDF_NONE, BSDF_DENSITY, BSDF_DELTA = 0, 1, 2
 HIT_AUTO, HIT_BRUTE, HIT_BLOCKS = 0, 1, 2
 HIT_MODES = {"auto": HIT_AUTO, "brute": HIT_BRUTE, "blocks": HIT_BLOCKS}
@@ -208,6 +209,7 @@
     _bind_env(L, skip_missing=bool(ab))
     _bind_camera(L, skip_missing=bool(ab))
     _bind_bsdf(L, skip_missing=bool(ab))
+    _bind_plane_cull(L, skip_missing=bool(ab))
     _lib = L
     return L
 
@@ -406,6 +408,16 @@
         if skip_missing and not hasattr(L, name):
             continue
         getattr(L, name).argtypes = _BSDF_SIGNATURES[name]
+
+
+def _bind_plane_cull(L, skip_missing=False) -> None:
+    dp = C.POINTER(C.c_double)
+    sigs = {"tor_debug_plane_cull_scene": [HittableList, C.c_int64, dp, dp, dp, C.POINTER(C.c_int8), C.POINTER(C.c_int32)],
+            "tor_debug_plane_cull_layout": [HittableList, C.c_int64, C.POINTER(C.c_int32), dp, C.POINTER(C.c_int64)]}
+    for name in PLANE_CULL_SYMBOLS:
+        if skip_missing and not hasattr(L, name):
+            continue
+        getattr(L, name).argtypes = sigs[name]
 
 
 def _check(rc: int) -> None:
@@ -2512,6 +2524,27 @@
     return keep, pad_kept, int(n_pad.value)
 
 
+def debug_plane_cull_scene(world: HittableList, o, d, time):
+    dp = lambda x: np.ascontiguousarray(x, dtype=np.float64)
+    o, d, time = dp(o), dp(d), dp(time)
+    culled = np.zeros((len(time), int(world.len)), dtype=np.int8)
+    words_kept = np.zeros(len(time), dtype=np.int32)
+    P = C.POINTER(C.c_double)
+    _check(lib().tor_debug_plane_cull_scene(world, len(time), o.ctypes.data_as(P), d.ctypes.data_as(P), time.ctypes.data_as(P),
+                                            culled.ctypes.data_as(C.POINTER(C.c_int8)), words_kept.ctypes.data_as(C.POINTER(C.c_int32))))
+    return culled, words_kept
+
+
+def debug_plane_cull_layout(world: HittableList):
+    n = C.c_int64(0)
+    _check(lib().tor_debug_plane_cull_layout(world, 0, None, None, C.byref(n)))
+    slots = np.full(int(n.value), -1, dtype=np.int32)
+    boxes = np.zeros(((int(n.value) + 31) // 32, 6), dtype=np.float64)
+    _check(lib().tor_debug_plane_cull_layout(world, len(slots), slots.ctypes.data_as(C.POINTER(C.c_int32)),
+                                             boxes.ctypes.data_as(C.POINTER(C.c_double)), C.byref(n)))
+    return slots, boxes
+
+
 def selftest_math(op: int, x: np.ndarray, y: np.ndarray | None = None, where: str = "device", device: int = -1):
     x = np.ascontiguousarray(x, dtype=np.float64)
     yy = np.ascontiguousarray(y, dtype=np.float64) if y is not None else None
diff --git a/trace-of-radiance_amd/csrc/kernel/integrate_loop_plane.inc b/trace-of-radiance_amd/csrc/kernel/integrate_loop_plane.inc
--- a/trace-of-radiance_amd/csrc/kernel/integrate_loop_plane.inc
+++ b/trace-of-radiance_amd/csrc/kernel/integrate_loop_plane.inc
@@ -16,9 +16,19 @@
                 using RecPtr = std::conditional_t<PW == 2, cfptr, cdptr>;
                 RecPtr rec = (RecPtr)(uintptr_t)(PW == 2 ? (const void*)p.xpl32 : (const void*)p.xpl) + ((long)pl_first + PW * (long)i);
                 PlaneSeg32 ps32{};
+                PlaneCull pc{0.0f, __builtin_inff()};
+                cfptr box = nullptr;
+                int box_step = 0;
                 Rec n0, n1, n2 = 0, n3 = 0;
                 if constexpr (PW == 2) {
                   ps32 = plane_seg32(sray, ps, h_r1, h_r2, (double)__int_as_float(__double2loint(h_r3)), (double)__int_as_float(__double2hiint(h_r3)));
+                  box = (cfptr)(uintptr_t)p.xpl32 + (long)pl_first;
+                  if (p.xbox != nullptr) {
+                    const cfptr sr = (cfptr)(uintptr_t)p.xbox + 8 * (long)seg;
+                    pc = plane_cull_seg(sray, ps32, h_r1, h_r2, __int_as_float(__double2hiint(h_r3)), SEG_REACH, SEG_TRAVEL, f, sr[4], sr[0], sr[1], sr[2], sr[3]);
+                    box = (cfptr)(uintptr_t)p.xbox + 8 * (long)p.n_segs;
+                    box_step = 4;
+                  }
                   n0 = __int_as_float(__double2loint(h_r0)); n1 = __int_as_float(__double2hiint(h_r0));
                 } else {
                   n0 = h_r0; n1 = h_r1; n2 = h_r2; n3 = h_r3;
@@ -67,11 +77,16 @@
                   nw = nw < kQCap - w_count ? nw : kQCap - w_count;
                   unsigned m = 0;
                   int w = 0;
+                  cfptr bx = box;
+                  if constexpr (PW == 2) bx += (long)box_step * (long)(gb >> 2);
                   auto word = [&]() {
                     m = 0;
+                    float b0 = 0.0f, b1 = 0.0f, b2 = 0.0f, b3 = 0.0f;
+                    if constexpr (PW == 2) { b0 = bx[0]; b1 = bx[1]; b2 = bx[2]; b3 = bx[3]; bx += box_step; }
 #pragma unroll
                     for (int j = 0; j < 4 * kBlock; ++j) m = one(m, j);
                     rec += PW * 4 * kBlock;
+                    if constexpr (PW == 2) m = plane_cull_word(ps32, pc, b0, b1, b2, b3) ? 0u : m;
                     q[(unsigned)(w_count + w) * 64] = m;
                     nz = push_cond(nz, m != 0u);
                     w += 1;
diff --git a/trace-of-radiance_amd/csrc/tor_api.cpp b/trace-of-radiance_amd/csrc/tor_api.cpp
--- a/trace-of-radiance_amd/csrc/tor_api.cpp
+++ b/trace-of-radiance_amd/csrc/tor_api.cpp
@@ -57,12 +57,13 @@
 hipError_t DeviceLayout::put(const HostLayout& lay, const std::vector<double>* cold_override) {
   const std::vector<double>& c = cold_override ? *cold_override : lay.cold;
   struct Part { const void* src; size_t bytes; size_t off; };
-  Part parts[11] = {{lay.stat.data(), lay.stat.size() * 8, 0}, {lay.mov.data(), lay.mov.size() * 8, 0},
+  Part parts[12] = {{lay.stat.data(), lay.stat.size() * 8, 0}, {lay.mov.data(), lay.mov.size() * 8, 0},
                    {lay.movy.data(), lay.movy.size() * 8, 0}, {lay.segs.data(), lay.segs.size() * 8, 0},
                    {c.data(), c.size() * 8, 0},               {lay.hot32.data(), lay.hot32.size() * 4, 0},
                    {lay.coop_trips.data(), lay.coop_trips.size() * 8, 0},
                    {lay.xhdr.data(), lay.xhdr.size() * 8, 0}, {lay.xrec.data(), lay.xrec.size() * 8, 0},
-                    {lay.xpl.data(), lay.xpl.size() * 8, 0}, {lay.xpl32.data(), lay.xpl32.size() * 4, 0}};
+                    {lay.xpl.data(), lay.xpl.size() * 8, 0}, {lay.xpl32.data(), lay.xpl32.size() * 4, 0},
+                    {lay.xbox.data(), lay.xbox.size() * 4, 0}};
   size_t total = 0;
   for (Part& p : parts) {
     p.off = total;
@@ -85,6 +86,7 @@
   xrec = (const double*)(b + parts[8].off);
   xpl = (const double*)(b + parts[9].off);
   xpl32 = (const float*)(b + parts[10].off);
+  xbox = (const float*)(b + parts[11].off);
   n_segs = lay.n_segs;
   n_sorted = (int)lay.n_sorted;
   n_xrec = (int)lay.xrec.size();
@@ -559,6 +561,7 @@
       q.xrec = L.xrec;
       q.xpl = ctx->plane_screen != 0 ? L.xpl : nullptr;
       q.xpl32 = ctx->plane_screen != 0 ? L.xpl32 : nullptr;
+      q.xbox = ctx->plane_screen != 0 && ctx->plane_screen != 3 ? L.xbox : nullptr;
       q.plane_gate2 = ctx->plane_screen == 2 ? 0.0 : 4.0 * tor::kPlaneGate * tor::kPlaneGate;
       q.xrec_lds_doubles = 0;
       if (q.xpl != nullptr && ctx->screen && accel == 0) {
@@ -1712,6 +1715,88 @@
   return TOR_OK;
 }
 
+int tor_debug_plane_cull_scene(TorHittableList world, int64_t n_rays, const double* o, const double* d, const double* time, int8_t* culled,
+                               int32_t* words_kept) {
+  if (world.len < 0 || (world.len > 0 && !world.objects) || n_rays < 0 || !o || !d || !time || !culled || !words_kept)
+    return fail(TOR_ERR_INVALID_ARGUMENT, "tor_debug_plane_cull_scene: bad argument");
+  std::vector<int64_t> ids((size_t)world.len);
+  for (int64_t i = 0; i < world.len; ++i) ids[(size_t)i] = i;
+  tor::HostLayout lay;
+  std::string err;
+  if (!tor::build_layout(world.objects, ids, lay, err, nullptr)) return fail(TOR_ERR_INVALID_ARGUMENT, err);
+  if (lay.xbox.size() < 8 * (size_t)lay.n_segs + 4 * (lay.n_sorted / 32 + 1))
+    return fail(TOR_ERR_INVALID_ARGUMENT, "tor_debug_plane_cull_scene: the box table is short (layout bug)");
+  auto orig_of = [&](size_t slot) {
+    int64_t v;
+    std::memcpy(&v, &lay.cold[16 * slot + 14], 8);
+    return v;
+  };
+  for (int64_t r = 0; r < n_rays; ++r) {
+    int8_t* cr = culled + r * world.len;
+    for (int64_t i = 0; i < world.len; ++i) cr[i] = 0;
+    words_kept[r] = 0;
+    const double* oo = o + 3 * r; const double* dd = d + 3 * r;
+    const double a = dd[0] * dd[0] + dd[1] * dd[1] + dd[2] * dd[2];
+    const tor::ScreenRay ray = tor::screen2_ray(oo[0], oo[1], oo[2], dd[0], dd[1], dd[2], a);
+    const tor::PlaneRay pray = tor::plane_ray(ray);
+    for (int s = 0; s < lay.n_segs; ++s) {
+      const double* sg = &lay.segs[8 * (size_t)s];
+      const double* xs = &lay.xsegs[8 * (size_t)s];
+      const double* h = &lay.xhdr[16 * (size_t)s];
+      const int xkind = (int)xs[0];
+      if (xkind < 10 || xkind == 13) continue;
+      const int count = (int)sg[2] & 0xffffff, real = count - ((int)sg[2] >> 24), block0 = (int)sg[3];
+      const double f = xkind >= 12 ? (time[r] - sg[4]) / sg[5] : 0.0;
+      const tor::PlaneSeg ps = tor::plane_seg(ray, pray, sg[6], sg[7], f, xs[4]);
+      float ec[2];
+      std::memcpy(ec, &h[15], 8);
+      const tor::PlaneSeg32 ps32 = tor::plane_seg32(ray, ps, h[13], h[14], (double)ec[0], (double)ec[1]);
+      const float* sr = &lay.xbox[8 * (size_t)s];
+      const tor::PlaneCull pc = tor::plane_cull_seg(ray, ps32, h[13], h[14], ec[1], sg[6], sg[7], f, sr[4], sr[0], sr[1], sr[2], sr[3]);
+      const size_t slot0 = (size_t)block0 * tor::kPad;
+      for (size_t w = (slot0 + 31) / 32; 32 * (w + 1) <= slot0 + (size_t)count; ++w) {
+        const float* b = &lay.xbox[8 * (size_t)lay.n_segs + 4 * w];
+        const bool drop = tor::plane_cull_word(ps32, pc, b[0], b[1], b[2], b[3]);
+        bool any = false;
+        for (size_t slot = 32 * w; slot < 32 * (w + 1) && slot < slot0 + (size_t)real; ++slot) {
+          any = true;
+          if (drop) cr[orig_of(slot)] = 1;
+        }
+        if (any && !drop) words_kept[r] += 1;
+      }
+    }
+  }
+  return TOR_OK;
+}
+
+int tor_debug_plane_cull_layout(TorHittableList world, int64_t max_slots, int32_t* slot_object, double* word_box, int64_t* n_slots_out) {
+  if (world.len < 0 || (world.len > 0 && !world.objects) || max_slots < 0 || (max_slots > 0 && (!slot_object || !word_box)) || !n_slots_out)
+    return fail(TOR_ERR_INVALID_ARGUMENT, "tor_debug_plane_cull_layout: bad argument");
+  std::vector<int64_t> ids((size_t)world.len);
+  for (int64_t i = 0; i < world.len; ++i) ids[(size_t)i] = i;
+  tor::HostLayout lay;
+  std::string err;
+  if (!tor::build_layout(world.objects, ids, lay, err, nullptr)) return fail(TOR_ERR_INVALID_ARGUMENT, err);
+  *n_slots_out = (int64_t)lay.n_sorted;
+  for (size_t slot = 0; slot < lay.n_sorted && (int64_t)slot < max_slots; ++slot) {
+    int64_t orig;
+    std::memcpy(&orig, &lay.cold[16 * slot + 14], 8);
+    slot_object[slot] = lay.cold[16 * slot + 15] < 0.0 ? -1 : (int32_t)orig;
+  }
+  for (size_t w = 0; 32 * w < lay.n_sorted && (int64_t)(32 * w) < max_slots; ++w) {
+    const float* b = &lay.xbox[8 * (size_t)lay.n_segs + 4 * w];
+    double* out = word_box + 6 * w;
+    for (int k = 0; k < 4; ++k) out[k] = (double)b[k];
+    out[4] = out[5] = 0.0;
+    for (int s = 0; s < lay.n_segs; ++s) {
+      const double* sg = &lay.segs[8 * (size_t)s];
+      const size_t slot0 = (size_t)sg[3] * tor::kPad, count = (size_t)((int)sg[2] & 0xffffff);
+      if (sg[0] < 3.0 && 32 * w >= slot0 && 32 * w < slot0 + count) { out[4] = lay.xpl32seg[4 * (size_t)s]; out[5] = lay.xpl32seg[4 * (size_t)s + 1]; }
+    }
+  }
+  return TOR_OK;
+}
+
 int tor_selftest_slab32_host(int64_t n, const double* o, const double* d, const double* lo, const double* hi,
                              const double* origin, int32_t* keep, int32_t* need) {
   if (n < 0 || !o || !d || !lo || !hi || !origin || !keep || !need)
diff --git a/trace-of-radiance_amd/csrc/tor_context.hpp b/trace-of-radiance_amd/csrc/tor_context.hpp
--- a/trace-of-radiance_amd/csrc/tor_context.hpp
+++ b/trace-of-radiance_amd/csrc/tor_context.hpp
@@ -69,6 +69,7 @@
   const double* coop_trips = nullptr;
   const double *xhdr = nullptr, *xrec = nullptr, *xpl = nullptr;
   const float* xpl32 = nullptr;
+  const float* xbox = nullptr;
   int n_segs = 0;
   int n_sorted = 0;
   int n_xrec = 0;
diff --git a/trace-of-radiance_amd/csrc/tor_kernels.hpp b/trace-of-radiance_amd/csrc/tor_kernels.hpp
--- a/trace-of-radiance_amd/csrc/tor_kernels.hpp
+++ b/trace-of-radiance_amd/csrc/tor_kernels.hpp
@@ -28,6 +28,7 @@
   const double* xhdr;
   const double* xpl;
   const float* xpl32;
+  const float* xbox;
   double plane_gate2;
   const float* hot32;
   double org[3];
diff --git a/trace-of-radiance_amd/csrc/tor_knobs.hpp b/trace-of-radiance_amd/csrc/tor_knobs.hpp
--- a/trace-of-radiance_amd/csrc/tor_knobs.hpp
+++ b/trace-of-radiance_amd/csrc/tor_knobs.hpp
@@ -26,7 +26,7 @@
     {"TOR_ACCEL_ORDER", "sah", "sah | morton", "upload", "order of the objects behind TOR_ACCEL_BLOCKS' boxes: top-down surface-area build (round 6) or the Morton curve of rounds 1-5 (A/B; same canvas)"},
     {"TOR_STAGE_LDS", "(no cap)", "bytes, 0 = off", "call", "cap of the LDS staging of block records / boxes (TOR_ACCEL_BLOCKS)"},
     {"TOR_SCREEN", "1", "0 | 1", "context", "0: strict brute-force launches evaluate the reference's unfused discriminant for every object instead of the conservative FMA screen (same canvas)"},
-    {"TOR_PLANE", "1", "0 | 1 | 2", "context", "stage one of the FMA screen (the 4-instruction plane screen in front of the segment's wave-uniform test, per-lane stage two on what it keeps): 0 off, 1 on the segments where it pays (default), 2 on every segment (same candidates, same canvas)"},
+    {"TOR_PLANE", "1", "0 | 1 | 2 | 3", "context", "stage one of the FMA screen (the 4-instruction plane screen in front of the segment's wave-uniform test, per-lane stage two on what it keeps): 0 off, 1 on the segments where it pays (default), 2 on every segment, 3 as 1 without the word cull behind stage one -- its per-word test still runs, against an infinite bound, so 3 shows what the cull drops, not the cost of a build without it; any other non-zero value is 1 (same candidates, same canvas)"},
     {"TOR_COOP_MAX_PIXELS", "114688", ">= 0", "context", "frames up to this many pixels (per device) run one WAVE per pixel when neither hand-off nor split mode applies; 0 = never"},
     {"TOR_LPT_MIN_SPP", "32", ">= 0", "context", "cost probe + chain-length-ordered tile schedule from this many spp on; 0 = never"},
     {"TOR_HOT_FRAC", "0.4", ">= 0", "context", "a pixel chain is HOT (arbiter priority 3) from this share of an average wave's iterations; 0 = off"},
diff --git a/trace-of-radiance_amd/csrc/tor_scene.cpp b/trace-of-radiance_amd/csrc/tor_scene.cpp
--- a/trace-of-radiance_amd/csrc/tor_scene.cpp
+++ b/trace-of-radiance_amd/csrc/tor_scene.cpp
@@ -125,6 +125,13 @@
   o.far_limit = 8.0 * dist[mid];
   if (!(o.far_limit > 0.0) || !std::isfinite(o.far_limit)) o.far_limit = 0.0;
   return o;
+}
+
+static int plane_gate(int xkind, size_t n_real, double rmax2, double ext_x, double ext_z) {
+  if (!(xkind >= 10 && n_real >= 48)) return 0;
+  const double band = 2.0 * kPlaneGate * std::sqrt(rmax2);
+  const double e_min = std::fmin(ext_x, ext_z), e_max = std::hypot(ext_x, ext_z);
+  return band < e_min ? 1 : (band < e_max ? 2 : 0);
 }
 
 bool build_layout(const TorHittableVariant* objs, const std::vector<int64_t>& ids, HostLayout& out, std::string& err,
@@ -298,8 +305,50 @@
 
   auto up = [](double x) { return x * (1.0 + 0x1p-40); };
   size_t sorted = 0, stat_rec = 0, mov_rec = 0, movy_rec = 0, x_off = 0, pl_off = 0;
-  for (const Seg64& sg : segs64) {
+  std::vector<float> box_seg, box_word(4 * (out.n_sorted / 32 + 1), 0.0f);
+  for (size_t w = 0; w < box_word.size() / 4; ++w) box_word[4 * w + 2] = box_word[4 * w + 3] = INFINITY;
+  for (Seg64& sg : segs64) {
     const size_t cnt_p = slots_of(sg, pad_words);
+    auto cx_of = [&](int64_t i) { return objs[i].kind == TOR_SPHERE ? objs[i].u.sphere.center.x : objs[i].u.moving_sphere.center0.x; };
+    auto cz_of = [&](int64_t i) { return objs[i].kind == TOR_SPHERE ? objs[i].u.sphere.center.z : objs[i].u.moving_sphere.center0.z; };
+    bool ordered = sg.xkind >= 10 && sg.xkind != 13 && sg.ids.size() >= 48;
+    if (ordered) {
+      double x0 = INFINITY, x1 = -INFINITY, z0 = INFINITY, z1 = -INFINITY, r2 = 0.0;
+      for (int64_t i : sg.ids) {
+        const double x = cx_of(i), z = cz_of(i);
+        if (std::isfinite(x)) { x0 = std::fmin(x0, x); x1 = std::fmax(x1, x); }
+        if (std::isfinite(z)) { z0 = std::fmin(z0, z); z1 = std::fmax(z1, z); }
+        r2 = std::fmax(r2, r2_of(i));
+      }
+      ordered = plane_gate(sg.xkind, sg.ids.size(), r2, x1 >= x0 ? x1 - x0 : 0.0, z1 >= z0 ? z1 - z0 : 0.0) == 1;
+    }
+    if (ordered) {
+      auto key = [](double v) { return std::isnan(v) ? INFINITY : v; };
+      std::vector<std::pair<size_t, size_t>> todo{{0, sg.ids.size()}};
+      while (!todo.empty()) {
+        const size_t lo = todo.back().first, hi = todo.back().second;
+        todo.pop_back();
+        const size_t wlo = (sorted + lo) / 32, whi = (sorted + hi + 31) / 32;
+        if (whi - wlo <= 1) {
+          std::sort(sg.ids.begin() + (long)lo, sg.ids.begin() + (long)hi);
+          continue;
+        }
+        const size_t mid = (wlo + (whi - wlo + 1) / 2) * 32 - sorted;
+        double x0 = INFINITY, x1 = -INFINITY, z0 = INFINITY, z1 = -INFINITY;
+        for (size_t k = lo; k < hi; ++k) {
+          const double x = cx_of(sg.ids[k]), z = cz_of(sg.ids[k]);
+          if (std::isfinite(x)) { x0 = std::fmin(x0, x); x1 = std::fmax(x1, x); }
+          if (std::isfinite(z)) { z0 = std::fmin(z0, z); z1 = std::fmax(z1, z); }
+        }
+        const bool by_x = !(z1 - z0 > x1 - x0);
+        std::nth_element(sg.ids.begin() + (long)lo, sg.ids.begin() + (long)mid, sg.ids.begin() + (long)hi, [&](int64_t a, int64_t b) {
+          const double ka = key(by_x ? cx_of(a) : cz_of(a)), kb = key(by_x ? cx_of(b) : cz_of(b));
+          return ka < kb || (ka == kb && a < b);
+        });
+        todo.push_back({lo, mid});
+        todo.push_back({mid, hi});
+      }
+    }
     double reach = 0.0, travel = 0.0, rmax2 = 0.0;
     double xlo = INFINITY, xhi = -INFINITY, zlo = INFINITY, zhi = -INFINITY, dcx_max = 0.0, dcz_max = 0.0;
     auto grow = [&](double x, double z) {
@@ -337,6 +386,44 @@
       cm32 = std::fmax(cm32, std::fmax(std::fabs((double)fx), std::fabs((double)fz)));
     }
     out.xpl32seg.insert(out.xpl32seg.end(), {orx, orz, e32, cm32});
+    {
+      double y0 = INFINITY, y1 = -INFINITY, d0 = 0.0, d1 = 0.0;
+      for (size_t k = 0; k < sg.ids.size() && ordered; ++k) {
+        const TorMovingSphere s = as_mover(sg.ids[k]);
+        const double dcy = s.center1.y - s.center0.y;
+        y0 = s.center0.y < y0 || std::isnan(s.center0.y) ? s.center0.y : y0;
+        y1 = s.center0.y > y1 || std::isnan(s.center0.y) ? s.center0.y : y1;
+        d0 = dcy < d0 || std::isnan(dcy) ? dcy : d0;
+        d1 = dcy > d1 || std::isnan(dcy) ? dcy : d1;
+      }
+      const double rup = std::sqrt(rmax2) * (1.0 + 0x1p-40);
+      box_seg.insert(box_seg.end(), {f32_below(y0), f32_above(y1), f32_below(d0), f32_above(d1), f32_above(rup), 0.0f, 0.0f, 0.0f});
+      for (size_t w = (sorted + 31) / 32; ordered && 32 * (w + 1) <= sorted + cnt_p; ++w) {
+        double lo[2] = {INFINITY, INFINITY}, hi[2] = {-INFINITY, -INFINITY};
+        bool bad = false;
+        size_t members = 0;
+        for (size_t k = 32 * w - sorted; k < 32 * (w + 1) - sorted && k < sg.ids.size(); ++k, ++members) {
+          const TorMovingSphere s = as_mover(sg.ids[k]);
+          const double dxz[2] = {s.center0.x - orx, s.center0.z - orz};
+          for (int a = 0; a < 2; ++a) {
+            bad = bad || !std::isfinite(dxz[a]);
+            lo[a] = std::fmin(lo[a], dxz[a]); hi[a] = std::fmax(hi[a], dxz[a]);
+          }
+        }
+        if (bad || members == 0) continue;
+        float* b = &box_word[4 * w];
+        for (int a = 0; a < 2; ++a) {
+          const float c = (float)(0.5 * lo[a] + 0.5 * hi[a]);
+          const double h = std::fmax(hi[a] - (double)c, (double)c - lo[a]), slack = std::fmax(std::fabs(lo[a]), std::fabs(hi[a])) * 0x1p-50;
+#if defined(TOR_SCREEN_MUTATE) && TOR_SCREEN_MUTATE == 6
+          b[a] = c; b[2 + a] = (float)(0.5 * (hi[a] - lo[a]));
+#else
+          b[a] = c; b[2 + a] = f32_above(h + slack);
+#endif
+          if (!std::isfinite(b[a]) || !std::isfinite(b[2 + a])) { b[0] = b[1] = 0.0f; b[2] = b[3] = INFINITY; break; }
+        }
+      }
+    }
     const size_t xs = (size_t)xs_of(sg.xkind), pw = (size_t)pw_of(sg.xkind);
     for (size_t k = 0; k < cnt_p && xs != 0; ++k) {
       double* x = &out.xrec[x_off + xs * k];
@@ -434,6 +521,7 @@
                                      (double)f32_round_up(mc0max * 1.000001), (double)f32_round_up(dcmax * 1.000001)});
     out.xsegs.insert(out.xsegs.end(), 8, 0.0);
     out.xpl32seg.insert(out.xpl32seg.end(), 4, 0.0);
+    box_seg.insert(box_seg.end(), 8, 0.0f);
     f_off += cnt_p / 2 * (size_t)stride;
     sorted += cnt_p;
     return true;
@@ -444,6 +532,8 @@
     if (!emit32(groups32[gi].ids, yonly32[gi] ? 6 : 7, first.time0, first.time1 - first.time0)) return false;
   }
   out.n_segs = (int)(out.segs.size() / 8);
+  out.xbox = box_seg;
+  out.xbox.insert(out.xbox.end(), box_word.begin(), box_word.end());
   if (out.segs.empty()) out.segs.assign(8, 0.0);
   if (out.xsegs.empty()) out.xsegs.assign(8, 0.0);
   out.xhdr.assign(16 * (size_t)std::max(out.n_segs, 1) + 16, 0.0);
@@ -451,13 +541,8 @@
     const double* sg = &out.segs[8 * (size_t)s];
     const double* xs = &out.xsegs[8 * (size_t)s];
     double* h = &out.xhdr[16 * (size_t)s];
-    int32_t gate = 0;
     const int n_real = ((int)sg[2] & 0xffffff) - ((int)sg[2] >> 24);
-    if ((int)xs[0] >= 10 && n_real >= 48) {
-      const double band = 2.0 * kPlaneGate * std::sqrt(xs[4]);
-      const double e_min = std::fmin(xs[5], xs[6]), e_max = std::hypot(xs[5], xs[6]);
-      gate = band < e_min ? 1 : (band < e_max ? 2 : 0);
-    }
+    const int32_t gate = plane_gate((int)xs[0], (size_t)n_real, xs[4], xs[5], xs[6]);
     const int32_t ints[8] = {(int32_t)xs[0], (int32_t)sg[0], (int32_t)sg[2], (int32_t)sg[3], (int32_t)sg[1], (int32_t)xs[1], (int32_t)xs[3], gate};
     std::memcpy(h, ints, sizeof(ints));
     h[4] = sg[4]; h[5] = sg[5]; h[6] = sg[6]; h[7] = sg[7];
diff --git a/trace-of-radiance_amd/csrc/tor_scene.hpp b/trace-of-radiance_amd/csrc/tor_scene.hpp
--- a/trace-of-radiance_amd/csrc/tor_scene.hpp
+++ b/trace-of-radiance_amd/csrc/tor_scene.hpp
@@ -15,6 +15,7 @@
   std::vector<double> xpl;
   std::vector<float> xpl32;
   std::vector<double> xpl32seg;
+  std::vector<float> xbox;
   std::vector<float> hot32;
   int n_segs = 0;
   size_t n_sorted = 0;
diff --git a/trace-of-radiance_amd/csrc/tor_screen.hpp b/trace-of-radiance_amd/csrc/tor_screen.hpp
--- a/trace-of-radiance_amd/csrc/tor_screen.hpp
+++ b/trace-of-radiance_amd/csrc/tor_screen.hpp
@@ -220,6 +220,73 @@
   return f;
 }
 
+struct PlaneCull {
+  float sc;
+  float hl;
+};
+TOR_HD float f32_above(double x) {
+  float f = (float)x;
+  if ((double)f < x) f = f > 0.0f ? __builtin_bit_cast(float, __builtin_bit_cast(uint32_t, f) + 1u)
+                         : (f < 0.0f ? __builtin_bit_cast(float, __builtin_bit_cast(uint32_t, f) - 1u) : 0x1p-149f);
+  return f;
+}
+TOR_HD float f32_below(double x) { return -f32_above(-x); }
+TOR_HD float rcp32(float x) {
+#if defined(__HIP_DEVICE_COMPILE__)
+  return __builtin_amdgcn_rcpf(x);
+#else
+  return 1.0f / x;
+#endif
+}
+TOR_HD PlaneCull plane_cull_seg(const ScreenRay& r, const PlaneSeg32& ps32, double orx, double orz, float cm, double reach,
+                                double travel, double f, float rup, float ylo, float yhi, float dlo, float dhi) {
+  const float up = 1.0f + 0x1p-20f;
+  const float ax = ps32.nz, az = -ps32.nx;
+  const float n1 = __builtin_fabsf(ax) + __builtin_fabsf(az);
+  const float aa = __builtin_fmaf(ax, ax, az * az);
+  const float Bf = (float)(r.s1 + reach + travel * __builtin_fabs(f)) * up;
+  const float ca = (float)-fma_((double)ax, r.ox - orx, (double)az * (r.oz - orz));
+  const float smax = __builtin_fmaf(4.0f * n1, cm, __builtin_fabsf(ca)) * (1.0f + 0x1p-10f) + 0x1p-100f;
+#if defined(TOR_SCREEN_MUTATE) && TOR_SCREEN_MUTATE == 4
+  const float rho0 = 0.0f, arho = 0.0f;
+#else
+  const float rho0 = __builtin_fmaf(Bf, 0x1p-22f, rup) * up;
+  const float arho = __builtin_fmaf(n1 * Bf, 0x1p-22f, ps32.T) * up;
+#endif
+  const float ff = (float)f, oy = (float)r.oy;
+  const float fd0 = ff * dlo, fd1 = ff * dhi;
+  const float yl = ylo + __builtin_fminf(fd0, fd1), yh = yhi + __builtin_fmaxf(fd0, fd1);
+  const float my = __builtin_fmaf(__builtin_fabsf(ylo) + __builtin_fabsf(yhi) + __builtin_fabsf(fd0) + __builtin_fabsf(fd1) + __builtin_fabsf(oy), 0x1p-20f, rho0);
+  const float a0 = (yl - oy) - my, a1 = (yh - oy) + my;
+  const float g = aa * rcp32((float)r.dny);
+  const bool ranged = __builtin_fabsf(g) < 0x1p60f && __builtin_fabsf(a0) < 0x1p60f && __builtin_fabsf(a1) < 0x1p60f;
+  const float e0 = a0 * g, e1 = a1 * g;
+  const float wd = __builtin_fmaf(__builtin_fabsf(e0) + __builtin_fabsf(e1), 0x1p-19f, 0x1p-80f);
+  float lo = ranged ? __builtin_fminf(e0, e1) - wd : -smax;
+  float hi = ranged ? __builtin_fmaxf(e0, e1) + wd : smax;
+#if defined(TOR_SCREEN_MUTATE) && TOR_SCREEN_MUTATE == 5
+  const float ahead = arho;
+#else
+  const float ahead = -((Bf * 0x1p-39f) * aa);
+#endif
+  lo = __builtin_fmaxf(lo, ahead);
+  lo = __builtin_fminf(__builtin_fmaxf(lo, -smax), smax);
+  hi = __builtin_fminf(__builtin_fmaxf(hi, -smax), smax);
+  const float mid = 0.5f * lo + 0.5f * hi, hf = 0.5f * hi - 0.5f * lo;
+  float hl = (hf + __builtin_fmaf(arho, 0x1p-18f, arho)) + __builtin_fmaf(smax, 0x1p-17f, 0x1p-100f);
+  hl = __builtin_fmaf(__builtin_fabsf(hl), 0x1p-20f, hl);
+  const bool all = !(ps32.T < __builtin_inff()) || !(smax < 0x1p60f) || !(arho < 0x1p60f) || !(aa > 0x1p-90f) || !(__builtin_fabsf(hl) < 0x1p60f);
+  PlaneCull c;
+  c.sc = all ? 0.0f : ca - mid;
+  c.hl = all ? __builtin_inff() : hl;
+  return c;
+}
+TOR_HD bool plane_cull_word(const PlaneSeg32& s, const PlaneCull& c, float bcx, float bcz, float hx, float hz) {
+  const float v = __builtin_fmaf(s.nz, bcx, __builtin_fmaf(-s.nx, bcz, c.sc));
+  const float e = __builtin_fmaf(__builtin_fabsf(s.nz), hx, __builtin_fmaf(__builtin_fabsf(s.nx), hz, c.hl));
+  return __builtin_fabsf(v) > e;
+}
+
 constexpr double kPlaneGate = 16.0;
 TOR_HD bool plane_pays(const PlaneRay& pr, double gate2, double rmax2, double sx, double sz) {
   const double e = fma_(__builtin_fabs(pr.nx), sx, __builtin_fabs(pr.nz) * sz);
```

After: 4051 (median of 6 runs). 1.04x the previous value.
